# leimao/Voice-Converter-CycleGAN

Measured on NVIDIA H100. Metric: CycleGAN-VC train steps/sec @ batch 256x[24,128] MCEP, higher is better.
Workload: dtype f16f8 (forward / data gradient: fp16 MMA + two e4m3 cross-term MMAs = 2 MMA units per product; weight gradient: fp16 MMA alone, 1 unit; f32 accumulate)

## Files before the change

include/cgvc.h:

```cpp
#ifndef CGVC_H
#define CGVC_H

#include <stddef.h>
#include <stdint.h>

#ifdef __cplusplus
extern "C" {
#endif

#define CGVC_ABI_VERSION 1
#define CGVC_NUM_LOSSES 8

typedef struct cgvc_engine* cgvc_handle;

typedef struct cgvc_config {
  int num_features;
  int max_batch;
  int max_frames;
  int precision;
  int device;
  int train;
} cgvc_config;

enum {
  CGVC_PREC_FP32_SIMT = 0,
  CGVC_PREC_BF16X3 = 1,
  CGVC_PREC_BF16 = 2,
  CGVC_PREC_F16F8 = 3
};

enum cgvc_arena {
  CGVC_ARENA_PARAM = 0,
  CGVC_ARENA_GRAD = 1,
  CGVC_ARENA_ADAM_M = 2,
  CGVC_ARENA_ADAM_V = 3,
  CGVC_ARENA_WORK = 4,
  CGVC_ARENA_COUNT = 5
};

int cgvc_abi_version(void);
int cgvc_create(const cgvc_config* cfg, cgvc_handle* out);
int cgvc_destroy(cgvc_handle h);
const char* cgvc_last_error(cgvc_handle h);

int cgvc_arena_bytes(cgvc_handle h, int arena, size_t* bytes);
int cgvc_bind_arena(cgvc_handle h, int arena, void* dev_ptr, size_t bytes);

int cgvc_param_count(cgvc_handle h, int* n_tensors, size_t* n_elements);
int cgvc_param_info(cgvc_handle h, int index, const char** name, size_t* offset, int* ndim, int shape_out[4]);

int cgvc_params_updated(cgvc_handle h, void* stream);
int cgvc_set_adam_step(cgvc_handle h, long long t);
int cgvc_get_adam_step(cgvc_handle h, long long* t);

typedef struct cgvc_loss_scale_info {
  float scale;
  int good_steps;
  long long skipped;
  int last_skipped;
  unsigned nonfinite;
  unsigned long long sat_grad;
  unsigned long long sat_act;
} cgvc_loss_scale_info;
int cgvc_loss_scale_state(cgvc_handle h, cgvc_loss_scale_info* out_dev, void* stream);
int cgvc_set_loss_scale_state(cgvc_handle h, float scale, int good_steps, long long skipped, void* stream);

int cgvc_train_step(cgvc_handle h, const float* A_dev, const float* B_dev, int batch, int frames,
                    float lambda_cycle, float lambda_identity, float lr_generator, float lr_discriminator,
                    float* gen_A_dev, float* gen_B_dev, float* losses_dev, void* stream);

int cgvc_compute_gradients(cgvc_handle h, const float* A_dev, const float* B_dev, int batch, int frames,
                           float lambda_cycle, float lambda_identity,
                           float* gen_A_dev, float* gen_B_dev, float* losses_dev, void* stream);

int cgvc_adam_step(cgvc_handle h, float lr_generator, float lr_discriminator, float grad_scale, void* stream);

int cgvc_generator_forward(cgvc_handle h, int direction, const float* in_dev, float* out_dev,
                           int batch, int frames, void* stream);
int cgvc_generator_forward_packed(cgvc_handle h, int direction, const float* in_dev, float* out_dev,
                                  const long long* offsets_host, int n, void* stream);
int cgvc_discriminator_forward(cgvc_handle h, int which, const float* in_dev, float* out_dev,
                               int batch, int frames, void* stream);

int cgvc_debug_activation(cgvc_handle h, const char* name, float* out_dev, size_t capacity, size_t* n_out, void* stream);

int cgvc_sample_plan(cgvc_handle h, const long long* offsets_A_dev, int n_A, const long long* offsets_B_dev, int n_B,
                     unsigned long long seed, long long epoch, int crop_frames, int* plan_dev, int* err_dev, void* stream);
int cgvc_gather_minibatch(cgvc_handle h, const float* corpus_A_dev, const long long* offsets_A_dev, const float* corpus_B_dev,
                          const long long* offsets_B_dev, const int* plan_dev, int num_pairs, int first_pair, int batch, int crop_frames,
                          float* A_out_dev, float* B_out_dev, void* stream);

int cgvc_comm_unique_id(cgvc_handle h, void* id128_host);
int cgvc_comm_init(cgvc_handle h, const void* id128_host, int rank, int nranks);
int cgvc_comm_destroy(cgvc_handle h);
int cgvc_allreduce_grads(cgvc_handle h, void* stream);

int cgvc_kernel_launches(unsigned long long* count);
int cgvc_set_option(cgvc_handle h, const char* name, int value);
int cgvc_profile_enable(int on);
int cgvc_profile_collect(double* ms3, double* flops3, long long* launches3);
int cgvc_profile_launches(double* ms, double* flops, long long* meta4, int capacity, int* n_out);

int cgvc_conv_forward(cgvc_handle h, int precision, const float* x, const float* w, const float* bias, float* y,
                      int B, int H, int W, int Cin, int kh, int kw, int Cout, int sh, int sw, void* stream);
int cgvc_conv_backward(cgvc_handle h, int precision, const float* x, const float* w, const float* dy,
                       float* dx, float* dw, float* dbias,
                       int B, int H, int W, int Cin, int kh, int kw, int Cout, int sh, int sw, void* stream);
int cgvc_in_glu_forward(cgvc_handle h, const float* p, const float* beta_a, const float* gamma_a,
                        const float* beta_g, const float* gamma_g, float* y, float* stats,
                        int B, int R, int C, int shuffle, void* stream);
int cgvc_in_glu_backward(cgvc_handle h, const float* dy, const float* p, const float* stats,
                         const float* beta_a, const float* gamma_a, const float* beta_g, const float* gamma_g,
                         float* dp, float* dbeta_a, float* dgamma_a, float* dbeta_g, float* dgamma_g,
                         int B, int R, int C, int shuffle, void* stream);
int cgvc_split_planes(cgvc_handle h, int precision, const float* x, long long rows, int C, void* hi, void* lo,
                      unsigned long long* sat, void* stream);
int cgvc_im2col_planes(cgvc_handle h, int precision, const float* x, long long rows, int T, int C, int kw, int dir, void* hi, void* lo,
                       unsigned long long* sat, void* stream);
int cgvc_in_glu_forward_planes(cgvc_handle h, const float* p, const float* beta_a, const float* gamma_a,
                               const float* beta_g, const float* gamma_g, float* y, float* stats,
                               int B, int R, int C, int shuffle, int precision, int gate, const float* resid,
                               void* hi, void* lo, unsigned long long* sat, void* stream);
int cgvc_in_glu_backward_planes(cgvc_handle h, const float* dy, const float* p, const float* stats,
                                const float* beta_a, const float* gamma_a, const float* beta_g, const float* gamma_g,
                                float* dp, float* dbeta_a, float* dgamma_a, float* dbeta_g, float* dgamma_g,
                                int B, int R, int C, int shuffle, int precision, int gate,
                                void* hi, void* lo, unsigned long long* sat, void* stream);

enum {
  CGVC_OK = 0,
  CGVC_ERR_ARG = -1,
  CGVC_ERR_CUDA = -2,
  CGVC_ERR_UNBOUND = -3,
  CGVC_ERR_DIRECTION = -4,
  CGVC_ERR_UNSUPPORTED = -5,
  CGVC_ERR_NCCL = -6
};

#ifdef __cplusplus
}
#endif
#endif
```

voice-converter-cyclegan_b200/_native.py:

```python
from __future__ import annotations

import ctypes as C
import os

from . import build as _build

_LIB = None

ARENA_PARAM, ARENA_GRAD, ARENA_ADAM_M, ARENA_ADAM_V, ARENA_WORK = range(5)
PREC_FP32_SIMT, PREC_BF16X3, PREC_BF16, PREC_F16F8 = 0, 1, 2, 3
PRECISIONS = {"fp32": PREC_FP32_SIMT, "fp32_simt": PREC_FP32_SIMT, "bf16x3": PREC_BF16X3, "bf16": PREC_BF16, "f16f8": PREC_F16F8}
ERR_DIRECTION = -4
ERR_UNSUPPORTED = -5

LOSS_NAMES = ("cycle_loss", "identity_loss", "generator_loss_A2B", "generator_loss_B2A", "generator_loss",
              "discriminator_loss_A", "discriminator_loss_B", "discriminator_loss")


class Config(C.Structure):
    _fields_ = [("num_features", C.c_int), ("max_batch", C.c_int), ("max_frames", C.c_int),
                ("precision", C.c_int), ("device", C.c_int), ("train", C.c_int)]


LOSS_SCALE_MODES = {"static": 0, "monitor": 1, "dynamic": 2}


class LossScaleInfo(C.Structure):
    _fields_ = [("scale", C.c_float), ("good_steps", C.c_int), ("skipped", C.c_longlong), ("last_skipped", C.c_int),
                ("nonfinite", C.c_uint), ("sat_grad", C.c_ulonglong), ("sat_act", C.c_ulonglong)]


class CgvcError(RuntimeError):
    def __init__(self, code, msg):
        super().__init__("libcgvc error %d: %s" % (code, msg))
        self.code = code


def _declare(lib):
    vp, ci, cf, sz = C.c_void_p, C.c_int, C.c_float, C.c_size_t
    P = C.POINTER
    sig = {
        "cgvc_abi_version": (ci, []),
        "cgvc_create": (ci, [P(Config), P(vp)]),
        "cgvc_destroy": (ci, [vp]),
        "cgvc_last_error": (C.c_char_p, [vp]),
        "cgvc_arena_bytes": (ci, [vp, ci, P(sz)]),
        "cgvc_bind_arena": (ci, [vp, ci, vp, sz]),
        "cgvc_param_count": (ci, [vp, P(ci), P(sz)]),
        "cgvc_param_info": (ci, [vp, ci, P(C.c_char_p), P(sz), P(ci), P(ci * 4)]),
        "cgvc_params_updated": (ci, [vp, vp]),
        "cgvc_set_adam_step": (ci, [vp, C.c_longlong]),
        "cgvc_get_adam_step": (ci, [vp, P(C.c_longlong)]),
        "cgvc_loss_scale_state": (ci, [vp, vp, vp]),
        "cgvc_set_loss_scale_state": (ci, [vp, cf, ci, C.c_longlong, vp]),
        "cgvc_train_step": (ci, [vp, vp, vp, ci, ci, cf, cf, cf, cf, vp, vp, vp, vp]),
        "cgvc_compute_gradients": (ci, [vp, vp, vp, ci, ci, cf, cf, vp, vp, vp, vp]),
        "cgvc_adam_step": (ci, [vp, cf, cf, cf, vp]),
        "cgvc_generator_forward": (ci, [vp, ci, vp, vp, ci, ci, vp]),
        "cgvc_generator_forward_packed": (ci, [vp, ci, vp, vp, P(C.c_longlong), ci, vp]),
        "cgvc_discriminator_forward": (ci, [vp, ci, vp, vp, ci, ci, vp]),
        "cgvc_debug_activation": (ci, [vp, C.c_char_p, vp, sz, P(sz), vp]),
        "cgvc_comm_unique_id": (ci, [vp, vp]),
        "cgvc_comm_init": (ci, [vp, vp, ci, ci]),
        "cgvc_comm_destroy": (ci, [vp]),
        "cgvc_allreduce_grads": (ci, [vp, vp]),
        "cgvc_sample_plan": (ci, [vp, vp, ci, vp, ci, C.c_ulonglong, C.c_longlong, ci, vp, vp, vp]),
        "cgvc_gather_minibatch": (ci, [vp, vp, vp, vp, vp, vp, ci, ci, ci, ci, vp, vp, vp]),
        "cgvc_kernel_launches": (ci, [P(C.c_ulonglong)]),
        "cgvc_set_option": (ci, [vp, C.c_char_p, ci]),
        "cgvc_profile_enable": (ci, [ci]),
        "cgvc_profile_collect": (ci, [P(C.c_double), P(C.c_double), P(C.c_longlong)]),
        "cgvc_profile_launches": (ci, [P(C.c_double), P(C.c_double), P(C.c_longlong), ci, P(ci)]),
        "cgvc_conv_forward": (ci, [vp, ci, vp, vp, vp, vp] + [ci] * 9 + [vp]),
        "cgvc_conv_backward": (ci, [vp, ci, vp, vp, vp, vp, vp, vp] + [ci] * 9 + [vp]),
        "cgvc_in_glu_forward": (ci, [vp] * 8 + [ci] * 4 + [vp]),
        "cgvc_in_glu_backward": (ci, [vp] * 13 + [ci] * 4 + [vp]),
        "cgvc_split_planes": (ci, [vp, ci, vp, C.c_longlong, ci, vp, vp, vp, vp]),
        "cgvc_im2col_planes": (ci, [vp, ci, vp, C.c_longlong, ci, ci, ci, ci, vp, vp, vp, vp]),
        "cgvc_in_glu_forward_planes": (ci, [vp] * 8 + [ci] * 6 + [vp] * 5),
        "cgvc_in_glu_backward_planes": (ci, [vp] * 13 + [ci] * 6 + [vp] * 4),
    }
    for name, (res, args) in sig.items():
        fn = getattr(lib, name)
        fn.restype = res
        fn.argtypes = args
    return sig


EXPORTED_SYMBOLS = None


def lib_path():
    return _build.LIB


def load(build_if_missing=True):
    global _LIB, EXPORTED_SYMBOLS
    if _LIB is not None:
        return _LIB
    path = _build.LIB
    if build_if_missing and _build.is_stale():
        _build.build()
    if not os.path.exists(path):
        raise RuntimeError("libcgvc.so not found at %s (run __graft_entry__.build()); there is no CPU fallback" % path)
    lib = C.CDLL(path, mode=C.RTLD_GLOBAL)
    EXPORTED_SYMBOLS = sorted(_declare(lib).keys())
    if lib.cgvc_abi_version() != 1:
        raise RuntimeError("libcgvc.so ABI version mismatch")
    _LIB = lib
    return lib


def check(handle, code):
    if code != 0:
        msg = _LIB.cgvc_last_error(handle)
        raise CgvcError(code, msg.decode() if msg else "?")
```

voice-converter-cyclegan_b200/csrc/engine.cu:

```cuda
#include "../../include/cgvc.h"
#include "kernels.cuh"
#include "tc_gemm.cuh"
#include "geom.h"

#include <dlfcn.h>
#include <stddef.h>
#include <math.h>
#include <stdarg.h>
#include <stdio.h>
#include <string.h>

#include <map>
#include <string>
#include <utility>
#include <vector>

static thread_local std::string g_create_error;

#define ADAM_B1 0.5f
#define ADAM_B2 0.999f
#define ADAM_EPS 1e-8f

struct TensorInfo { std::string name; size_t off; int ndim; int shape[4]; size_t numel; };
struct ConvW { size_t k, b; int kh, kw, cin, cout; };
// ... 1124 lines not shown
  DeviceGuard dguard; CK(dguard.set(e->cfg.device));
  Bump ws; ws.reset(e->arena[CGVC_ARENA_WORK], e->arena_bytes[CGVC_ARENA_WORK]);
  TrainPlan P; plan_train(e, ws, P, B, T);
  if (ws.overflow) return fail(e, CGVC_ERR_UNBOUND, "WORK arena too small for batch %d x %d frames", B, T);
  const size_t img = (size_t)B * nf * T;
  float* sc = e->d_scalars; float* L = sc + 8;
  (void)lc;
  CK(cudaMemsetAsync(L, 0, 8 * sizeof(float), st));
  if (e->ls_mode) CK(cudaMemsetAsync(&e->ls->nonfinite, 0, (char*)(&e->ls->sat_act + 1) - (char*)&e->ls->nonfinite, st));
  struct Counting { cgvc_engine* e; ~Counting() { e->counting = false; } } counting{e};
  e->counting = true;
  CK(cudaMemsetAsync(e->G(), 0, e->n_params * sizeof(float), st));
  CK(launch_transpose_ft(A_dev, P.lane[0].in, B, nf, T, st));
  CK(launch_transpose_ft(B_dev, P.lane[0].in + img, B, nf, T, st));
  CK(cudaMemcpyAsync(P.lane[1].in, P.lane[0].in + img, img * sizeof(float), cudaMemcpyDeviceToDevice, st));
  CK(cudaMemcpyAsync(P.lane[1].in + img, P.lane[0].in, img * sizeof(float), cudaMemcpyDeviceToDevice, st));
  for (int l = 0; l < 2; ++l) {
    SideQ& q = e->sideq[l];
    q.on = e->side_wgrad && e->two_streams && !e->fuse_bwd && !tc_profile_is_on() && q.side != nullptr;
    q.used[0] = q.used[1] = false; q.cur = 0;
  }
  if (e->two_streams) {
    CK(cudaEventRecord(e->ev_fork, st));
    for (int l = 0; l < 2; ++l) CK(cudaStreamWaitEvent(e->lane_stream[l], e->ev_fork, 0));
    RET(run_lane(e, P.lane[0], 0, B_dev, B, T, li, gen_B_dev, e->lane_stream[0]));
    RET(run_lane(e, P.lane[1], 1, A_dev, B, T, li, gen_A_dev, e->lane_stream[1]));
    for (int l = 0; l < 2; ++l) { CK(cudaEventRecord(e->ev_join[l], e->lane_stream[l])); CK(cudaStreamWaitEvent(st, e->ev_join[l], 0)); }
  } else {
    RET(run_lane(e, P.lane[0], 0, B_dev, B, T, li, gen_B_dev, st));
    RET(run_lane(e, P.lane[1], 1, A_dev, B, T, li, gen_A_dev, st));
  }
  CK(launch_finalize_losses(L, sc, st));
  if (losses_dev) CK(cudaMemcpyAsync(losses_dev, L, 8 * sizeof(float), cudaMemcpyDeviceToDevice, st));
  return 0;
}

}

static int set_lambdas(cgvc_engine* e, float lc, float li, cudaStream_t st) {
  float v[6] = {lc, li, 0, 0, 0, 0};
  CK(launch_set_scalars(e->d_scalars, 0, 2, v, st));
  return 0;
}
static int set_adam_scalars(cgvc_engine* e, float lr_g, float lr_d, float grad_scale, cudaStream_t st, bool deferred = false) {
  e->adam_t += 1;
  if (deferred) {
    float v[6] = {lr_g, grad_scale, lr_d, grad_scale, 0, 0};
    CK(launch_set_scalars(e->d_scalars, 2, 4, v, st));
    return 0;
  }
  double t = (double)e->adam_t;
  double corr = sqrt(1.0 - pow((double)ADAM_B2, t)) / (1.0 - pow((double)ADAM_B1, t));
  float v[6] = {(float)(lr_g * corr), grad_scale, (float)(lr_d * corr), grad_scale, 0, 0};
  CK(launch_set_scalars(e->d_scalars, 2, 4, v, st));
  return 0;
}
static int adam_body(cgvc_engine* e, cudaStream_t st, const int* skip = nullptr) {
  float* p = e->P(); float* g = e->G(); float* m = (float*)e->arena[CGVC_ARENA_ADAM_M]; float* v = (float*)e->arena[CGVC_ARENA_ADAM_V];
  size_t gend = e->gen[1].end;
  CK(launch_adam(p, g, m, v, (long long)gend, e->d_scalars + 2, ADAM_B1, ADAM_B2, ADAM_EPS, st, skip));
  CK(launch_adam(p + gend, g + gend, m + gend, v + gend, (long long)(e->n_params - gend), e->d_scalars + 4, ADAM_B1, ADAM_B2, ADAM_EPS, st, skip));
  return cgvc_params_updated(e, (void*)st);
}

static int ls_check_grads(cgvc_engine* e, cudaStream_t st) {
  CK(launch_check_finite(e->G(), (long long)e->n_params, (long long)e->gen[1].end, &e->ls->nonfinite, st));
  return 0;
}
static int ls_update(cgvc_engine* e, cudaStream_t st) {
  CK(launch_loss_scale_update(e->ls, e->d_scalars + 2, e->cfg.precision == CGVC_PREC_F16F8, e->ls_growth, ADAM_B1, ADAM_B2, st));
  return 0;
}
static const int* ls_skip(const cgvc_engine* e) { return e->ls_mode == 2 ? &e->ls->last_skipped : nullptr; }

static int ls_prepare(cgvc_engine* e, int batch, cudaStream_t st) {
  const bool dyn = e->ls_mode == 2 && !e->ls_ready, mon = e->ls_mode == 1 && e->ls_batch != batch;
  if (!dyn && !mon) return 0;
  const float v[6] = {loss_scale(e, batch), 0, 0, 0, 0, 0};
  CK(launch_set_scalars(&e->ls->scale, 0, 1, v, st));
  e->ls_ready = e->ls_mode == 2; e->ls_batch = e->ls_mode == 1 ? batch : 0;
  return 0;
}

template <class Body>
static int run_captured(cgvc_engine* e, const GraphKey& key, cudaStream_t user, Body body) {
  if (!e->use_graphs || tc_profile_is_on()) return body(user);
  cudaStream_t st = user;
  const bool bridge = (user == nullptr || user == cudaStreamLegacy || user == cudaStreamPerThread);
  if (bridge) { st = e->graph_stream; CK(cudaEventRecord(e->ev_bridge, user)); CK(cudaStreamWaitEvent(st, e->ev_bridge, 0)); }
  auto it = e->graphs.find(key);
  GraphEntry ent{nullptr, 0};
  if (it != e->graphs.end()) ent = it->second;
  else {
    if (e->graphs.size() >= 16) { for (auto& kv : e->graphs) cudaGraphExecDestroy(kv.second.exec); e->graphs.clear(); }
    cudaGraph_t graph = nullptr;
    const unsigned long long before = g_cgvc_launches;
    cudaError_t ce = cudaStreamBeginCapture(st, cudaStreamCaptureModeThreadLocal);
    if (ce != cudaSuccess) { cudaGetLastError(); e->use_graphs = 0; return body(user); }
    int rc = body(st);
    ce = cudaStreamEndCapture(st, &graph);
    ent.launches = g_cgvc_launches - before;
    g_cgvc_launches = before;
    if (rc != 0 || ce != cudaSuccess || !graph) {
      if (graph) cudaGraphDestroy(graph);
      cudaGetLastError();
      if (rc != 0 && ce == cudaSuccess) return rc;
      e->use_graphs = 0;
      return body(user);
    }
    ce = cudaGraphInstantiate(&ent.exec, graph, 0);
    cudaGraphDestroy(graph);
    if (ce != cudaSuccess) { cudaGetLastError(); e->use_graphs = 0; return body(user); }
    e->graphs[key] = ent;
  }
  cudaGraphExec_t exec = ent.exec;
  g_cgvc_launches += ent.launches;
  CK(cudaGraphLaunch(exec, st));
  if (bridge) { CK(cudaEventRecord(e->ev_bridge2, st)); CK(cudaStreamWaitEvent(user, e->ev_bridge2, 0)); }
  return 0;
}

extern "C" {

int cgvc_compute_gradients(cgvc_handle e, const float* A_dev, const float* B_dev, int batch, int frames,
                           float lambda_cycle, float lambda_identity, float* gen_A_dev, float* gen_B_dev, float* losses_dev, void* stream) {
  if (!e || !A_dev || !B_dev) return fail(e, CGVC_ERR_ARG, "null argument");
  DeviceGuard dguard; CK(dguard.set(e->cfg.device));
  RET(set_lambdas(e, lambda_cycle, lambda_identity, (cudaStream_t)stream));
  RET(ls_prepare(e, batch, (cudaStream_t)stream));
  RET(forward_backward(e, A_dev, B_dev, batch, frames, lambda_cycle, lambda_identity, gen_A_dev, gen_B_dev, losses_dev, (cudaStream_t)stream));
  if (e->ls_mode == 2) CK(launch_scale(e->G(), (long long)e->n_params, 1.f, (cudaStream_t)stream, &e->ls->scale));
  else if (loss_scale(e, batch) != 1.f) CK(launch_scale(e->G(), (long long)e->n_params, 1.f / loss_scale(e, batch), (cudaStream_t)stream));
  return 0;
}

int cgvc_adam_step(cgvc_handle e, float lr_g, float lr_d, float grad_scale, void* stream) {
  if (!e) return CGVC_ERR_ARG;
  for (int a = 0; a < 4; ++a) if (!e->arena[a]) return fail(e, CGVC_ERR_UNBOUND, "PARAM/GRAD/ADAM_M/ADAM_V arenas must be bound");
  DeviceGuard dguard; CK(dguard.set(e->cfg.device));
  if (e->ls_mode == 2) { long long t; RET(cgvc_get_adam_step(e, &t)); }
  const long long t_before = e->adam_t;
  RET(set_adam_scalars(e, lr_g, lr_d, grad_scale, (cudaStream_t)stream));
  int r = adam_body(e, (cudaStream_t)stream);
  if (r != 0) { e->adam_t = t_before; return r; }
  if (e->ls_mode == 2) RET(cgvc_set_adam_step(e, e->adam_t));
  return 0;
}

int cgvc_train_step(cgvc_handle e, const float* A_dev, const float* B_dev, int batch, int frames,
                    float lambda_cycle, float lambda_identity, float lr_g, float lr_d,
                    float* gen_A_dev, float* gen_B_dev, float* losses_dev, void* stream) {
  if (!e || !A_dev || !B_dev) return fail(e, CGVC_ERR_ARG, "null argument");
  for (int a = 0; a < 4; ++a) if (!e->arena[a]) return fail(e, CGVC_ERR_UNBOUND, "PARAM/GRAD/ADAM_M/ADAM_V arenas must be bound");
  RET(check_bt(e, batch, frames, 16));
  DeviceGuard dguard; CK(dguard.set(e->cfg.device));
  cudaStream_t st = (cudaStream_t)stream;
  const float gscale = (e->comm ? 1.f / (float)e->nranks : 1.f) / loss_scale(e, batch);
  RET(set_lambdas(e, lambda_cycle, lambda_identity, st));
  const long long adam_t_before = e->adam_t;
  struct Rollback { cgvc_engine* e; long long t; bool armed; ~Rollback() { if (armed) e->adam_t = t; } } rollback{e, adam_t_before, true};
  RET(set_adam_scalars(e, lr_g, lr_d, e->ls_mode == 2 ? (e->comm ? 1.f / (float)e->nranks : 1.f) : gscale, st, e->ls_mode == 2));
  RET(ls_prepare(e, batch, st));
  if (e->use_graphs && !tc_profile_is_on()) {
    const size_t img = (size_t)batch * e->cfg.num_features * frames;
    const size_t cap = (size_t)e->cfg.max_batch * e->cfg.num_features * e->cfg.max_frames;
    if (!e->stage) CK(cudaMalloc(&e->stage, 2 * cap * sizeof(float)));
    float* sA = e->stage; float* sB = e->stage + cap;
    CK(cudaMemcpyAsync(sA, A_dev, img * sizeof(float), cudaMemcpyDeviceToDevice, st));
    CK(cudaMemcpyAsync(sB, B_dev, img * sizeof(float), cudaMemcpyDeviceToDevice, st));
    GraphKey key; memset(&key, 0, sizeof key);
    key.batch = batch; key.frames = frames; key.id_off = lambda_identity == 0.f; key.lanes = e->two_streams; key.fuse = e->fuse_in | (e->fuse_bwd << 1) | (e->side_wgrad << 2) | (e->fuse_c1 << 3) | (e->edge_lower << 4); key.kind = 0;
    RET(run_captured(e, key, st, [&](cudaStream_t s) {
      return forward_backward(e, sA, sB, batch, frames, lambda_cycle, lambda_identity, nullptr, nullptr, nullptr, s);
    }));
    if (gen_A_dev || gen_B_dev) {
      Bump ws; ws.reset(e->arena[CGVC_ARENA_WORK], e->arena_bytes[CGVC_ARENA_WORK]);
      TrainPlan P; plan_train(e, ws, P, batch, frames);
      if (gen_B_dev) CK(cudaMemcpyAsync(gen_B_dev, P.lane[0].din + img, img * sizeof(float), cudaMemcpyDeviceToDevice, st));
      if (gen_A_dev) CK(cudaMemcpyAsync(gen_A_dev, P.lane[1].din + img, img * sizeof(float), cudaMemcpyDeviceToDevice, st));
    }
    if (losses_dev) CK(cudaMemcpyAsync(losses_dev, e->d_scalars + 8, 8 * sizeof(float), cudaMemcpyDeviceToDevice, st));
  } else {
    RET(forward_backward(e, A_dev, B_dev, batch, frames, lambda_cycle, lambda_identity, gen_A_dev, gen_B_dev, losses_dev, st));
  }
  if (e->comm && e->pipelined_comm && e->comm_stream) {
    auto al4 = [](size_t v) { return (v + 3) & ~(size_t)3; };
    const size_t cut[5] = {0, al4(e->gen[1].begin), al4(e->disc[0].begin), al4(e->disc[1].begin), e->n_params};
    struct Range { size_t b, n; const float* hyper; } rg[4];
    for (int k = 0; k < 4; ++k) { rg[k].b = cut[k]; rg[k].n = cut[k + 1] - cut[k]; rg[k].hyper = e->d_scalars + (k < 2 ? 2 : 4); }
    CK(cudaEventRecord(e->ev_grads, st));
    CK(cudaStreamWaitEvent(e->comm_stream, e->ev_grads, 0));
    for (int k = 0; k < 4; ++k) {
      int r = e->nccl.AllReduce(e->G() + rg[k].b, e->G() + rg[k].b, rg[k].n, 7, 0, e->comm, e->comm_stream);
      if (r != 0) return fail(e, CGVC_ERR_NCCL, "ncclAllReduce: %s", e->nccl.GetErrorString ? e->nccl.GetErrorString(r) : "?");
      CK(cudaEventRecord(e->ev_ar[k], e->comm_stream));
    }
    if (e->ls_mode) {
      if (e->ls_mode == 2) {
        int r = e->nccl.AllReduce(&e->ls->sat_grad, &e->ls->sat_grad, 1, 5, 0, e->comm, e->comm_stream);
        if (r != 0) return fail(e, CGVC_ERR_NCCL, "ncclAllReduce: %s", e->nccl.GetErrorString ? e->nccl.GetErrorString(r) : "?");
      }
      RET(ls_check_grads(e, e->comm_stream));
      CK(cudaEventRecord(e->ev_ls, e->comm_stream));
      if (e->ls_mode == 2) { CK(cudaStreamWaitEvent(st, e->ev_ls, 0)); RET(ls_update(e, st)); }
    }
    float* pp = e->P(); float* gg = e->G(); float* mm = (float*)e->arena[CGVC_ARENA_ADAM_M]; float* vv = (float*)e->arena[CGVC_ARENA_ADAM_V];
    for (int k = 0; k < 4; ++k) {
      CK(cudaStreamWaitEvent(st, e->ev_ar[k], 0));
      GraphKey kk; memset(&kk, 0, sizeof kk); kk.kind = 2 + k;
      const Range R = rg[k];
      RET(run_captured(e, kk, st, [&](cudaStream_t s) {
        CK(launch_adam(pp + R.b, gg + R.b, mm + R.b, vv + R.b, (long long)R.n, R.hyper, ADAM_B1, ADAM_B2, ADAM_EPS, s, ls_skip(e)));
        if (e->cfg.precision != CGVC_PREC_FP32_SIMT) {
          int r = tc_refresh_weights_range(e->tcw, pp, R.b, R.b + R.n, s);
          if (r != 0) return fail(e, CGVC_ERR_CUDA, "tc_refresh_weights: %s", cudaGetErrorString((cudaError_t)r));
        }
        return 0;
      }));
    }
    if (e->ls_mode == 1) CK(cudaStreamWaitEvent(st, e->ev_ls, 0));
    rollback.armed = false;
    return 0;
  }
  if (e->comm) {
    RET(cgvc_allreduce_grads(e, stream));
    if (e->ls_mode == 2) {
      int r = e->nccl.AllReduce(&e->ls->sat_grad, &e->ls->sat_grad, 1, 5, 0, e->comm, st);
      if (r != 0) return fail(e, CGVC_ERR_NCCL, "ncclAllReduce: %s", e->nccl.GetErrorString ? e->nccl.GetErrorString(r) : "?");
    }
  }
  GraphKey k2; memset(&k2, 0, sizeof k2); k2.kind = 1;
  RET(run_captured(e, k2, st, [&](cudaStream_t s) {
    if (e->ls_mode) RET(ls_check_grads(e, s));
    if (e->ls_mode == 2) RET(ls_update(e, s));
    return adam_body(e, s, ls_skip(e));
  }));
  rollback.armed = false;
  return 0;
}

static int load_nccl(cgvc_engine* e) {
  if (e->nccl.lib) return 0;
  const char* names[] = {"libnccl.so.2", "libnccl.so"};
  void* lib = nullptr;
  for (const char* n : names) { lib = dlopen(n, RTLD_NOW | RTLD_GLOBAL); if (lib) break; }
  if (!lib) return fail(e, CGVC_ERR_NCCL, "cannot dlopen libnccl.so.2: %s", dlerror());
  e->nccl.lib = lib;
  *(void**)&e->nccl.GetUniqueId = dlsym(lib, "ncclGetUniqueId");
  *(void**)&e->nccl.CommInitRank = dlsym(lib, "ncclCommInitRank");
  *(void**)&e->nccl.CommDestroy = dlsym(lib, "ncclCommDestroy");
  *(void**)&e->nccl.AllReduce = dlsym(lib, "ncclAllReduce");
  *(void**)&e->nccl.GetErrorString = dlsym(lib, "ncclGetErrorString");
  if (!e->nccl.GetUniqueId || !e->nccl.CommInitRank || !e->nccl.AllReduce || !e->nccl.CommDestroy)
    return fail(e, CGVC_ERR_NCCL, "libnccl is missing required symbols");
  return 0;
}

int cgvc_comm_unique_id(cgvc_handle e, void* id128_host) {
  if (!e || !id128_host) return CGVC_ERR_ARG;
  RET(load_nccl(e));
  int r = e->nccl.GetUniqueId(id128_host);
  if (r != 0) return fail(e, CGVC_ERR_NCCL, "ncclGetUniqueId: %s", e->nccl.GetErrorString ? e->nccl.GetErrorString(r) : "?");
  return 0;
}

int cgvc_comm_init(cgvc_handle e, const void* id128_host, int rank, int nranks) {
  if (!e || !id128_host || nranks < 1 || rank < 0 || rank >= nranks) return fail(e, CGVC_ERR_ARG, "cgvc_comm_init: bad argument");
  RET(load_nccl(e));
  DeviceGuard dguard; CK(dguard.set(e->cfg.device));
  Id128 id; memcpy(id.b, id128_host, 128);
  int r = e->nccl.CommInitRank(&e->comm, nranks, id, rank);
  if (r != 0) { e->comm = nullptr; return fail(e, CGVC_ERR_NCCL, "ncclCommInitRank: %s", e->nccl.GetErrorString ? e->nccl.GetErrorString(r) : "?"); }
  e->rank = rank; e->nranks = nranks;
  return 0;
}

int cgvc_comm_destroy(cgvc_handle e) {
  if (!e) return CGVC_ERR_ARG;
  if (e->comm) { e->nccl.CommDestroy(e->comm); e->comm = nullptr; e->nranks = 1; e->rank = 0; }
  return 0;
}

int cgvc_allreduce_grads(cgvc_handle e, void* stream) {
  if (!e) return CGVC_ERR_ARG;
  if (!e->comm) return fail(e, CGVC_ERR_NCCL, "no communicator attached");
  if (!e->arena[CGVC_ARENA_GRAD]) return fail(e, CGVC_ERR_UNBOUND, "GRAD arena must be bound");
  int r = e->nccl.AllReduce(e->G(), e->G(), e->n_params, 7, 0, e->comm, (cudaStream_t)stream);
  if (r != 0) return fail(e, CGVC_ERR_NCCL, "ncclAllReduce: %s", e->nccl.GetErrorString ? e->nccl.GetErrorString(r) : "?");
  return 0;
}

int cgvc_set_option(cgvc_handle e, const char* name, int value) {
  if (!e || !name) return CGVC_ERR_ARG;
  if (!strcmp(name, "two_streams")) { e->two_streams = value != 0; return 0; }
  if (!strcmp(name, "fuse_in")) { e->fuse_in = value != 0; return 0; }
  if (!strcmp(name, "fuse_bwd")) { e->fuse_bwd = value != 0; return 0; }
  if (!strcmp(name, "edge_lower")) { e->edge_lower = value != 0; return 0; }
  if (!strcmp(name, "side_wgrad")) { e->side_wgrad = value != 0; return 0; }
  if (!strcmp(name, "pipelined_comm")) { e->pipelined_comm = value != 0; return 0; }
  if (!strcmp(name, "fuse_c1")) { e->fuse_c1 = value != 0; return 0; }
  if (!strcmp(name, "debug_taps")) { e->debug_taps = value != 0; return 0; }
  if (!strcmp(name, "cuda_graph")) { e->use_graphs = value != 0; return 0; }
  if (!strcmp(name, "tc_debug")) { tc_set_debug(value); return 0; }
  if (!strcmp(name, "post_onepass")) {
    post_set_onepass(value);
    for (auto& kv : e->graphs) cudaGraphExecDestroy(kv.second.exec);
    e->graphs.clear();
    return 0;
  }
  if (!strcmp(name, "wgrad_f16")) {
    e->tcw.wgrad16 = value != 0;
    for (auto& kv : e->graphs) cudaGraphExecDestroy(kv.second.exec);
    e->graphs.clear();
    return 0;
  }
  if (!strcmp(name, "loss_scale") || !strcmp(name, "loss_scale_growth_interval")) {
    const bool mode = !strcmp(name, "loss_scale");
    if (mode ? (value < 0 || value > 2) : value < 1) return fail(e, CGVC_ERR_ARG, "option %s: bad value %d", name, value);
    if (mode && value != e->ls_mode) {
      DeviceGuard dguard; CK(dguard.set(e->cfg.device));
      long long t = 0;
      RET(cgvc_get_adam_step(e, &t));
      e->ls_mode = value;
      RET(cgvc_set_adam_step(e, t));
      e->ls_ready = false; e->ls_batch = 0;
    }
    if (!mode) e->ls_growth = value;
    for (auto& kv : e->graphs) cudaGraphExecDestroy(kv.second.exec);
    e->graphs.clear();
    return 0;
  }
  if (!strcmp(name, "post_stream")) {
    post_set_stream(value);
    for (auto& kv : e->graphs) cudaGraphExecDestroy(kv.second.exec);
    e->graphs.clear();
    return 0;
  }
  if (!strcmp(name, "prep_batched")) {
    tc_set_prep_batched(value);
    for (auto& kv : e->graphs) cudaGraphExecDestroy(kv.second.exec);
    e->graphs.clear();
    return 0;
  }
  return fail(e, CGVC_ERR_ARG, "unknown option '%s'", name);
}
int cgvc_kernel_launches(unsigned long long* count) { if (!count) return CGVC_ERR_ARG; *count = g_cgvc_launches; return 0; }
int cgvc_profile_enable(int on) { tc_profile_enable(on); return 0; }
int cgvc_profile_launches(double* ms, double* flops, long long* meta4, int capacity, int* n_out) {
  if (!ms || !flops || !meta4 || capacity < 0) return CGVC_ERR_ARG;
  return tc_profile_launches(ms, flops, meta4, capacity, n_out) == 0 ? 0 : CGVC_ERR_CUDA;
}
int cgvc_profile_collect(double* ms3, double* flops3, long long* launches3) {
  if (!ms3 || !flops3 || !launches3) return CGVC_ERR_ARG;
  return tc_profile_collect(ms3, flops3, launches3) == 0 ? 0 : CGVC_ERR_CUDA;
}

int cgvc_sample_plan(cgvc_handle e, const long long* offsets_A_dev, int n_A, const long long* offsets_B_dev, int n_B,
                     unsigned long long seed, long long epoch, int crop_frames, int* plan_dev, int* err_dev, void* stream) {
  if (!e || !offsets_A_dev || !offsets_B_dev || !plan_dev || !err_dev) return fail(e, CGVC_ERR_ARG, "null argument");
  if (n_A < 1 || n_B < 1 || crop_frames < 1 || epoch < 0) return fail(e, CGVC_ERR_ARG, "cgvc_sample_plan: empty corpus or bad crop / epoch");
  DeviceGuard dguard; CK(dguard.set(e->cfg.device));
  CK(cudaMemsetAsync(err_dev, 0, sizeof(int), (cudaStream_t)stream));
  CK(launch_sample_plan(offsets_A_dev, n_A, offsets_B_dev, n_B, seed, epoch, crop_frames, plan_dev, err_dev, (cudaStream_t)stream));
  return 0;
}

int cgvc_gather_minibatch(cgvc_handle e, const float* corpus_A_dev, const long long* offsets_A_dev, const float* corpus_B_dev,
                          const long long* offsets_B_dev, const int* plan_dev, int num_pairs, int first_pair, int batch, int crop_frames,
                          float* A_out_dev, float* B_out_dev, void* stream) {
  if (!e || !corpus_A_dev || !corpus_B_dev || !offsets_A_dev || !offsets_B_dev || !plan_dev || !A_out_dev || !B_out_dev)
    return fail(e, CGVC_ERR_ARG, "null argument");
  if (batch < 1 || first_pair < 0 || first_pair + batch > num_pairs || crop_frames < 1)
    return fail(e, CGVC_ERR_ARG, "cgvc_gather_minibatch: pairs [%d, %d) outside the epoch's %d", first_pair, first_pair + batch, num_pairs);
  DeviceGuard dguard; CK(dguard.set(e->cfg.device));
  CK(launch_gather_minibatch(corpus_A_dev, offsets_A_dev, corpus_B_dev, offsets_B_dev, plan_dev, num_pairs, first_pair, batch,
                             e->cfg.num_features, crop_frames, A_out_dev, B_out_dev, (cudaStream_t)stream));
  return 0;
}

int cgvc_conv_forward(cgvc_handle e, int precision, const float* x, const float* w, const float* bias, float* y,
                      int B, int H, int W, int Cin, int kh, int kw, int Cout, int sh, int sw, void* stream) {
  if (!e || !x || !w || !y) return fail(e, CGVC_ERR_ARG, "null argument");
  if (kh * kw > CGVC_MAX_TAPS) return fail(e, CGVC_ERR_UNSUPPORTED, "at most %d filter taps", CGVC_MAX_TAPS);
  DeviceGuard dguard; CK(dguard.set(e->cfg.device));
  cudaStream_t st = (cudaStream_t)stream;
  if (precision != CGVC_PREC_FP32_SIMT)
    return tc_result(e, tc_conv_fwd_adhoc(precision, x, w, bias, y, B, H, W, Cin, kh, kw, Cout, sh, sw, st), nullptr, "conv forward");
  GatherGeom g = fwd_geom(B, H, W, kh, kw, sh, sw);
  GemmOperands op; memset(&op, 0, sizeof op);
  op.src = x; op.s_ld = Cin; op.C = Cin; op.w = w; op.w_ts = (long long)Cin * Cout; op.w_cs = Cout; op.w_ns = 1; op.N = Cout;
  op.dst = y; op.d_ld = Cout; op.bias = bias;
  CK(launch_gg_simt(g, op, st));
  return 0;
}

int cgvc_conv_backward(cgvc_handle e, int precision, const float* x, const float* w, const float* dy,
                       float* dx, float* dw, float* dbias, int B, int H, int W, int Cin, int kh, int kw, int Cout, int sh, int sw, void* stream) {
  if (!e || !x || !w || !dy) return fail(e, CGVC_ERR_ARG, "null argument");
  if (kh * kw > CGVC_MAX_TAPS) return fail(e, CGVC_ERR_UNSUPPORTED, "at most %d filter taps", CGVC_MAX_TAPS);
  DeviceGuard dguard; CK(dguard.set(e->cfg.device));
  cudaStream_t st = (cudaStream_t)stream;
  if (precision != CGVC_PREC_FP32_SIMT)
    return tc_result(e, tc_conv_bwd_adhoc(precision, x, w, dy, dx, dw, dbias, B, H, W, Cin, kh, kw, Cout, sh, sw, st, e->tcw.wgrad16 ? 1 : 0),
                     nullptr, "conv backward");
  ConvW c; c.k = 0; c.b = 0; c.kh = kh; c.kw = kw; c.cin = Cin; c.cout = Cout;
  if (dx) RET(conv_dgrad_simt(e, w, c, sh, sw, B, H, W, dy, Cout, 0, dx, 0, st));
  if (dw) {
    GatherGeom g = fwd_geom(B, H, W, kh, kw, sh, sw);
    CK(launch_wgrad_simt(g, x, Cin, 0, Cin, dy, Cout, 0, Cout, dw, (long long)Cin * Cout, Cout, 1, st));
    if (dbias) CK(launch_colsum(dy, (long long)g.B * g.Hy * g.Wx, Cout, 0, Cout, dbias, st));
  }
  return 0;
}

static int plane_precision(cgvc_engine* e, int precision, const void* hi, const void* lo) {
  if (precision != CGVC_PREC_BF16X3 && precision != CGVC_PREC_BF16 && precision != CGVC_PREC_F16F8)
    return fail(e, CGVC_ERR_ARG, "operand planes: precision %d has none", precision);
  if (!hi || !lo) return fail(e, CGVC_ERR_ARG, "null argument");
  return 0;
}

int cgvc_split_planes(cgvc_handle e, int precision, const float* x, long long rows, int C, void* hi, void* lo,
                      unsigned long long* sat, void* stream) {
  if (!e || !x) return fail(e, CGVC_ERR_ARG, "null argument");
  RET(plane_precision(e, precision, hi, lo));
  if (rows < 0 || C < 1) return fail(e, CGVC_ERR_ARG, "cgvc_split_planes: bad shape [%lld, %d]", rows, C);
  DeviceGuard dguard; CK(dguard.set(e->cfg.device));
  CK(tc_split_planes(precision, x, rows, C, (__nv_bfloat16*)hi, (__nv_bfloat16*)lo, (cudaStream_t)stream, sat));
  return 0;
}

int cgvc_im2col_planes(cgvc_handle e, int precision, const float* x, long long rows, int T, int C, int kw, int dir, void* hi, void* lo,
                       unsigned long long* sat, void* stream) {
  if (!e || !x) return fail(e, CGVC_ERR_ARG, "null argument");
  RET(plane_precision(e, precision, hi, lo));
  if (T < 1 || rows < 0 || rows % T || C < 4 || C % 4 || kw < 1 || kw > CGVC_MAX_TAPS || (dir != 1 && dir != -1))
    return fail(e, CGVC_ERR_ARG, "cgvc_im2col_planes: bad shape (rows %lld, T %d, C %d, kw %d, dir %d)", rows, T, C, kw, dir);
  DeviceGuard dguard; CK(dguard.set(e->cfg.device));
  CK(launch_im2col_taps(x, rows, T, C, kw, dir, edge_cpad(kw * C), precision == CGVC_PREC_F16F8, hi, lo, (cudaStream_t)stream,
                        nullptr, 0, sat));
  return 0;
}

int cgvc_in_glu_forward_planes(cgvc_handle e, const float* p, const float* beta_a, const float* gamma_a, const float* beta_g,
                               const float* gamma_g, float* y, float* stats, int B, int R, int C, int shuffle, int precision, int gate,
                               const float* resid, void* hi, void* lo, unsigned long long* sat, void* stream) {
  if (!e || !p || !y || !stats) return fail(e, CGVC_ERR_ARG, "null argument");
  if (C % 32 != 0 || shuffle < 1 || R % shuffle != 0) return fail(e, CGVC_ERR_UNSUPPORTED, "C must be a multiple of 32 and R of shuffle");
  if (precision != CGVC_PREC_FP32_SIMT) RET(plane_precision(e, precision, hi, lo));
  DeviceGuard dguard; CK(dguard.set(e->cfg.device));
  PostParams q; memset(&q, 0, sizeof q);
  q.p = p; q.ldp = (gate ? 2 : 1) * C * shuffle; q.Cc = C * shuffle; q.B = B; q.R = R; q.C = C; q.sh = shuffle;
  q.beta_a = beta_a; q.gamma_a = gamma_a; q.beta_g = beta_g; q.gamma_g = gamma_g; q.has_in = 1; q.has_gate = gate != 0; q.resid = resid;
  q.y = y; q.stats = stats;
  if (precision != CGVC_PREC_FP32_SIMT) {
    q.y_hi = (__nv_bfloat16*)hi; q.y_lo = (__nv_bfloat16*)lo; q.qmode = precision == CGVC_PREC_F16F8; q.sat = q.qmode ? sat : nullptr;
  }
  CK(launch_post_fwd(q, (cudaStream_t)stream));
  return 0;
}

int cgvc_in_glu_backward_planes(cgvc_handle e, const float* dy, const float* p, const float* stats,
                                const float* beta_a, const float* gamma_a, const float* beta_g, const float* gamma_g,
                                float* dp, float* dbeta_a, float* dgamma_a, float* dbeta_g, float* dgamma_g,
                                int B, int R, int C, int shuffle, int precision, int gate, void* hi, void* lo, unsigned long long* sat,
                                void* stream) {
  if (!e || !dy || !p || !stats || !dp) return fail(e, CGVC_ERR_ARG, "null argument");
  if (C % 32 != 0 || shuffle < 1 || R % shuffle != 0) return fail(e, CGVC_ERR_UNSUPPORTED, "C must be a multiple of 32 and R of shuffle");
  if (precision != CGVC_PREC_FP32_SIMT) RET(plane_precision(e, precision, hi, lo));
  DeviceGuard dguard; CK(dguard.set(e->cfg.device));
  PostBwdParams q; memset(&q, 0, sizeof q);
  q.dy1 = dy; q.p = p; q.ldp = (gate ? 2 : 1) * C * shuffle; q.Cc = C * shuffle; q.B = B; q.R = R; q.C = C; q.sh = shuffle;
  q.beta_a = beta_a; q.gamma_a = gamma_a; q.beta_g = beta_g; q.gamma_g = gamma_g; q.has_in = 1; q.has_gate = gate != 0; q.stats = stats;
  q.dp = dp; q.dbeta_a = dbeta_a; q.dgamma_a = dgamma_a; q.dbeta_g = dbeta_g; q.dgamma_g = dgamma_g;
  if (precision != CGVC_PREC_FP32_SIMT) {
    q.dp_hi = (__nv_bfloat16*)hi; q.dp_lo = (__nv_bfloat16*)lo; q.qmode = precision == CGVC_PREC_F16F8; q.sat = q.qmode ? sat : nullptr;
  }
  CK(launch_post_bwd(q, (cudaStream_t)stream));
  return 0;
}

int cgvc_in_glu_forward(cgvc_handle e, const float* p, const float* beta_a, const float* gamma_a, const float* beta_g, const float* gamma_g,
                        float* y, float* stats, int B, int R, int C, int shuffle, void* stream) {
  return cgvc_in_glu_forward_planes(e, p, beta_a, gamma_a, beta_g, gamma_g, y, stats, B, R, C, shuffle, CGVC_PREC_FP32_SIMT, 1, nullptr,
                                    nullptr, nullptr, nullptr, stream);
}

int cgvc_in_glu_backward(cgvc_handle e, const float* dy, const float* p, const float* stats,
                         const float* beta_a, const float* gamma_a, const float* beta_g, const float* gamma_g,
                         float* dp, float* dbeta_a, float* dgamma_a, float* dbeta_g, float* dgamma_g,
                         int B, int R, int C, int shuffle, void* stream) {
  return cgvc_in_glu_backward_planes(e, dy, p, stats, beta_a, gamma_a, beta_g, gamma_g, dp, dbeta_a, dgamma_a, dbeta_g, dgamma_g,
                                     B, R, C, shuffle, CGVC_PREC_FP32_SIMT, 1, nullptr, nullptr, nullptr, stream);
}

}
```

voice-converter-cyclegan_b200/csrc/geom.h:

```cpp
#pragma once
#include "kernels.cuh"
#include <string.h>
#include <vector>

static inline void same_pad(int n, int k, int s, int& before, int& out) {
  out = (n + s - 1) / s;
  int total = (out - 1) * s + k - n; if (total < 0) total = 0;
  before = total / 2;
}

static inline GatherGeom fwd_geom(int B, int H, int W, int kh, int kw, int sh, int sw) {
  GatherGeom g; memset(&g, 0, sizeof g);
  int ph, pw, Ho, Wo; same_pad(H, kh, sh, ph, Ho); same_pad(W, kw, sw, pw, Wo);
  g.B = B; g.Hy = Ho; g.Wx = Wo; g.Hs = H; g.Ws = W; g.sy = sh; g.sx = sw;
  g.Hd = Ho; g.Wd = Wo; g.dsy = 1; g.dsx = 1; g.doy = 0; g.dox = 0;
  g.ntaps = 0;
  for (int i = 0; i < kh; ++i) for (int j = 0; j < kw; ++j) {
    g.oy[g.ntaps] = (short)(i - ph); g.ox[g.ntaps] = (short)(j - pw); g.widx[g.ntaps] = (short)(i * kw + j); g.ntaps++;
  }
  return g;
}

static inline bool divisible(int v, int s) { return ((v % s) + s) % s == 0; }

static inline std::vector<GatherGeom> dgrad_geoms(int B, int H, int W, int kh, int kw, int sh, int sw) {
  std::vector<GatherGeom> out;
  int ph, pw, Ho, Wo; same_pad(H, kh, sh, ph, Ho); same_pad(W, kw, sw, pw, Wo);
  for (int py = 0; py < sh; ++py) for (int px = 0; px < sw; ++px) {
    GatherGeom g; memset(&g, 0, sizeof g);
    g.B = B; g.Hy = (H - py + sh - 1) / sh; g.Wx = (W - px + sw - 1) / sw;
    if (g.Hy <= 0 || g.Wx <= 0) continue;
    g.Hs = Ho; g.Ws = Wo; g.sy = 1; g.sx = 1;
    g.Hd = H; g.Wd = W; g.dsy = sh; g.dsx = sw; g.doy = py; g.dox = px;
    g.ntaps = 0;
    for (int i = 0; i < kh; ++i) for (int j = 0; j < kw; ++j) {
      if (!divisible(py + ph - i, sh) || !divisible(px + pw - j, sw)) continue;
      g.oy[g.ntaps] = (short)((py + ph - i) / sh); g.ox[g.ntaps] = (short)((px + pw - j) / sw);
      g.widx[g.ntaps] = (short)(i * kw + j); g.ntaps++;
    }
    out.push_back(g);
  }
  return out;
}
```

voice-converter-cyclegan_b200/csrc/tc_gemm.cu:

```cuda
#include "tc_gemm.cuh"
#include "geom.h"
#include "kernels.cuh"
#include "wgmma.cuh"

#include <cuda.h>
#include <stdint.h>
#include <stdio.h>

namespace {

typedef CUresult (*EncodeTiledFn)(CUtensorMap*, CUtensorMapDataType, cuuint32_t, void*, const cuuint64_t*, const cuuint64_t*,
                                  const cuuint32_t*, const cuuint32_t*, CUtensorMapInterleave, CUtensorMapSwizzle,
                                  CUtensorMapL2promotion, CUtensorMapFloatOOBfill);
EncodeTiledFn get_encoder() {
  static EncodeTiledFn fn = nullptr;
  if (!fn) {
    void* p = nullptr; cudaDriverEntryPointQueryResult q;
    if (cudaGetDriverEntryPoint("cuTensorMapEncodeTiled", &p, cudaEnableDefault, &q) == cudaSuccess && q == cudaDriverEntryPointSuccess)
      fn = (EncodeTiledFn)p;
  }
  return fn;
}
bool make_tmap3(CUtensorMap* m, const void* base, uint64_t d0, uint64_t d1, uint64_t d2, uint32_t b1) {
  EncodeTiledFn enc = get_encoder();
  if (!enc) return false;
  cuuint64_t dims[3] = {d0, d1, d2};
  cuuint64_t strides[2] = {d0 * 2, d0 * d1 * 2};
  cuuint32_t box[3] = {64, b1, 1};
  cuuint32_t es[3] = {1, 1, 1};
  return enc(m, CU_TENSOR_MAP_DATA_TYPE_BFLOAT16, 3, const_cast<void*>(base), dims, strides, box, es, CU_TENSOR_MAP_INTERLEAVE_NONE,
             CU_TENSOR_MAP_SWIZZLE_128B, CU_TENSOR_MAP_L2_PROMOTION_L2_256B, CU_TENSOR_MAP_FLOAT_OOB_FILL_NONE) == CUDA_SUCCESS;
}

bool make_tmap3_t(CUtensorMap* m, const void* base, CUtensorMapDataType dt, int esize, uint64_t d0, uint64_t d1, uint64_t d2, uint32_t b0, uint32_t b1) {
  EncodeTiledFn enc = get_encoder();
  if (!enc) return false;
  cuuint64_t dims[3] = {d0, d1, d2};
  cuuint64_t strides[2] = {d0 * (uint64_t)esize, d0 * d1 * (uint64_t)esize};
  cuuint32_t box[3] = {b0, b1, 1};
  cuuint32_t es[3] = {1, 1, 1};
  return enc(m, dt, 3, const_cast<void*>(base), dims, strides, box, es, CU_TENSOR_MAP_INTERLEAVE_NONE,
             b0 * esize == 64 ? CU_TENSOR_MAP_SWIZZLE_64B : CU_TENSOR_MAP_SWIZZLE_128B, CU_TENSOR_MAP_L2_PROMOTION_L2_256B,
             CU_TENSOR_MAP_FLOAT_OOB_FILL_NONE) == CUDA_SUCCESS;
}

__device__ __forceinline__ uint32_t smem_u32(const void* p) { return (uint32_t)__cvta_generic_to_shared(p); }

__device__ __forceinline__ void mbar_init(uint64_t* bar, uint32_t count) {
  asm volatile("mbarrier.init.shared::cta.b64 [%0], %1;" ::"r"(smem_u32(bar)), "r"(count));
}
__device__ __forceinline__ void fence_barrier_init() { asm volatile("fence.mbarrier_init.release.cluster;" ::: "memory"); }
__device__ __forceinline__ void mbar_wait(uint64_t* bar, uint32_t parity) {
  asm volatile(
      "{\n\t"
      ".reg .pred p;\n\t"
      "WAIT_LOOP:\n\t"
      "mbarrier.try_wait.parity.shared::cta.b64 p, [%0], %1;\n\t"
      "@p bra.uni WAIT_DONE;\n\t"
      "bra.uni WAIT_LOOP;\n\t"
      "WAIT_DONE:\n\t"
      "}" ::"r"(smem_u32(bar)), "r"(parity) : "memory");
}
__device__ __forceinline__ void cp_async16(uint32_t dst_smem, const void* src, uint32_t src_bytes) {
  asm volatile("cp.async.cg.shared.global [%0], [%1], 16, %2;" ::"r"(dst_smem), "l"(src), "r"(src_bytes) : "memory");
}
__device__ __forceinline__ void cp_async_arrive_noinc(uint64_t* bar) {
  asm volatile("cp.async.mbarrier.arrive.noinc.shared::cta.b64 [%0];" ::"r"(smem_u32(bar)) : "memory");
}
__device__ __forceinline__ void mbar_expect_tx(uint64_t* bar, uint32_t bytes) {
  asm volatile("mbarrier.arrive.expect_tx.shared::cta.b64 _, [%0], %1;" ::"r"(smem_u32(bar)), "r"(bytes) : "memory");
}
__device__ __forceinline__ void tma_load3(uint32_t dst_smem, const CUtensorMap* map, int c0, int c1, int c2, uint64_t* bar) {
  asm volatile("cp.async.bulk.tensor.3d.shared::cluster.global.tile.mbarrier::complete_tx::bytes [%0], [%1, {%2, %3, %4}], [%5];"
               ::"r"(dst_smem), "l"(map), "r"(c0), "r"(c1), "r"(c2), "r"(smem_u32(bar)) : "memory");
}
__device__ __forceinline__ void tma_prefetch_desc(const CUtensorMap* map) {
  asm volatile("prefetch.tensormap [%0];" ::"l"(map) : "memory");
}
__device__ __forceinline__ void fence_proxy_async() { asm volatile("fence.proxy.async.shared::cta;" ::: "memory"); }
__device__ __forceinline__ uint64_t make_desc(uint32_t smem_addr, uint32_t lbo_bytes, uint32_t sbo_bytes, uint64_t layout = 1) {
  return (uint64_t)((smem_addr >> 4) & 0x3FFF) | ((uint64_t)((lbo_bytes >> 4) & 0x3FFF) << 16) |
         ((uint64_t)((sbo_bytes >> 4) & 0x3FFF) << 32) | (layout << 62);
}
__device__ __forceinline__ uint64_t make_desc64(uint32_t smem_addr) { return make_desc(smem_addr, 16, 512, 2); }
template <int N>
__device__ __forceinline__ void fence_acc(float (&d)[N]) {
#pragma unroll
  for (int i = 0; i < N; ++i) asm volatile("" : "+f"(d[i])::"memory");
}
__device__ __forceinline__ void mbar_arrive(uint64_t* bar) {
  asm volatile("mbarrier.arrive.shared::cta.b64 _, [%0];" ::"r"(smem_u32(bar)) : "memory");
}
__device__ __forceinline__ void consumer_bar() { asm volatile("bar.sync 3, 256;" ::: "memory"); }
__device__ __forceinline__ void st_shared16(uint32_t addr, uint4 v) {
  asm volatile("st.shared.v4.b32 [%0], {%1, %2, %3, %4};" ::"r"(addr), "r"(v.x), "r"(v.y), "r"(v.z), "r"(v.w) : "memory");
}
__device__ __forceinline__ uint4 e4m3x8_to_f16x8(uint2 v) {
  uint32_t w[4];
#pragma unroll
  for (int i = 0; i < 4; ++i) {
    const uint32_t src = (i < 2 ? v.x : v.y) >> (16 * (i & 1));
    const __half2_raw h = __nv_cvt_fp8x2_to_halfraw2((__nv_fp8x2_storage_t)(src & 0xFFFFu), __NV_E4M3);
    w[i] = (uint32_t)h.x | ((uint32_t)h.y << 16);
  }
  return make_uint4(w[0], w[1], w[2], w[3]);
}

struct FastDiv { uint32_t mul, shr, d; };
__host__ inline FastDiv make_fastdiv(uint32_t d) {
  FastDiv f; f.d = d;
  uint32_t l = 0; while ((1ull << l) < d) ++l;
  f.mul = (uint32_t)(((1ull << 32) * ((1ull << l) - d)) / d + 1);
  f.shr = l;
  return f;
}
__device__ __forceinline__ uint32_t fdiv(uint32_t n, const FastDiv& f) { return (uint32_t)(((uint64_t)__umulhi(n, f.mul) + n) >> f.shr); }

__device__ __forceinline__ uint32_t sw128(int r, int c) { return (uint32_t)((r >> 3) * 1024 + (r & 7) * 128 + ((c ^ (r & 7)) << 4)); }

struct TcNTParams {
  GatherGeom g;
  const __nv_bfloat16 *a_hi, *a_lo; int a_ld; int C;
  const __nv_bfloat16 *b_hi, *b_lo; int Nw;
  int N;
  int n_tiles;
  int debug;
  float* dst; int d_ld; const float* bias; int accumulate;
  int perm; int Cc;
  int R;
  const float *gamma_a, *beta_a, *gamma_g, *beta_g;
  float* stats;
  const float* resid;
  float* y; __nv_bfloat16 *y_hi, *y_lo;
  int C_out;
  const float* bp; int bp_ld;
  __nv_bfloat16 *dp_hi, *dp_lo; int dp_ld;
  float *dbeta_a, *dgamma_a, *dbeta_g, *dgamma_g;
  CUtensorMap tm_b_hi, tm_b_lo;
  const uint8_t *a8_hi, *a8_lo;
  CUtensorMap tm_b8_hi, tm_b8_lo;
  uint8_t* y8;
  PackGeom pk;
};

struct TcTNParams {
  GatherGeom g;
  const __nv_bfloat16 *x_hi, *x_lo; int x_ld; int C;
  const __nv_bfloat16 *g_hi, *g_lo; int g_ld; int N;
  float* dw_a; float* dw_g; int n_split;
  int ksplit;
  FastDiv div_hw, div_w;
  CUtensorMap tm_g_hi, tm_g_lo;
  const uint8_t *x8_hi, *x8_lo;
  const uint8_t *g8_hi, *g8_lo;
  int w16;
  int fold_n;
};

__device__ __forceinline__ float* tn_dst(float* base, int slab, int C, int c, int ncols, int col, int fold_n) {
  if (fold_n) { const int t = col / fold_n; return base + ((long long)t * C + c) * fold_n + (col - t * fold_n); }
  return base + ((long long)slab * C + c) * ncols + col;
}

constexpr int kProducerThreads = 128;


template <int BN, int NPL>
struct NTCfg {
  static constexpr int A_PLANE = 128 * 128;
  static constexpr int B_PLANE = BN * 128;
  static constexpr int PLANES = NPL == 2 ? 2 : 1;
  static constexpr int STAGE = PLANES * (A_PLANE + B_PLANE);
  static constexpr int STAGES = (192 * 1024) / STAGE;
  static constexpr int SMEM = STAGES * STAGE + 1024;
  static_assert(STAGES * STAGE >= 128 * BN * 4, "the finished fp32 tile is staged over the pipeline stages");
};

template <int BN>
__device__ __forceinline__ int acc_off(int r, int n) { return r * BN + (n & ~31) + ((((n >> 2) & 7) ^ (r & 7)) << 2) + (n & 3); }
template <int BN>
__device__ __forceinline__ void acc_ld32(const float* acc, int r, int col, uint32_t (&v)[32]) {
#pragma unroll
  for (int c = 0; c < 8; ++c) {
    const float4 x = *reinterpret_cast<const float4*>(acc + r * BN + col + ((c ^ (r & 7)) << 2));
    v[4 * c] = __float_as_uint(x.x); v[4 * c + 1] = __float_as_uint(x.y); v[4 * c + 2] = __float_as_uint(x.z); v[4 * c + 3] = __float_as_uint(x.w);
  }
}

__device__ __forceinline__ float warp_colsum32(float (&t)[32], int lane) {
#pragma unroll
  for (int o = 16, n = 32; o >= 1; o >>= 1, n >>= 1) {
    const bool up = (lane & o) != 0;
#pragma unroll
    for (int i = 0; i < n / 2; ++i) {
      float send = up ? t[i] : t[i + n / 2];
      float keep = up ? t[i + n / 2] : t[i];
      t[i] = keep + __shfl_xor_sync(0xffffffffu, send, o);
    }
  }
  return t[0];
}
__device__ __forceinline__ void epi_bar(int id) { asm volatile("bar.sync %0, 128;" ::"r"(id) : "memory"); }

__device__ __forceinline__ float sample_sum(float v, float (*xch)[32], int q, int lane, int spw, int barid) {
  if (spw == 1) return v;
  epi_bar(barid);
  xch[q][lane] = v;
  epi_bar(barid);
  const int q0 = (q / spw) * spw;
  float r = 0.f;
  for (int w = 0; w < spw; ++w) r += xch[q0 + w][lane];
  return r;
}
__device__ __forceinline__ void bc4(const float* p, float (&v)[4]) { const float4 x = *reinterpret_cast<const float4*>(p); v[0] = x.x; v[1] = x.y; v[2] = x.z; v[3] = x.w; }
__device__ __forceinline__ float fast_sigmoid(float x) { return __fdividef(1.f, 1.f + __expf(-x)); }
__device__ __forceinline__ void chunk_norm_coeffs(const float (&v)[32], const float* __restrict__ gamma, const float* __restrict__ beta,
                                                  int ch, int R, float (*xch)[32], float* bc, int q, int lane, int spw, int barid, float& mean, float& rstd) {
  float t[32];
#pragma unroll
  for (int k = 0; k < 32; ++k) t[k] = v[k];
  float s = warp_colsum32(t, lane);
  s = sample_sum(s, xch, q, lane, spw, barid);
  mean = s / (float)R;
  __syncwarp();
  bc[lane] = mean;
  __syncwarp();
#pragma unroll
  for (int k = 0; k < 32; k += 4) {
    float4 m4 = *reinterpret_cast<const float4*>(bc + k);
    float d0 = v[k] - m4.x, d1 = v[k + 1] - m4.y, d2 = v[k + 2] - m4.z, d3 = v[k + 3] - m4.w;
    t[k] = d0 * d0; t[k + 1] = d1 * d1; t[k + 2] = d2 * d2; t[k + 3] = d3 * d3;
  }
  float ss = warp_colsum32(t, lane);
  ss = sample_sum(ss, xch, q, lane, spw, barid);
  rstd = 1.f / sqrtf(ss / (float)R + 1e-6f);
  const float sc = rstd * gamma[ch + lane];
  const float of = beta[ch + lane] - mean * sc;
  __syncwarp();
  bc[lane] = sc; bc[32 + lane] = of;
  __syncwarp();
}

__device__ __forceinline__ void pair_norm_coeffs(const float (&v0)[32], const float (&v1)[32], const float* __restrict__ gamma, const float* __restrict__ beta,
                                                 int ch, int R, float (*xch)[32], float* bc, int q, int lane, int spw, int barid, float& mean, float& rstd) {
  float t[32];
#pragma unroll
  for (int k = 0; k < 32; ++k) t[k] = v0[k] + v1[k];
  float s = warp_colsum32(t, lane);
  s = sample_sum(s, xch, q, lane, spw, barid);
  const float inv = 1.f / (float)(2 * R);
  mean = s * inv;
  __syncwarp();
  bc[lane] = mean;
  __syncwarp();
#pragma unroll
  for (int k = 0; k < 32; k += 4) {
    float4 m4 = *reinterpret_cast<const float4*>(bc + k);
    const float m[4] = {m4.x, m4.y, m4.z, m4.w};
#pragma unroll
    for (int j = 0; j < 4; ++j) { const float d0 = v0[k + j] - m[j], d1 = v1[k + j] - m[j]; t[k + j] = fmaf(d0, d0, d1 * d1); }
  }
  float ss = warp_colsum32(t, lane);
  ss = sample_sum(ss, xch, q, lane, spw, barid);
  rstd = 1.f / sqrtf(ss * inv + 1e-6f);
  const float sc = rstd * gamma[ch + lane];
  const float of = beta[ch + lane] - mean * sc;
  __syncwarp();
  bc[lane] = sc; bc[32 + lane] = of;
  __syncwarp();
}

__device__ __forceinline__ uint32_t hp_off(int r, int c) { return (uint32_t)(r * 16 + ((c ^ ((r >> 1) & 3)) << 2)); }
template <class F>
__device__ __forceinline__ void rows_out(float* stg, const float (&o)[32], int lane, F f) {
  const int hc = lane & 3, hr = lane >> 2;
#pragma unroll
  for (int h = 0; h < 2; ++h) {
    __syncwarp();
#pragma unroll
    for (int c = 0; c < 4; ++c)
      *reinterpret_cast<float4*>(stg + hp_off(lane, c)) = make_float4(o[16 * h + 4 * c], o[16 * h + 4 * c + 1], o[16 * h + 4 * c + 2], o[16 * h + 4 * c + 3]);
    __syncwarp();
#pragma unroll
    for (int i = 0; i < 4; ++i) {
      const int rr = hr + 8 * i;
      f(rr, 16 * h + 4 * hc, *reinterpret_cast<const float4*>(stg + hp_off(rr, hc)));
    }
  }
}
__device__ __forceinline__ void rows_in(float* stg, float (&v)[32], int lane, const float4 (&pre)[8]) {
  const int hc = lane & 3, hr = lane >> 2;
#pragma unroll
  for (int h = 0; h < 2; ++h) {
    __syncwarp();
#pragma unroll
    for (int i = 0; i < 4; ++i) *reinterpret_cast<float4*>(stg + hp_off(hr + 8 * i, hc)) = pre[4 * h + i];
    __syncwarp();
#pragma unroll
    for (int c = 0; c < 4; ++c) {
      const float4 x = *reinterpret_cast<const float4*>(stg + hp_off(lane, c));
      v[16 * h + 4 * c] = x.x; v[16 * h + 4 * c + 1] = x.y; v[16 * h + 4 * c + 2] = x.z; v[16 * h + 4 * c + 3] = x.w;
    }
  }
}
__device__ __forceinline__ void rows_fetch(float4 (&pre)[8], const float* base, long long ld, long long mq, long long M, int col, int lane) {
  const int hc = lane & 3, hr = lane >> 2;
#pragma unroll
  for (int h = 0; h < 2; ++h)
#pragma unroll
    for (int i = 0; i < 4; ++i) {
      const int rr = hr + 8 * i;
      pre[4 * h + i] = make_float4(0.f, 0.f, 0.f, 0.f);
      if (mq + rr < M) pre[4 * h + i] = *reinterpret_cast<const float4*>(base + (mq + rr) * ld + col + 16 * h + 4 * hc);
    }
}
__device__ __forceinline__ void hload_rows(float* stg, float (&v)[32], const float* base, long long ld, long long mq, long long M, int col, int lane) {
  float4 pre[8];
  rows_fetch(pre, base, ld, mq, M, col, lane);
  rows_in(stg, v, lane, pre);
}
__device__ __forceinline__ void hwrite_rows_f32(float* stg, const float (&o)[32], float* const* rowp, int col0, int lane) {
  rows_out(stg, o, lane, [&](int rr, int w0, float4 val) {
    float* rp = rowp[rr];
    if (rp != nullptr) *reinterpret_cast<float4*>(rp + col0 + w0) = val;
  });
}
__device__ __forceinline__ void hwrite_y(float* stg, const float (&y)[32], float* yf, __nv_bfloat16* yhi, __nv_bfloat16* ylo,
                                         long long mq, long long M, int C, int ch, int lane, int rs = 1, int ro = 0) {
  if (yf)
    rows_out(stg, y, lane, [&](int rr, int w0, float4 val) {
      if (mq + rr < M) *reinterpret_cast<float4*>(yf + ((mq + rr) * rs + ro) * C + ch + w0) = val;
    });
  float hl[32];
#pragma unroll
  for (int k = 0; k < 16; ++k) {
    __nv_bfloat162 hh = __floats2bfloat162_rn(y[2 * k], y[2 * k + 1]);
    float2 f = __bfloat1622float2(hh);
    __nv_bfloat162 ll = __floats2bfloat162_rn(y[2 * k] - f.x, y[2 * k + 1] - f.y);
    hl[k] = __uint_as_float(*reinterpret_cast<uint32_t*>(&hh)); hl[16 + k] = __uint_as_float(*reinterpret_cast<uint32_t*>(&ll));
  }
  rows_out(stg, hl, lane, [&](int rr, int w0, float4 val) {
    __nv_bfloat16* plane = (w0 < 16) ? yhi : ylo;
    if (mq + rr < M) *reinterpret_cast<float4*>(plane + ((mq + rr) * rs + ro) * C + ch + 2 * (w0 & 15)) = val;
  });
}
__device__ __forceinline__ void hwrite_yq(float* stg, const float (&y)[32], float* yf, __nv_bfloat16* q16, uint8_t* q8,
                                          long long mq, long long M, int C, int ch, int lane, int rs = 1, int ro = 0) {
  if (yf)
    rows_out(stg, y, lane, [&](int rr, int w0, float4 val) {
      if (mq + rr < M) *reinterpret_cast<float4*>(yf + ((mq + rr) * rs + ro) * C + ch + w0) = val;
    });
  float w[32];
#pragma unroll
  for (int k = 0; k < 8; ++k) {
    const float v[4] = {y[4 * k], y[4 * k + 1], y[4 * k + 2], y[4 * k + 3]};
    uint2 h; uint32_t b_hi, b_lo;
    cgvc_quant4(v, CGVC_Q_ACT_SHI, CGVC_Q_ACT_SLO, h, b_hi, b_lo);
    w[2 * k] = __uint_as_float(h.x); w[2 * k + 1] = __uint_as_float(h.y);
    w[16 + k] = __uint_as_float(b_hi); w[24 + k] = __uint_as_float(b_lo);
  }
  rows_out(stg, w, lane, [&](int rr, int w0, float4 val) {
    if (mq + rr >= M) return;
    const long long r = (mq + rr) * rs + ro;
    uint8_t* dst;
    if (w0 < 16) dst = reinterpret_cast<uint8_t*>(q16) + (r * C + ch + 2 * w0) * 2;
    else if (w0 < 24) dst = q8 + r * C + ch + 4 * (w0 - 16);
    else dst = q8 + M * rs * C + r * C + ch + 4 * (w0 - 24);
    *reinterpret_cast<float4*>(dst) = val;
  });
}

template <int BN, int NPL, int EPI>
__device__ __forceinline__ void nt_tile_epilogue(const TcNTParams& p, const long long M, const int HW, const long long m0, const int n0,
                                                 const int q, const int lane, float* stg, float** rowp, float* bc, float (*epi_xch)[32],
                                                 const float* acc, const int grp = 0, const int ngrp = 1) {
  const GatherGeom& g = p.g;
  const int barid = 1 + grp;
  const int arow = q * 32 + lane;
  const long long mq = m0 + q * 32;
  const long long m = mq + lane;
  float* drow = nullptr;
  if (m < M && p.dst) {
    int b = (int)(m / HW); int rem = (int)(m - (long long)b * HW);
    int y = rem / g.Wx; int x = rem - y * g.Wx;
    long long dr = ((long long)(b * g.Hd + y * g.dsy + g.doy) * g.Wd + x * g.dsx + g.dox);
    drow = p.dst + dr * p.d_ld;
  }
  __syncwarp();
  rowp[lane] = drow;
  __syncwarp();
  {
    const int spw = p.R >> 5;
    const long long sample = mq / p.R;
    const bool stat_writer = (q % spw) == 0 && mq < M && p.stats != nullptr;
    if (EPI == 1) {
      const int ch0 = n0 >> 1;
#pragma unroll 1
      for (int cb = grp; cb < 4; cb += ngrp) {
        const int ch = ch0 + cb * 32;
        float va[32], vg[32];
        { uint32_t u[32]; acc_ld32<BN>(acc, arow, (cb * 32), u);
#pragma unroll
          for (int k = 0; k < 32; k += 4) { float4 bb = *reinterpret_cast<const float4*>(p.bias + n0 + cb * 32 + k);
            va[k] = __uint_as_float(u[k]) + bb.x; va[k + 1] = __uint_as_float(u[k + 1]) + bb.y; va[k + 2] = __uint_as_float(u[k + 2]) + bb.z; va[k + 3] = __uint_as_float(u[k + 3]) + bb.w; } }
        { uint32_t u[32]; acc_ld32<BN>(acc, arow, (128 + cb * 32), u);
#pragma unroll
          for (int k = 0; k < 32; k += 4) { float4 bb = *reinterpret_cast<const float4*>(p.bias + n0 + 128 + cb * 32 + k);
            vg[k] = __uint_as_float(u[k]) + bb.x; vg[k + 1] = __uint_as_float(u[k + 1]) + bb.y; vg[k + 2] = __uint_as_float(u[k + 2]) + bb.z; vg[k + 3] = __uint_as_float(u[k + 3]) + bb.w; } }
        if (p.dst) {
          hwrite_rows_f32(stg, va, rowp, ch, lane);
          hwrite_rows_f32(stg, vg, rowp, p.Cc + ch, lane);
        }
        float mean_a, rstd_a, mean_g, rstd_g;
        chunk_norm_coeffs(va, p.gamma_a, p.beta_a, ch, p.R, epi_xch, bc, q, lane, spw, barid, mean_a, rstd_a);
        chunk_norm_coeffs(vg, p.gamma_g, p.beta_g, ch, p.R, epi_xch, bc + 64, q, lane, spw, barid, mean_g, rstd_g);
        if (stat_writer) {
          float* st = p.stats + sample * 4 * p.C_out + ch + lane;
          st[0] = mean_a; st[p.C_out] = rstd_a; st[2 * p.C_out] = mean_g; st[3 * p.C_out] = rstd_g;
        }
#pragma unroll
        for (int k = 0; k < 32; k += 4) {
          float4 sa = *reinterpret_cast<const float4*>(bc + k), oa = *reinterpret_cast<const float4*>(bc + 32 + k);
          float4 sg = *reinterpret_cast<const float4*>(bc + 64 + k), og = *reinterpret_cast<const float4*>(bc + 96 + k);
          va[k]     = fmaf(va[k],     sa.x, oa.x) * fast_sigmoid(fmaf(vg[k],     sg.x, og.x));
          va[k + 1] = fmaf(va[k + 1], sa.y, oa.y) * fast_sigmoid(fmaf(vg[k + 1], sg.y, og.y));
          va[k + 2] = fmaf(va[k + 2], sa.z, oa.z) * fast_sigmoid(fmaf(vg[k + 2], sg.z, og.z));
          va[k + 3] = fmaf(va[k + 3], sa.w, oa.w) * fast_sigmoid(fmaf(vg[k + 3], sg.w, og.w));
        }
        if (NPL == 3) hwrite_yq(stg, va, p.y, p.y_hi, p.y8, mq, M, p.C_out, ch, lane);
        else hwrite_y(stg, va, p.y, p.y_hi, p.y_lo, mq, M, p.C_out, ch, lane);
      }
    } else if (EPI == 5) {
      const int Ch = p.C_out;
      const int ch0 = n0 >> 2;
#pragma unroll 1
      for (int cb = grp; cb < 2; cb += ngrp) {
        const int ch = ch0 + cb * 32;
        auto load = [&](float (&v)[32], int tcol) {
          uint32_t u[32]; acc_ld32<BN>(acc, arow, tcol, u);
#pragma unroll
          for (int k = 0; k < 32; k += 4) { float4 bb = *reinterpret_cast<const float4*>(p.bias + n0 + tcol + k);
            v[k] = __uint_as_float(u[k]) + bb.x; v[k + 1] = __uint_as_float(u[k + 1]) + bb.y; v[k + 2] = __uint_as_float(u[k + 2]) + bb.z; v[k + 3] = __uint_as_float(u[k + 3]) + bb.w; }
        };
        float mean_a, rstd_a, mean_g, rstd_g;
        {
          float g0[32], g1[32];
          load(g0, 128 + cb * 32); load(g1, 192 + cb * 32);
          if (p.dst) { hwrite_rows_f32(stg, g0, rowp, p.Cc + ch, lane); hwrite_rows_f32(stg, g1, rowp, p.Cc + Ch + ch, lane); }
          pair_norm_coeffs(g0, g1, p.gamma_g, p.beta_g, ch, p.R, epi_xch, bc + 64, q, lane, spw, barid, mean_g, rstd_g);
        }
        float a0[32], a1[32];
        load(a0, cb * 32); load(a1, 64 + cb * 32);
        if (p.dst) { hwrite_rows_f32(stg, a0, rowp, ch, lane); hwrite_rows_f32(stg, a1, rowp, Ch + ch, lane); }
        pair_norm_coeffs(a0, a1, p.gamma_a, p.beta_a, ch, p.R, epi_xch, bc, q, lane, spw, barid, mean_a, rstd_a);
        if (stat_writer) {
          float* st = p.stats + sample * 4 * Ch + ch + lane;
          st[0] = mean_a; st[Ch] = rstd_a; st[2 * Ch] = mean_g; st[3 * Ch] = rstd_g;
        }
        auto emit = [&](const float (&a)[32], const int s) {
          float gg[32];
          load(gg, 128 + s * 64 + cb * 32);
#pragma unroll
          for (int k = 0; k < 32; k += 4) {
            float4 sa = *reinterpret_cast<const float4*>(bc + k), oa = *reinterpret_cast<const float4*>(bc + 32 + k);
            float4 sg = *reinterpret_cast<const float4*>(bc + 64 + k), og = *reinterpret_cast<const float4*>(bc + 96 + k);
            gg[k]     = fmaf(a[k],     sa.x, oa.x) * fast_sigmoid(fmaf(gg[k],     sg.x, og.x));
            gg[k + 1] = fmaf(a[k + 1], sa.y, oa.y) * fast_sigmoid(fmaf(gg[k + 1], sg.y, og.y));
            gg[k + 2] = fmaf(a[k + 2], sa.z, oa.z) * fast_sigmoid(fmaf(gg[k + 2], sg.z, og.z));
            gg[k + 3] = fmaf(a[k + 3], sa.w, oa.w) * fast_sigmoid(fmaf(gg[k + 3], sg.w, og.w));
          }
          if (NPL == 3) hwrite_yq(stg, gg, p.y, p.y_hi, p.y8, mq, M, Ch, ch, lane, 2, s);
          else hwrite_y(stg, gg, p.y, p.y_hi, p.y_lo, mq, M, Ch, ch, lane, 2, s);
        };
        emit(a1, 1);
        emit(a0, 0);
      }
    } else if (EPI == 2) {
#pragma unroll 1
      for (int cb = grp; cb < BN / 32; cb += ngrp) {
        const int ch = n0 + cb * 32;
        if (ch >= p.N) break;
        float4 rpre[8];
        rows_fetch(rpre, p.resid, p.C_out, mq, M, ch, lane);
        float va[32];
        { uint32_t u[32]; acc_ld32<BN>(acc, arow, (cb * 32), u);
#pragma unroll
          for (int k = 0; k < 32; k += 4) { float4 bb = *reinterpret_cast<const float4*>(p.bias + ch + k);
            va[k] = __uint_as_float(u[k]) + bb.x; va[k + 1] = __uint_as_float(u[k + 1]) + bb.y; va[k + 2] = __uint_as_float(u[k + 2]) + bb.z; va[k + 3] = __uint_as_float(u[k + 3]) + bb.w; } }
        if (p.dst) hwrite_rows_f32(stg, va, rowp, ch, lane);
        float mean_a, rstd_a;
        chunk_norm_coeffs(va, p.gamma_a, p.beta_a, ch, p.R, epi_xch, bc, q, lane, spw, barid, mean_a, rstd_a);
        if (stat_writer) {
          float* st = p.stats + sample * 4 * p.C_out + ch + lane;
          st[0] = mean_a; st[p.C_out] = rstd_a; st[2 * p.C_out] = 0.f; st[3 * p.C_out] = 1.f;
        }
        float res[32];
        rows_in(stg, res, lane, rpre);
#pragma unroll
        for (int k = 0; k < 32; k += 4) {
          float4 scl = *reinterpret_cast<const float4*>(bc + k), of = *reinterpret_cast<const float4*>(bc + 32 + k);
          va[k] = fmaf(va[k], scl.x, of.x) + res[k]; va[k + 1] = fmaf(va[k + 1], scl.y, of.y) + res[k + 1];
          va[k + 2] = fmaf(va[k + 2], scl.z, of.z) + res[k + 2]; va[k + 3] = fmaf(va[k + 3], scl.w, of.w) + res[k + 3];
        }
        if (NPL == 3) hwrite_yq(stg, va, p.y, p.y_hi, p.y8, mq, M, p.C_out, ch, lane);
        else hwrite_y(stg, va, p.y, p.y_hi, p.y_lo, mq, M, p.C_out, ch, lane);
      }
    } else {
      const int C = p.C_out;
      const float invR = 1.f / (float)p.R;
      const bool live = mq < M;
#pragma unroll 1
      for (int cb = grp; cb < BN / 32; cb += ngrp) {
        const int ch = n0 + cb * 32;
        if (ch >= p.N) break;
        float dy[32], xa[32];
        { uint32_t u[32]; acc_ld32<BN>(acc, arow, (cb * 32), u);
#pragma unroll
          for (int k = 0; k < 32; ++k) dy[k] = __uint_as_float(u[k]); }
        if (p.accumulate) {
          hload_rows(stg, xa, p.dst, p.d_ld, mq, M, ch, lane);
#pragma unroll
          for (int k = 0; k < 32; ++k) dy[k] += xa[k];
        }
        if (EPI == 4) {
          rows_out(stg, dy, lane, [&](int rr, int w0, float4 val) {
            if (mq + rr < M) *reinterpret_cast<float4*>(p.dst + (mq + rr) * p.d_ld + ch + w0) = val;
          });
        }
        {
          const float* st = p.stats + sample * 4 * C + ch + lane;
          const float mean = live ? st[0] : 0.f, rstd = live ? st[C] : 1.f;
          const float scl = rstd * p.gamma_a[ch + lane];
          __syncwarp();
          bc[lane] = rstd; bc[32 + lane] = -mean * rstd; bc[64 + lane] = scl;
          if (EPI == 3) {
            bc[96 + lane] = p.beta_a[ch + lane] - mean * scl;
            const float mg = live ? st[2 * C] : 0.f, rg = live ? st[3 * C] : 1.f;
            const float sg = rg * p.gamma_g[ch + lane];
            bc[128 + lane] = rg; bc[160 + lane] = -mg * rg; bc[192 + lane] = sg; bc[224 + lane] = p.beta_g[ch + lane] - mg * sg;
          }
          __syncwarp();
        }
        hload_rows(stg, xa, p.bp, p.bp_ld, mq, M, ch, lane);
        float dg[32], xg[32];
        if (EPI == 3) {
          hload_rows(stg, xg, p.bp, p.bp_ld, mq, M, C + ch, lane);
#pragma unroll
          for (int k = 0; k < 32; k += 4) {
            float ra[4], ha[4], sa[4], oa[4], rg[4], hg[4], sg[4], og[4];
            bc4(bc + k, ra); bc4(bc + 32 + k, ha); bc4(bc + 64 + k, sa); bc4(bc + 96 + k, oa);
            bc4(bc + 128 + k, rg); bc4(bc + 160 + k, hg); bc4(bc + 192 + k, sg); bc4(bc + 224 + k, og);
#pragma unroll
            for (int j = 0; j < 4; ++j) {
              const float na = fmaf(xa[k + j], sa[j], oa[j]), ng = fmaf(xg[k + j], sg[j], og[j]);
              const float sgm = fast_sigmoid(ng);
              const float dna = dy[k + j] * sgm;
              dy[k + j] = dna; dg[k + j] = dna * na * (1.f - sgm);
              xa[k + j] = fmaf(xa[k + j], ra[j], ha[j]);
              xg[k + j] = fmaf(xg[k + j], rg[j], hg[j]);
            }
          }
        } else {
#pragma unroll
          for (int k = 0; k < 32; k += 4) {
            float ra[4], ha[4];
            bc4(bc + k, ra); bc4(bc + 32 + k, ha);
#pragma unroll
            for (int j = 0; j < 4; ++j) xa[k + j] = fmaf(xa[k + j], ra[j], ha[j]);
          }
        }
        float t[32];
#pragma unroll
        for (int k = 0; k < 32; ++k) t[k] = dy[k];
        float s1a = warp_colsum32(t, lane);
#pragma unroll
        for (int k = 0; k < 32; ++k) t[k] = dy[k] * xa[k];
        float s2a = warp_colsum32(t, lane);
        float s1g = 0.f, s2g = 0.f;
        if (EPI == 3) {
#pragma unroll
          for (int k = 0; k < 32; ++k) t[k] = dg[k];
          s1g = warp_colsum32(t, lane);
#pragma unroll
          for (int k = 0; k < 32; ++k) t[k] = dg[k] * xg[k];
          s2g = warp_colsum32(t, lane);
        }
        if (p.dbeta_a && live) {
          atomicAdd(p.dbeta_a + ch + lane, s1a); atomicAdd(p.dgamma_a + ch + lane, s2a);
          if (EPI == 3) { atomicAdd(p.dbeta_g + ch + lane, s1g); atomicAdd(p.dgamma_g + ch + lane, s2g); }
        }
        s1a = sample_sum(s1a, epi_xch, q, lane, spw, barid); s2a = sample_sum(s2a, epi_xch, q, lane, spw, barid);
        if (EPI == 3) { s1g = sample_sum(s1g, epi_xch, q, lane, spw, barid); s2g = sample_sum(s2g, epi_xch, q, lane, spw, barid); }
        {
          const float sca = bc[64 + lane], scg = EPI == 3 ? bc[192 + lane] : 0.f;
          __syncwarp();
          bc[256 + lane] = sca * s1a * invR; bc[288 + lane] = sca * s2a * invR;
          if (EPI == 3) { bc[320 + lane] = scg * s1g * invR; bc[352 + lane] = scg * s2g * invR; }
          __syncwarp();
        }
#pragma unroll
        for (int k = 0; k < 32; k += 4) {
          float c1[4], c2[4], c3[4];
          bc4(bc + 64 + k, c1); bc4(bc + 256 + k, c2); bc4(bc + 288 + k, c3);
#pragma unroll
          for (int j = 0; j < 4; ++j) dy[k + j] = fmaf(c1[j], dy[k + j], -fmaf(xa[k + j], c3[j], c2[j]));
        }
        hwrite_y(stg, dy, nullptr, p.dp_hi, p.dp_lo, mq, M, p.dp_ld, ch, lane);
        if (EPI == 3) {
#pragma unroll
          for (int k = 0; k < 32; k += 4) {
            float c1[4], c2[4], c3[4];
            bc4(bc + 192 + k, c1); bc4(bc + 320 + k, c2); bc4(bc + 352 + k, c3);
#pragma unroll
            for (int j = 0; j < 4; ++j) dg[k + j] = fmaf(c1[j], dg[k + j], -fmaf(xg[k + j], c3[j], c2[j]));
          }
          hwrite_y(stg, dg, nullptr, p.dp_hi, p.dp_lo, mq, M, p.dp_ld, C + ch, lane);
        }
      }
    }
  }
}

enum { MMA_BF16 = 0, MMA_BF16X3 = 1, MMA_E4M3_CROSS = 2, MMA_F16 = 3, MMA_F16_CROSS = 4 };

template <int BN, int KIND, int TN, class Cfg>
__device__ __forceinline__ void consume_stages(float (&d)[BN / 2], int nkb, int& stage, uint32_t& phase, int& prev,
                                               uint64_t* full_bar, uint64_t* empty_bar, uint32_t smem_base, int wg, int lane) {
  for (int kb = 0; kb < nkb; ++kb) {
    mbar_wait(&full_bar[stage], phase);
    fence_proxy_async();
    const uint32_t sA = smem_base + stage * Cfg::STAGE + wg * 8192;
    const uint32_t sB = smem_base + stage * Cfg::STAGE + Cfg::PLANES * Cfg::A_PLANE;
    fence_acc(d);
    wgmma_fence();
    if constexpr (TN == 0) {
      if constexpr (KIND == MMA_E4M3_CROSS) {
#pragma unroll
        for (int k = 0; k < 2; ++k) {
          wgmma_e4m3<BN>(d, make_desc(sA + k * 32, 16, 1024), make_desc64(sB + Cfg::B_PLANE / 2 + k * 32), 1);
          wgmma_e4m3<BN>(d, make_desc(sA + 64 + k * 32, 16, 1024), make_desc64(sB + k * 32), 1);
        }
      } else if constexpr (KIND == MMA_F16) {
#pragma unroll
        for (int k = 0; k < 4; ++k)
          wgmma_f16<BN, 0, 0>(d, make_desc(sA + k * 32, 16, 1024), make_desc(sB + k * 32, 16, 1024), 1);
      } else {
#pragma unroll
        for (int k = 0; k < 4; ++k) {
          const uint64_t a_hi = make_desc(sA + k * 32, 16, 1024), b_hi = make_desc(sB + k * 32, 16, 1024);
          wgmma_bf16<BN, 0, 0>(d, a_hi, b_hi, 1);
          if constexpr (KIND == MMA_BF16X3) {
            const uint64_t a_lo = make_desc(sA + Cfg::A_PLANE + k * 32, 16, 1024), b_lo = make_desc(sB + Cfg::B_PLANE + k * 32, 16, 1024);
            wgmma_bf16<BN, 0, 0>(d, a_hi, b_lo, 1);
            wgmma_bf16<BN, 0, 0>(d, a_lo, b_hi, 1);
          }
        }
      }
    } else {
#pragma unroll
      for (int k = 0; k < 4; ++k) {
        const uint64_t a0 = make_desc(sA + k * 2048, 8192, 1024), b0 = make_desc(sB + k * 2048, 8192, 1024);
        const uint64_t a1 = make_desc(sA + Cfg::A_PLANE + k * 2048, 8192, 1024), b1 = make_desc(sB + Cfg::B_PLANE + k * 2048, 8192, 1024);
        if constexpr (KIND == MMA_F16_CROSS) {
          wgmma_f16<BN, 1, 1>(d, a0, b1, 1);
          wgmma_f16<BN, 1, 1>(d, a1, b0, 1);
        } else if constexpr (KIND == MMA_F16) {
          wgmma_f16<BN, 1, 1>(d, a0, b0, 1);
        } else {
          wgmma_bf16<BN, 1, 1>(d, a0, b0, 1);
          if constexpr (KIND == MMA_BF16X3) {
            wgmma_bf16<BN, 1, 1>(d, a0, b1, 1);
            wgmma_bf16<BN, 1, 1>(d, a1, b0, 1);
          }
        }
      }
    }
    wgmma_commit();
    wgmma_wait<1>();
    fence_acc(d);
    if (prev >= 0 && lane == 0) mbar_arrive(&empty_bar[prev]);
    prev = stage;
    if (++stage == Cfg::STAGES) { stage = 0; phase ^= 1; }
  }
}
template <int N>
__device__ __forceinline__ void rescale_acc(float (&d)[N], float scale) {
  wgmma_wait<0>();
  fence_acc(d);
#pragma unroll
  for (int i = 0; i < N; ++i) d[i] *= scale;
}

template <int BN>
__device__ __forceinline__ void nt_store_fragments(const TcNTParams& p, const float (&d)[BN / 2], const long long M, const int HW,
                                                   const long long m0, const int n0, const int r, const int c) {
  const GatherGeom& g = p.g;
  float* rowp[2];
#pragma unroll
  for (int h = 0; h < 2; ++h) {
    const long long m = m0 + r + 8 * h;
    rowp[h] = nullptr;
    if (m < M && p.dst) {
      int b = (int)(m / HW); int rem = (int)(m - (long long)b * HW);
      int y = rem / g.Wx; int x = rem - y * g.Wx;
      rowp[h] = p.dst + ((long long)(b * g.Hd + y * g.dsy + g.doy) * g.Wd + x * g.dsx + g.dox) * p.d_ld;
    }
  }
  const bool vec = (p.d_ld & 1) == 0;
#pragma unroll
  for (int j = 0; j < BN / 8; ++j) {
    const int cb = j >> 2;
    const int n = (p.perm == 2 ? (cb >> 2) * p.Cc + ((cb >> 1) & 1) * (p.Cc >> 1) + (n0 >> 2) + (cb & 1) * 32
                   : p.perm    ? ((cb < 4) ? (n0 >> 1) + cb * 32 : p.Cc + (n0 >> 1) + (cb - 4) * 32) : n0 + cb * 32) + ((8 * j) & 31) + c;
    if (n >= p.N) continue;
    float2 bb = make_float2(0.f, 0.f);
    if (p.bias) bb = *reinterpret_cast<const float2*>(p.bias + n0 + 8 * j + c);
#pragma unroll
    for (int h = 0; h < 2; ++h) {
      float* rp = rowp[h];
      if (rp == nullptr) continue;
      float v0 = d[4 * j + 2 * h], v1 = d[4 * j + 2 * h + 1];
      if (p.bias) { v0 += bb.x; v1 += bb.y; }
      if (vec && n + 2 <= p.N) {
        if (p.accumulate)
          asm volatile("red.global.add.v2.f32 [%0], {%1, %2};" ::"l"(rp + n), "f"(v0), "f"(v1) : "memory");
        else
          *reinterpret_cast<float2*>(rp + n) = make_float2(v0, v1);
      } else {
        if (p.accumulate) atomicAdd(rp + n, v0); else rp[n] = v0;
        if (n + 1 < p.N) { if (p.accumulate) atomicAdd(rp + n + 1, v1); else rp[n + 1] = v1; }
      }
    }
  }
}

constexpr int kNTThreads = 384;

template <int BN, int NPL, int EPI, bool PK = false>
__global__ void __launch_bounds__(kNTThreads, 1)
tc_gg_nt_kernel(const __grid_constant__ TcNTParams p) {
  static_assert(!PK || EPI == 0, "packed rows never take the fused epilogues (they need whole equal-length samples per tile)");
  using Cfg = NTCfg<BN, NPL>;
  __shared__ float epi_xch[2][4][32];
  __shared__ __align__(16) float epi_bc[8][(EPI == 3 || EPI == 4) ? 384 : 128];
  __shared__ __align__(16) float epi_stage[8][32 * 16];
  __shared__ float* epi_rowp[8][32];
  constexpr int S = Cfg::STAGES;
  extern __shared__ uint8_t smem_raw[];
  __shared__ __align__(8) uint64_t full_bar[S], empty_bar[S], acc_free_bar;

  const uint32_t smem_base = (smem_u32(smem_raw) + 1023u) & ~1023u;
  const int warp = threadIdx.x >> 5, lane = threadIdx.x & 31;
  const GatherGeom& g = p.g;
  const long long M = (long long)g.B * g.Hy * g.Wx;
  const int HW = g.Hy * g.Wx;
  const int cchunks = p.C >> 6;
  const int kb_pass = g.ntaps * cchunks;
  const int num_kb = NPL == 3 ? 2 * kb_pass : kb_pass;
  const int m_tiles = (int)((M + 127) / 128);
  const int n_tiles = p.n_tiles;
  const int num_tiles = m_tiles * n_tiles;

  if (threadIdx.x == 0) {
    for (int s = 0; s < S; ++s) { mbar_init(&full_bar[s], kProducerThreads + 1); mbar_init(&empty_bar[s], 8); }
    mbar_init(&acc_free_bar, 8);
    fence_barrier_init();
    tma_prefetch_desc(&p.tm_b_hi);
    if (NPL == 2) tma_prefetch_desc(&p.tm_b_lo);
    if (NPL == 3) { tma_prefetch_desc(&p.tm_b8_hi); tma_prefetch_desc(&p.tm_b8_lo); }
  }
  __syncthreads();

  if (warp < 4) {
    const int t = threadIdx.x;
    const int chunk = t & 7, rsub = t >> 3;
    int stage = 0; uint32_t phase = 0;
    int it = 0;
    for (int tile = blockIdx.x; tile < num_tiles; tile += gridDim.x, ++it) {
      const long long m0 = (long long)(tile % m_tiles) * 128;
      const int n0 = (tile / m_tiles) * BN;
      if (EPI != 0 && it > 0) mbar_wait(&acc_free_bar, (uint32_t)(it - 1) & 1u);
      int rb[8], ry[8], rx[8];
#pragma unroll
      for (int i = 0; i < 8; ++i) {
        long long m = m0 + rsub + 16 * i;
        if (m < M) {
          if constexpr (PK) {
            const int dout = p.pk.div * g.sx;
            const int u = pack_find(p.pk.off, p.pk.n, m * dout);
            const long long o0 = __ldg(p.pk.off + u), o1 = __ldg(p.pk.off + u + 1);
            rb[i] = (int)(o0 / p.pk.div); ry[i] = (int)((o1 - o0) / p.pk.div); rx[i] = (int)(m - o0 / dout) * g.sx;
          } else {
            int b = (int)(m / HW); int rem = (int)(m - (long long)b * HW);
            int y = rem / g.Wx; int x = rem - y * g.Wx;
            rb[i] = b; ry[i] = y * g.sy; rx[i] = x * g.sx;
          }
        } else { rb[i] = -1; ry[i] = 0; rx[i] = 0; }
      }
      for (int pass = 0; pass < (NPL == 3 ? 2 : 1); ++pass)
      for (int tap = 0; tap < g.ntaps; ++tap) {
        long long aoff[8];
#pragma unroll
        for (int i = 0; i < 8; ++i) {
          const int cofs = NPL == 3 && pass == 0 ? (chunk & 3) * 16 : chunk * 8;
          if constexpr (PK) {
            const int xx = rx[i] + g.ox[tap];
            aoff[i] = rb[i] >= 0 && xx >= 0 && xx < ry[i] ? (long long)(rb[i] + xx) * p.a_ld + cofs : -1;
          } else {
            int yy = ry[i] + g.oy[tap], xx = rx[i] + g.ox[tap];
            bool ok = rb[i] >= 0 && yy >= 0 && yy < g.Hs && xx >= 0 && xx < g.Ws;
            aoff[i] = ok ? ((long long)(rb[i] * g.Hs + yy) * g.Ws + xx) * p.a_ld + cofs : -1;
          }
        }
        for (int cc = 0; cc < cchunks; ++cc) {
          const int c0 = cc << 6;
          mbar_wait(&empty_bar[stage], phase ^ 1);
          const uint32_t sA = smem_base + stage * Cfg::STAGE;
          const uint32_t sB = sA + Cfg::PLANES * Cfg::A_PLANE;
          if (t == 0) {
            mbar_expect_tx(&full_bar[stage], Cfg::PLANES * Cfg::B_PLANE);
            if (NPL == 3) {
              if (pass == 0) {
                tma_load3(sB, &p.tm_b8_hi, c0, n0, g.widx[tap], &full_bar[stage]);
                tma_load3(sB + Cfg::B_PLANE / 2, &p.tm_b8_lo, c0, n0, g.widx[tap], &full_bar[stage]);
              } else {
                tma_load3(sB, &p.tm_b_hi, c0, n0, g.widx[tap], &full_bar[stage]);
              }
            } else {
              tma_load3(sB, &p.tm_b_hi, c0, n0, g.widx[tap], &full_bar[stage]);
              if (NPL == 2) tma_load3(sB + Cfg::B_PLANE, &p.tm_b_lo, c0, n0, g.widx[tap], &full_bar[stage]);
            }
          }
          if (!(p.debug & 4)) {
#pragma unroll
            for (int i = 0; i < 8; ++i) {
              const int r = rsub + 16 * i;
              const uint32_t so = sw128(r, chunk);
              const bool ok = aoff[i] >= 0;
              const long long off = ok ? aoff[i] + c0 : 0;
              if (NPL == 3) {
                if (pass == 0)
                  cp_async16(sA + so, (chunk < 4 ? p.a8_hi : p.a8_lo) + off, ok ? 16u : 0u);
                else
                  cp_async16(sA + so, p.a_hi + off, ok ? 16u : 0u);
              } else {
                cp_async16(sA + so, p.a_hi + off, ok ? 16u : 0u);
                if (NPL == 2) cp_async16(sA + Cfg::A_PLANE + so, p.a_lo + off, ok ? 16u : 0u);
              }
            }
          }
          cp_async_arrive_noinc(&full_bar[stage]);
          if (++stage == S) { stage = 0; phase ^= 1; }
        }
      }
    }
  } else {
    const int cw = warp - 4;
    const int wg = cw >> 2;
    const int tw = threadIdx.x - 128 * (wg + 1);
    float* acc_s = reinterpret_cast<float*>(smem_raw + (smem_base - smem_u32(smem_raw)));
    int stage = 0; uint32_t phase = 0;
    for (int tile = blockIdx.x; tile < num_tiles; tile += gridDim.x) {
      const long long m0 = (long long)(tile % m_tiles) * 128;
      const int n0 = (tile / m_tiles) * BN;
      float d[BN / 2];
#pragma unroll
      for (int i = 0; i < BN / 2; ++i) d[i] = 0.f;
      int prev = -1;
      if constexpr (NPL == 3) {
        consume_stages<BN, MMA_E4M3_CROSS, 0, Cfg>(d, kb_pass, stage, phase, prev, full_bar, empty_bar, smem_base, wg, lane);
        rescale_acc(d, 1.f / (float)(1 << CGVC_Q_ACC_SHIFT));
        consume_stages<BN, MMA_F16, 0, Cfg>(d, kb_pass, stage, phase, prev, full_bar, empty_bar, smem_base, wg, lane);
      } else {
        consume_stages<BN, NPL == 2 ? MMA_BF16X3 : MMA_BF16, 0, Cfg>(d, num_kb, stage, phase, prev, full_bar, empty_bar, smem_base, wg, lane);
      }
      wgmma_wait<0>();
      fence_acc(d);
      if (lane == 0) mbar_arrive(&empty_bar[prev]);
      const int r0 = wg * 64 + (tw >> 5) * 16 + ((tw & 31) >> 2), c0 = 2 * (tw & 3);
      if constexpr (EPI == 0) {
        if (!(p.debug & 3)) nt_store_fragments<BN>(p, d, M, HW, m0, n0, r0, c0);
      } else {
        consumer_bar();
        if (!(p.debug & 2)) {
#pragma unroll
          for (int j = 0; j < BN / 8; ++j) {
            *reinterpret_cast<float2*>(acc_s + acc_off<BN>(r0, 8 * j + c0)) = make_float2(d[4 * j], d[4 * j + 1]);
            *reinterpret_cast<float2*>(acc_s + acc_off<BN>(r0 + 8, 8 * j + c0)) = make_float2(d[4 * j + 2], d[4 * j + 3]);
          }
        }
        consumer_bar();
        nt_tile_epilogue<BN, NPL, EPI>(p, M, HW, m0, n0, cw & 3, lane, epi_stage[cw], epi_rowp[cw], epi_bc[cw], epi_xch[wg], acc_s, wg, 2);
        fence_proxy_async();
        __syncwarp();
        if (lane == 0) mbar_arrive(&acc_free_bar);
      }
    }
  }
}

#define CGVC_Q_WGRAD_SHIFT 12
template <int NPL, int W16>
struct TNCfg {
  static constexpr int A_PLANE = 64 * 256;
  static constexpr int B_PLANE = 64 * 512;
  static constexpr int PLANES = (NPL == 1 || W16) ? 1 : 2;
  static constexpr int STAGE = PLANES * (A_PLANE + B_PLANE);
  static constexpr int STAGES = (192 * 1024) / STAGE;
  static constexpr int SMEM = STAGES * STAGE + 1024;
};

template <int NPL, int W16>
__global__ void __launch_bounds__(kNTThreads, 1)
tc_gg_tn_kernel(const __grid_constant__ TcTNParams p) {
  static_assert(W16 == 0 || NPL == 3, "the fp16-only weight gradient is a form of CGVC_PREC_F16F8");
  using Cfg = TNCfg<NPL, W16>;
  constexpr int S = Cfg::STAGES;
  constexpr int BN = 256;
  extern __shared__ uint8_t smem_raw[];
  __shared__ __align__(8) uint64_t full_bar[S], empty_bar[S];

  const uint32_t smem_base = (smem_u32(smem_raw) + 1023u) & ~1023u;
  const int warp = threadIdx.x >> 5, lane = threadIdx.x & 31;
  const GatherGeom& g = p.g;
  const long long M = (long long)g.B * g.Hy * g.Wx;
  const int HW = g.Hy * g.Wx;
  const int n_tiles = (p.g_ld + BN - 1) / BN, c_tiles = (p.x_ld + 127) / 128;
  const int num_items = n_tiles * c_tiles * g.ntaps * p.ksplit;
  constexpr int pass0 = (NPL == 3 && !W16) ? 0 : 1;
  long long chunk_rows = (M + p.ksplit - 1) / p.ksplit;
  chunk_rows = (chunk_rows + 63) / 64 * 64;

  struct Item { int n0, c0, tap; long long mbeg, mend; int num_kb; };
  auto decode = [&](int item) -> Item {
    Item w;
    int n_t = item % n_tiles; int t1 = item / n_tiles;
    int c_t = t1 % c_tiles; int t2 = t1 / c_tiles;
    w.tap = t2 % g.ntaps; int ks = t2 / g.ntaps;
    w.n0 = n_t * BN; w.c0 = c_t * 128;
    w.mbeg = (long long)ks * chunk_rows;
    w.mend = (w.mbeg + chunk_rows < M) ? w.mbeg + chunk_rows : M;
    w.num_kb = w.mend > w.mbeg ? (int)((w.mend - w.mbeg + 63) / 64) : 0;
    return w;
  };

  if (threadIdx.x == 0) {
    for (int s = 0; s < S; ++s) { mbar_init(&full_bar[s], kProducerThreads + 1); mbar_init(&empty_bar[s], 8); }
    fence_barrier_init();
    tma_prefetch_desc(&p.tm_g_hi);
    if (NPL == 2) tma_prefetch_desc(&p.tm_g_lo);
  }
  __syncthreads();

  if (warp < 4) {
    const int t = threadIdx.x;
    const int chunk = t & 7, rsub = t >> 3;
    int stage = 0; uint32_t phase = 0;
    for (int item = blockIdx.x; item < num_items; item += gridDim.x) {
      const Item w = decode(item);
      for (int pass = pass0; pass < 2; ++pass)
      for (int kb = 0; kb < w.num_kb; ++kb) {
        mbar_wait(&empty_bar[stage], phase ^ 1);
        const uint32_t sA = smem_base + stage * Cfg::STAGE;
        const uint32_t sB = sA + Cfg::PLANES * Cfg::A_PLANE;
        long long xoff[4];
#pragma unroll
        for (int i = 0; i < 4; ++i) {
          const long long m = w.mbeg + (long long)kb * 64 + rsub + 16 * i;
          xoff[i] = -1;
          if (m < w.mend) {
            const uint32_t mu = (uint32_t)m;
            int b = (int)fdiv(mu, p.div_hw); int rem = (int)(mu - (uint32_t)b * (uint32_t)HW);
            int y = (int)fdiv((uint32_t)rem, p.div_w); int x = rem - y * g.Wx;
            int yy = y * g.sy + g.oy[w.tap], xx = x * g.sx + g.ox[w.tap];
            if (yy >= 0 && yy < g.Hs && xx >= 0 && xx < g.Ws)
              xoff[i] = ((long long)(b * g.Hs + yy) * g.Ws + xx) * p.x_ld + w.c0 + chunk * 8;
          }
        }
        if (NPL == 3 && pass == 0) {
#pragma unroll
          for (int i = 0; i < 4; ++i) {
            const int kr = rsub + 16 * i;
            const uint32_t so = sw128(kr, chunk);
#pragma unroll
            for (int a = 0; a < 2; ++a) {
              const bool ok = xoff[i] >= 0 && (w.c0 + a * 64) < p.x_ld;
              uint2 vh = make_uint2(0u, 0u), vl = make_uint2(0u, 0u);
              if (ok) { vh = __ldg(reinterpret_cast<const uint2*>(p.x8_hi + xoff[i] + a * 64)); vl = __ldg(reinterpret_cast<const uint2*>(p.x8_lo + xoff[i] + a * 64)); }
              st_shared16(sA + a * 8192 + so, e4m3x8_to_f16x8(vh));
              st_shared16(sA + Cfg::A_PLANE + a * 8192 + so, e4m3x8_to_f16x8(vl));
            }
            const long long m = w.mbeg + (long long)kb * 64 + kr;
#pragma unroll
            for (int a = 0; a < 4; ++a) {
              const int col = w.n0 + a * 64 + chunk * 8;
              const bool ok = m < w.mend && col < p.g_ld;
              uint2 vh = make_uint2(0u, 0u), vl = make_uint2(0u, 0u);
              if (ok) { vh = __ldg(reinterpret_cast<const uint2*>(p.g8_hi + m * p.g_ld + col)); vl = __ldg(reinterpret_cast<const uint2*>(p.g8_lo + m * p.g_ld + col)); }
              st_shared16(sB + a * 8192 + so, e4m3x8_to_f16x8(vh));
              st_shared16(sB + Cfg::B_PLANE + a * 8192 + so, e4m3x8_to_f16x8(vl));
            }
          }
          fence_proxy_async();
          if (t == 0) mbar_expect_tx(&full_bar[stage], 0);
          mbar_arrive(&full_bar[stage]);
        } else {
          if (t == 0) {
            const int row0 = (int)(w.mbeg + (long long)kb * 64);
            int natoms = 0;
#pragma unroll
            for (int a = 0; a < 4; ++a) natoms += (w.n0 + a * 64) < p.g_ld ? 1 : 0;
            mbar_expect_tx(&full_bar[stage], (NPL == 2 ? 2 : 1) * natoms * 8192);
#pragma unroll
            for (int a = 0; a < 4; ++a) {
              if ((w.n0 + a * 64) < p.g_ld) {
                tma_load3(sB + a * 8192, &p.tm_g_hi, w.n0 + a * 64, row0, 0, &full_bar[stage]);
                if (NPL == 2) tma_load3(sB + Cfg::B_PLANE + a * 8192, &p.tm_g_lo, w.n0 + a * 64, row0, 0, &full_bar[stage]);
              }
            }
          }
#pragma unroll
          for (int i = 0; i < 4; ++i) {
            const uint32_t so = sw128(rsub + 16 * i, chunk);
#pragma unroll
            for (int a = 0; a < 2; ++a) {
              const bool ok = xoff[i] >= 0 && (w.c0 + a * 64) < p.x_ld;
              const long long off = ok ? xoff[i] + a * 64 : 0;
              cp_async16(sA + a * 8192 + so, p.x_hi + off, ok ? 16u : 0u);
              if (NPL == 2) cp_async16(sA + Cfg::A_PLANE + a * 8192 + so, p.x_lo + off, ok ? 16u : 0u);
            }
          }
          cp_async_arrive_noinc(&full_bar[stage]);
        }
        if (++stage == S) { stage = 0; phase ^= 1; }
      }
    }
  } else {
    const int cw = warp - 4;
    const int wg = cw >> 2;
    const int tw = threadIdx.x - 128 * (wg + 1);
    int stage = 0; uint32_t phase = 0;
    for (int item = blockIdx.x; item < num_items; item += gridDim.x) {
      const Item w = decode(item);
      if (w.num_kb == 0) continue;
      float d[BN / 2];
#pragma unroll
      for (int i = 0; i < BN / 2; ++i) d[i] = 0.f;
      int prev = -1;
      if constexpr (NPL == 3 && !W16) {
        consume_stages<BN, MMA_F16_CROSS, 1, Cfg>(d, w.num_kb, stage, phase, prev, full_bar, empty_bar, smem_base, wg, lane);
        rescale_acc(d, 1.f / (float)(1 << CGVC_Q_WGRAD_SHIFT));
        consume_stages<BN, MMA_F16, 1, Cfg>(d, w.num_kb, stage, phase, prev, full_bar, empty_bar, smem_base, wg, lane);
      } else if constexpr (NPL == 3) {
        consume_stages<BN, MMA_F16, 1, Cfg>(d, w.num_kb, stage, phase, prev, full_bar, empty_bar, smem_base, wg, lane);
      } else {
        consume_stages<BN, NPL == 2 ? MMA_BF16X3 : MMA_BF16, 1, Cfg>(d, w.num_kb, stage, phase, prev, full_bar, empty_bar, smem_base, wg, lane);
      }
      wgmma_wait<0>();
      fence_acc(d);
      if (lane == 0) mbar_arrive(&empty_bar[prev]);
      const int c = w.c0 + wg * 64 + (tw >> 5) * 16 + ((tw & 31) >> 2);
#pragma unroll
      for (int j = 0; j < BN / 8; ++j) {
        const int n = w.n0 + 8 * j + 2 * (tw & 3);
        if (n >= p.N) continue;
        float* base; int nn; int ncols;
        if (n < p.n_split) { base = p.dw_a; nn = n; ncols = p.n_split; } else { base = p.dw_g; nn = n - p.n_split; ncols = p.N - p.n_split; }
#pragma unroll
        for (int h = 0; h < 2; ++h) {
          if (c + 8 * h >= p.C) continue;
          float* dst = tn_dst(base, g.widx[w.tap], p.C, c + 8 * h, ncols, nn, p.fold_n);
          asm volatile("red.global.add.v2.f32 [%0], {%1, %2};" ::"l"(dst), "f"(d[4 * j + 2 * h]), "f"(d[4 * j + 2 * h + 1]) : "memory");
        }
      }
    }
  }
}

__host__ __device__ __forceinline__ int perm_row(int perm, int co, int cout, int noff) {
  if (perm == 1) return (co >> 7) * 256 + (noff ? 128 : 0) + (co & 127);
  if (perm == 2) { const int Ch = cout >> 1; const int s = co >= Ch ? 1 : 0; const int c = co - s * Ch; return (c >> 6) * 256 + (noff ? 128 : 0) + s * 64 + (c & 63); }
  return noff + co;
}
__host__ __device__ __forceinline__ long long w_src(int tap, int ci, int co, int cin, int cout, int fold_n) {
  if (fold_n) { const int t = co / fold_n; return ((long long)t * cin + ci) * fold_n + (co - t * fold_n); }
  return ((long long)tap * cin + ci) * cout + co;
}
__global__ void __launch_bounds__(256)
prep_weights_kernel(const float* __restrict__ w, int taps, int cin, int cout, int nt_n, int cin_k, int cin_n, int nt_k, int noff, int perm, int fold_n,
                    __nv_bfloat16* __restrict__ wf_hi, __nv_bfloat16* __restrict__ wf_lo,
                    __nv_bfloat16* __restrict__ wd_hi, __nv_bfloat16* __restrict__ wd_lo) {
  __shared__ float tile[32][33];
  const int tap = blockIdx.z;
  const int ci0 = blockIdx.y * 32, co0 = blockIdx.x * 32;
  const int tx = threadIdx.x & 31, ty = threadIdx.x >> 5;
  for (int r = ty; r < 32; r += 8) {
    int ci = ci0 + r, co = co0 + tx;
    float v = 0.f;
    if (ci < cin && co < cout) {
      v = w[w_src(tap, ci, co, cin, cout, fold_n)];
      __nv_bfloat16 h = __float2bfloat16_rn(v);
      __nv_bfloat16 l = __float2bfloat16_rn(v - __bfloat162float(h));
      long long o = ((long long)tap * cin_n + ci) * nt_k + noff + co;
      wd_hi[o] = h; wd_lo[o] = l;
    }
    tile[r][tx] = v;
  }
  __syncthreads();
  for (int r = ty; r < 32; r += 8) {
    int co = co0 + r, ci = ci0 + tx;
    if (ci < cin && co < cout) {
      float v = tile[tx][r];
      __nv_bfloat16 h = __float2bfloat16_rn(v);
      __nv_bfloat16 l = __float2bfloat16_rn(v - __bfloat162float(h));
      const int nrow = perm_row(perm, co, cout, noff);
      long long o = ((long long)tap * nt_n + nrow) * cin_k + ci;
      wf_hi[o] = h; wf_lo[o] = l;
    }
  }
}

__global__ void copy_bias_kernel(const float* __restrict__ b, float* __restrict__ dst, int n, int noff, int perm) {
  int i = blockIdx.x * 256 + threadIdx.x;
  if (i < n) dst[perm_row(perm, i, n, noff)] = b[i];
}

__global__ void __launch_bounds__(256)
prep_weights_q_kernel(const float* __restrict__ w, int taps, int cin, int cout, int nt_n, int cin_q, int noff, int perm, int fold_n,
                      __half* __restrict__ q16, uint8_t* __restrict__ q8hi, uint8_t* __restrict__ q8lo) {
  const int cq = cin / 4;
  const long long total = (long long)taps * cout * cq;
  for (long long i = (long long)blockIdx.x * 256 + threadIdx.x; i < total; i += (long long)gridDim.x * 256) {
    const int c4 = (int)(i % cq); long long r = i / cq;
    const int co = (int)(r % cout); const int tap = (int)(r / cout);
    const int ci = c4 * 4;
    float v[4];
#pragma unroll
    for (int k = 0; k < 4; ++k) v[k] = w[w_src(tap, ci + k, co, cin, cout, fold_n)];
    const int nrow = perm_row(perm, co, cout, noff);
    const long long o = ((long long)tap * nt_n + nrow) * cin_q + ci;
    uint2 hh; uint32_t b_hi, b_lo;
    cgvc_quant4(v, CGVC_Q_W_SHI, CGVC_Q_W_SLO, hh, b_hi, b_lo);
    *reinterpret_cast<uint2*>(q16 + o) = hh;
    *reinterpret_cast<uint32_t*>(q8hi + o) = b_hi;
    *reinterpret_cast<uint32_t*>(q8lo + o) = b_lo;
  }
}

__global__ void __launch_bounds__(256)
prep_weights_qd_kernel(const float* __restrict__ w, int taps, int cin, int cout, int cin_n, int nt_q, int noff, int fold_n,
                       __half* __restrict__ q16, uint8_t* __restrict__ q8hi, uint8_t* __restrict__ q8lo) {
  const int cq = cout / 4;
  const long long total = (long long)taps * cin * cq;
  for (long long i = (long long)blockIdx.x * 256 + threadIdx.x; i < total; i += (long long)gridDim.x * 256) {
    const int c4 = (int)(i % cq); long long r = i / cq;
    const int ci = (int)(r % cin); const int tap = (int)(r / cin);
    const float4 v4 = *reinterpret_cast<const float4*>(w + w_src(tap, ci, c4 * 4, cin, cout, fold_n));
    const float v[4] = {v4.x, v4.y, v4.z, v4.w};
    const long long o = ((long long)tap * cin_n + ci) * nt_q + noff + c4 * 4;
    uint2 hh; uint32_t b_hi, b_lo;
    cgvc_quant4(v, CGVC_Q_W_SHI, CGVC_Q_W_SLO, hh, b_hi, b_lo);
    *reinterpret_cast<uint2*>(q16 + o) = hh;
    *reinterpret_cast<uint32_t*>(q8hi + o) = b_hi;
    *reinterpret_cast<uint32_t*>(q8lo + o) = b_lo;
  }
}

struct PrepJob {
  long long w_off, b_off;
  int taps, cin, cout, nt_n, cin_q, cin_n, nt_q, noff, perm, fold_n;
  __half* q16; uint8_t *q8hi, *q8lo;
  __half* dq16; uint8_t *dq8hi, *dq8lo;
  float* bias;
  int tiles_ci, tiles_co;
  int first_block;
};

__global__ void __launch_bounds__(256)
prep_weights_q_all_kernel(const float* __restrict__ params, const PrepJob* __restrict__ jobs, int j0, int j1, int block0) {
  __shared__ float tile[32][65];
  const int blk = (int)blockIdx.x + block0;
  int lo = j0, hi = j1 - 1;
  while (lo < hi) { const int mid = (lo + hi + 1) >> 1; if (jobs[mid].first_block <= blk) lo = mid; else hi = mid - 1; }
  const PrepJob& J = jobs[lo];
  int r = blk - J.first_block;
  const int tco = r % J.tiles_co; r /= J.tiles_co;
  const int tci = r % J.tiles_ci; const int tap = r / J.tiles_ci;
  const int ci0 = tci * 32, co0 = tco * 64;
  const float* __restrict__ w = params + J.w_off;
  const int t = threadIdx.x;
  {
    const int c4 = (t & 15) * 4;
    for (int rr = t >> 4; rr < 32; rr += 16) {
      const int ci = ci0 + rr, co = co0 + c4;
      float v[4] = {0.f, 0.f, 0.f, 0.f};
      if (ci < J.cin && co < J.cout) {
        const float4 q = *reinterpret_cast<const float4*>(w + w_src(tap, ci, co, J.cin, J.cout, J.fold_n));
        v[0] = q.x; v[1] = q.y; v[2] = q.z; v[3] = q.w;
        if (J.dq16) {
          const long long o = ((long long)tap * J.cin_n + ci) * J.nt_q + J.noff + co;
          uint2 hh; uint32_t b_hi, b_lo;
          cgvc_quant4(v, CGVC_Q_W_SHI, CGVC_Q_W_SLO, hh, b_hi, b_lo);
          *reinterpret_cast<uint2*>(J.dq16 + o) = hh;
          *reinterpret_cast<uint32_t*>(J.dq8hi + o) = b_hi;
          *reinterpret_cast<uint32_t*>(J.dq8lo + o) = b_lo;
        }
      }
      tile[rr][c4] = v[0]; tile[rr][c4 + 1] = v[1]; tile[rr][c4 + 2] = v[2]; tile[rr][c4 + 3] = v[3];
    }
  }
  __syncthreads();
  {
    const int lane = t & 31, warp = t >> 5;
    const int cig = (lane & 3) * 8;
    const int col = warp * 8 + (lane >> 2);
    const int co = co0 + col;
    if (co < J.cout && ci0 + cig < J.cin_q) {
      float va[4], vb[4];
#pragma unroll
      for (int k = 0; k < 4; ++k) { va[k] = tile[cig + k][col]; vb[k] = tile[cig + 4 + k][col]; }
      const int nrow = perm_row(J.perm, co, J.cout, J.noff);
      const long long o = ((long long)tap * J.nt_n + nrow) * J.cin_q + ci0 + cig;
      uint2 ha, hb; uint32_t a_hi, a_lo, b_hi, b_lo;
      cgvc_quant4(va, CGVC_Q_W_SHI, CGVC_Q_W_SLO, ha, a_hi, a_lo);
      cgvc_quant4(vb, CGVC_Q_W_SHI, CGVC_Q_W_SLO, hb, b_hi, b_lo);
      *reinterpret_cast<uint4*>(J.q16 + o) = make_uint4(ha.x, ha.y, hb.x, hb.y);
      *reinterpret_cast<uint2*>(J.q8hi + o) = make_uint2(a_hi, b_hi);
      *reinterpret_cast<uint2*>(J.q8lo + o) = make_uint2(a_lo, b_lo);
    }
  }
  if (tap == 0 && tci == 0 && tco == 0 && J.b_off >= 0)
    for (int i = t; i < J.cout; i += 256) J.bias[perm_row(J.perm, i, J.cout, J.noff)] = params[J.b_off + i];
}

template <class K>
cudaError_t set_smem(K kernel, int bytes) {
  static std::vector<const void*> done;
  const void* key = (const void*)kernel;
  for (const void* d : done) if (d == key) return cudaSuccess;
  cudaError_t e = cudaFuncSetAttribute(kernel, cudaFuncAttributeMaxDynamicSharedMemorySize, bytes);
  if (e == cudaSuccess) done.push_back(key);
  return e;
}

struct ProfRec { cudaEvent_t a, b; double flops; int cls; long long M; int N, K; };
int g_tc_debug = 0;
int g_tc_prep_batched = 1;
bool g_prof_on = false;
std::vector<ProfRec> g_prof;
void prof_begin(cudaStream_t st, double flops, int cls, long long M = 0, int N = 0, int K = 0) {
  if (!g_prof_on) return;
  ProfRec r; r.flops = flops; r.cls = cls; r.M = M; r.N = N; r.K = K;
  cudaEventCreate(&r.a); cudaEventCreate(&r.b);
  cudaEventRecord(r.a, st);
  g_prof.push_back(r);
}
void prof_end(cudaStream_t st) { if (g_prof_on && !g_prof.empty()) cudaEventRecord(g_prof.back().b, st); }

inline int tile_rows(int n_real, int n_padded) { return (n_padded % 256 == 0) ? 256 : (n_real <= 32 ? 32 : 128); }

int num_sms() {
  static int n = 0;
  if (!n) { int dev = 0; cudaGetDevice(&dev); cudaDeviceGetAttribute(&n, cudaDevAttrMultiProcessorCount, dev); }
  return n;
}

cudaError_t launch_nt(TcNTParams p, int precision, cudaStream_t st, int epi) {
  const long long M = (long long)p.g.B * p.g.Hy * p.g.Wx;
  if (M == 0) return cudaSuccess;
  const bool x3 = precision == 1;
  if (p.g.ntaps == 0) return cudaErrorInvalidValue;
  const int bn = tile_rows(p.N, p.Nw);
  p.n_tiles = bn == 32 ? 1 : p.Nw / bn;
  const long long tiles = ((M + 127) / 128) * p.n_tiles;
  dim3 grid((unsigned)(tiles < num_sms() ? tiles : num_sms()));
  cudaError_t e;
  ++g_cgvc_launches;
  p.debug = g_tc_debug;
  prof_begin(st, 2.0 * (double)M * p.N * p.g.ntaps * p.C, (epi == 1 || epi == 2 || epi == 5) ? 2 : 0, M, p.N, p.g.ntaps * p.C);
#define LAUNCH_NT(BN_, NPL_, EPI_, ...)                                                                        \
  do {                                                                                                         \
    e = set_smem(tc_gg_nt_kernel<BN_, NPL_, EPI_, ##__VA_ARGS__>, NTCfg<BN_, NPL_>::SMEM);                     \
    if (e != cudaSuccess) return e;                                                                            \
    tc_gg_nt_kernel<BN_, NPL_, EPI_, ##__VA_ARGS__><<<grid, kNTThreads, NTCfg<BN_, NPL_>::SMEM, st>>>(p);      \
  } while (0)
  if (epi != 0 && bn != 256) return cudaErrorInvalidValue;
  if (p.pk.off) {
    if (epi != 0 || p.g.B != 1 || p.g.Hy != 1) return cudaErrorInvalidValue;
    const int npl = precision == 3 ? 3 : x3 ? 2 : 1;
    if (bn == 256)      { if (npl == 3) LAUNCH_NT(256, 3, 0, true); else if (npl == 2) LAUNCH_NT(256, 2, 0, true); else LAUNCH_NT(256, 1, 0, true); }
    else if (bn == 128) { if (npl == 3) LAUNCH_NT(128, 3, 0, true); else if (npl == 2) LAUNCH_NT(128, 2, 0, true); else LAUNCH_NT(128, 1, 0, true); }
    else                { if (npl == 3) LAUNCH_NT(32, 3, 0, true);  else if (npl == 2) LAUNCH_NT(32, 2, 0, true);  else LAUNCH_NT(32, 1, 0, true); }
  }
  else if (precision == 3) {
    if (epi == 1)       LAUNCH_NT(256, 3, 1);
    else if (epi == 2)  LAUNCH_NT(256, 3, 2);
    else if (epi == 5)  LAUNCH_NT(256, 3, 5);
    else if (epi != 0)  return cudaErrorInvalidValue;
    else if (bn == 256) LAUNCH_NT(256, 3, 0);
    else if (bn == 128) LAUNCH_NT(128, 3, 0);
    else                LAUNCH_NT(32, 3, 0);
  }
  else if (epi == 1)  { if (x3) LAUNCH_NT(256, 2, 1); else LAUNCH_NT(256, 1, 1); }
  else if (epi == 2)  { if (x3) LAUNCH_NT(256, 2, 2); else LAUNCH_NT(256, 1, 2); }
  else if (epi == 3)  { if (x3) LAUNCH_NT(256, 2, 3); else LAUNCH_NT(256, 1, 3); }
  else if (epi == 4)  { if (x3) LAUNCH_NT(256, 2, 4); else LAUNCH_NT(256, 1, 4); }
  else if (epi == 5)  { if (x3) LAUNCH_NT(256, 2, 5); else LAUNCH_NT(256, 1, 5); }
  else if (bn == 256) { if (x3) LAUNCH_NT(256, 2, 0); else LAUNCH_NT(256, 1, 0); }
  else if (bn == 128) { if (x3) LAUNCH_NT(128, 2, 0); else LAUNCH_NT(128, 1, 0); }
  else                { if (x3) LAUNCH_NT(32, 2, 0);  else LAUNCH_NT(32, 1, 0); }
#undef LAUNCH_NT
  prof_end(st);
  return cudaGetLastError();
}

cudaError_t launch_tn(TcTNParams p, int precision, cudaStream_t st) {
  const long long M = (long long)p.g.B * p.g.Hy * p.g.Wx;
  if (M == 0) return cudaSuccess;
  if (M >= (1ll << 31)) return cudaErrorInvalidValue;
  const int tiles = ((p.g_ld + 255) / 256) * ((p.x_ld + 127) / 128) * p.g.ntaps;
  const int nsm = num_sms();
  long long maxsplit = M / 1024; if (maxsplit < 1) maxsplit = 1; if (maxsplit > 32) maxsplit = 32;
  int ksplit = 1; double best = 0.0;
  for (int ks = 1; ks <= (int)maxsplit; ++ks) {
    long long items = (long long)tiles * ks;
    double eff = (double)items / (double)(((items + nsm - 1) / nsm) * nsm);
    if (items < nsm) eff *= 0.5;
    if (eff > best + 0.02) { best = eff; ksplit = ks; }
  }
  p.ksplit = ksplit;
  p.div_hw = make_fastdiv((uint32_t)(p.g.Hy * p.g.Wx)); p.div_w = make_fastdiv((uint32_t)p.g.Wx);
  const long long items = (long long)tiles * ksplit;
  dim3 grid((unsigned)(items < nsm ? items : nsm));
  cudaError_t e;
  ++g_cgvc_launches;
  prof_begin(st, 2.0 * (double)M * p.N * p.g.ntaps * p.C, 1, M, p.N, p.g.ntaps * p.C);
#define LAUNCH_TN(NPL_, W16_)                                                                     \
  do {                                                                                            \
    e = set_smem(tc_gg_tn_kernel<NPL_, W16_>, TNCfg<NPL_, W16_>::SMEM);                           \
    if (e != cudaSuccess) return e;                                                               \
    tc_gg_tn_kernel<NPL_, W16_><<<grid, kNTThreads, TNCfg<NPL_, W16_>::SMEM, st>>>(p);            \
  } while (0)
  if (precision == 3) { if (p.w16) LAUNCH_TN(3, 1); else LAUNCH_TN(3, 0); }
  else if (precision == 1) LAUNCH_TN(2, 0);
  else                     LAUNCH_TN(1, 0);
#undef LAUNCH_TN
  prof_end(st);
  return cudaGetLastError();
}

inline int ru(int v, int m) { return (v + m - 1) / m * m; }
inline int Ntot(const TcLayer& L) { return L.cout * (L.gated ? 2 : 1); }
inline int cin_k(const TcLayer& L) { return ru(L.cin, 64); }
inline int cin_n(const TcLayer& L) { return ru(L.cin, 128); }
inline int nt_k(const TcLayer& L) { return ru(Ntot(L), 64); }
inline int nt_n(const TcLayer& L) { return ru(Ntot(L), 128); }
inline int cin_q(const TcLayer& L) { return ru(L.cin, 128); }
inline int nt_q(const TcLayer& L) { return ru(Ntot(L), 128); }
inline size_t wq_elems(const TcLayer& L) { return (size_t)L.kh * L.kw * nt_n(L) * cin_q(L); }
inline size_t wdq_elems(const TcLayer& L) { return (size_t)L.kh * L.kw * cin_n(L) * nt_q(L); }
inline size_t wf_elems(const TcLayer& L) { return (size_t)L.kh * L.kw * nt_n(L) * cin_k(L); }
inline size_t wd_elems(const TcLayer& L) { return (size_t)L.kh * L.kw * cin_n(L) * nt_k(L); }
inline int layer_perm(const TcLayer& L) {
  if (L.gated && L.shuffle == 2 && L.cout % 128 == 0) return 2;
  return (L.gated && L.cout % 128 == 0) ? 1 : 0;
}
inline bool layer_ok(const TcLayer& L) {
  if (L.fold && (L.gated || L.kh * L.kw != 1 || L.cout % L.fold || (L.cout / L.fold) % 4)) return false;
  return L.kh * L.kw <= CGVC_MAX_TAPS && Ntot(L) % 4 == 0;
}
inline bool layer_ok_q(const TcLayer& L) { return layer_ok(L) && L.cin % 4 == 0; }


bool make_layer_maps(TcLayer& L) {
  const int taps = L.kh * L.kw;
  const int bf = tile_rows(Ntot(L), nt_n(L)), bd = tile_rows(L.cin, cin_n(L));
  return make_tmap3(&L.tm_f_hi, L.wf_hi, cin_k(L), nt_n(L), taps, bf) &&
         make_tmap3(&L.tm_f_lo, L.wf_lo, cin_k(L), nt_n(L), taps, bf) &&
         make_tmap3(&L.tm_d_hi, L.wd_hi, nt_k(L), cin_n(L), taps, bd) &&
         make_tmap3(&L.tm_d_lo, L.wd_lo, nt_k(L), cin_n(L), taps, bd);
}

bool make_layer_maps_q(TcLayer& L) {
  const int taps = L.kh * L.kw;
  const int bf = tile_rows(Ntot(L), nt_n(L)), bd = tile_rows(L.cin, cin_n(L));
  const CUtensorMapDataType F16 = CU_TENSOR_MAP_DATA_TYPE_FLOAT16, U8 = CU_TENSOR_MAP_DATA_TYPE_UINT8;
  bool ok = make_tmap3_t(&L.tm_q16, L.wq16, F16, 2, cin_q(L), nt_n(L), taps, 64, bf) &&
            make_tmap3_t(&L.tm_q8hi, L.wq8hi, U8, 1, cin_q(L), nt_n(L), taps, 64, bf) &&
            make_tmap3_t(&L.tm_q8lo, L.wq8lo, U8, 1, cin_q(L), nt_n(L), taps, 64, bf);
  if (ok && L.wdq16)
    ok = make_tmap3_t(&L.tm_dq16, L.wdq16, F16, 2, nt_q(L), cin_n(L), taps, 64, bd) &&
         make_tmap3_t(&L.tm_dq8hi, L.wdq8hi, U8, 1, nt_q(L), cin_n(L), taps, 64, bd) &&
         make_tmap3_t(&L.tm_dq8lo, L.wdq8lo, U8, 1, nt_q(L), cin_n(L), taps, 64, bd);
  return ok;
}


int refresh_layer(TcLayer& L, const float* ka, const float* kg, const float* ba, const float* bg, cudaStream_t st) {
  const int taps = L.kh * L.kw;
  dim3 grid((L.cout + 31) / 32, (L.cin + 31) / 32, taps);
  g_cgvc_launches += L.gated ? 4 : 2;
  const int perm = layer_perm(L);
  const int fn = L.fold ? L.cout / L.fold : 0;
  if (!L.wq16) prep_weights_kernel<<<grid, 256, 0, st>>>(ka, taps, L.cin, L.cout, nt_n(L), cin_k(L), cin_n(L), nt_k(L), 0, perm, fn, L.wf_hi, L.wf_lo, L.wd_hi, L.wd_lo);
  if (!L.fold) copy_bias_kernel<<<(L.cout + 255) / 256, 256, 0, st>>>(ba, L.bias, L.cout, 0, perm);
  if (L.gated) {
    if (!L.wq16) prep_weights_kernel<<<grid, 256, 0, st>>>(kg, taps, L.cin, L.cout, nt_n(L), cin_k(L), cin_n(L), nt_k(L), L.cout, perm, fn, L.wf_hi, L.wf_lo, L.wd_hi, L.wd_lo);
    copy_bias_kernel<<<(L.cout + 255) / 256, 256, 0, st>>>(bg, L.bias, L.cout, L.cout, perm);
  }
  if (L.wq16) {
    long long tot = (long long)taps * L.cout * (L.cin / 4); long long nb = (tot + 255) / 256; if (nb > num_sms() * 32) nb = num_sms() * 32;
    g_cgvc_launches += L.gated ? 2 : 1;
    prep_weights_q_kernel<<<(unsigned)nb, 256, 0, st>>>(ka, taps, L.cin, L.cout, nt_n(L), cin_q(L), 0, perm, fn, (__half*)L.wq16, L.wq8hi, L.wq8lo);
    if (L.gated) prep_weights_q_kernel<<<(unsigned)nb, 256, 0, st>>>(kg, taps, L.cin, L.cout, nt_n(L), cin_q(L), L.cout, perm, fn, (__half*)L.wq16, L.wq8hi, L.wq8lo);
    if (L.wdq16) {
      g_cgvc_launches += L.gated ? 2 : 1;
      prep_weights_qd_kernel<<<(unsigned)nb, 256, 0, st>>>(ka, taps, L.cin, L.cout, cin_n(L), nt_q(L), 0, fn, (__half*)L.wdq16, L.wdq8hi, L.wdq8lo);
      if (L.gated) prep_weights_qd_kernel<<<(unsigned)nb, 256, 0, st>>>(kg, taps, L.cin, L.cout, cin_n(L), nt_q(L), L.cout, fn, (__half*)L.wdq16, L.wdq8hi, L.wdq8lo);
    }
  }
  return (int)cudaGetLastError();
}

int layer_fwd(const TcLayer& L, int precision, const __nv_bfloat16* xhi, const __nv_bfloat16* xlo, int n, int H, int W, int sh, int sw,
              float* P, cudaStream_t st, const TcFuse* fuse = nullptr, bool* fused_out = nullptr, const PackGeom* pk = nullptr) {
  if (!layer_ok(L) || (precision == 3 && !layer_ok_q(L))) return TC_UNSUPPORTED;
  if (pk && (n != 1 || H != 1 || L.kh != 1 || fuse)) return (int)cudaErrorInvalidValue;
  TcNTParams p; memset(&p, 0, sizeof p);
  p.g = fwd_geom(n, H, W, L.kh, L.kw, sh, sw);
  if (pk) p.pk = *pk;
  p.a_hi = xhi; p.a_lo = xlo; p.a_ld = cin_k(L); p.C = cin_k(L);
  p.b_hi = L.wf_hi; p.b_lo = L.wf_lo; p.Nw = nt_n(L); p.N = Ntot(L);
  p.dst = P; p.d_ld = Ntot(L); p.bias = L.bias; p.accumulate = 0;
  p.perm = layer_perm(L); p.Cc = L.cout;
  p.tm_b_hi = L.tm_f_hi; p.tm_b_lo = L.tm_f_lo;
  if (precision == 3) {
    if (!L.wq16) return TC_UNSUPPORTED;
    p.a_ld = cin_q(L); p.C = cin_q(L); p.a_lo = nullptr;
    p.a8_hi = reinterpret_cast<const uint8_t*>(xlo); p.a8_lo = p.a8_hi + (size_t)n * H * W * cin_q(L);
    p.tm_b_hi = L.tm_q16; p.tm_b8_hi = L.tm_q8hi; p.tm_b8_lo = L.tm_q8lo;
  }
  int epi = 0;
  if (fuse && fuse->R > 0) {
    const bool shape_ok = H == 1 && (fuse->R == 32 || fuse->R == 64 || fuse->R == 128) && p.g.Wx == fuse->R && nt_n(L) % 256 == 0 && Ntot(L) == nt_n(L);
    if (shape_ok && L.gated && p.perm == 1) epi = 1; else if (shape_ok && L.gated && p.perm == 2) epi = 5; else if (shape_ok && !L.gated) epi = 2;
    if (epi) {
      p.R = fuse->R; p.gamma_a = fuse->gamma_a; p.beta_a = fuse->beta_a; p.gamma_g = fuse->gamma_g; p.beta_g = fuse->beta_g;
      p.stats = fuse->stats; p.resid = fuse->resid; p.y = fuse->y; p.y_hi = fuse->y_hi; p.y_lo = fuse->y_lo;
      p.y8 = reinterpret_cast<uint8_t*>(fuse->y_lo);
      p.C_out = epi == 5 ? L.cout / 2 : (L.gated ? L.cout : Ntot(L));
      if (!p.y_hi || (epi == 2 && !p.resid)) epi = 0;
    }
  }
  if (fused_out) *fused_out = epi != 0;
  if (!epi && !P) return (int)cudaErrorInvalidValue;
  return (int)launch_nt(p, precision, st, epi);
}

int layer_dgrad(const TcLayer& L, int precision, const __nv_bfloat16* dPhi, const __nv_bfloat16* dPlo, int n, int H, int W, int sh, int sw,
                float* dx, int accumulate, cudaStream_t st, const TcBwdFuse* fuse = nullptr, bool* fused_out = nullptr) {
  if (fused_out) *fused_out = false;
  if (!layer_ok(L) || (precision == 3 && (!layer_ok_q(L) || !L.wdq16))) return TC_UNSUPPORTED;
  std::vector<GatherGeom> gs = dgrad_geoms(n, H, W, L.kh, L.kw, sh, sw);
  for (const GatherGeom& g : gs) if (g.ntaps == 0) return TC_UNSUPPORTED;
  int epi = 0;
  if (fuse && fuse->R > 0 && gs.size() == 1 && H == 1 && sh == 1 && sw == 1 && (fuse->R == 32 || fuse->R == 64 || fuse->R == 128) &&
      gs[0].Wx == fuse->R && cin_n(L) % 256 == 0 && L.cin == cin_n(L) && fuse->bp && fuse->stats && fuse->dp_hi && fuse->dp_lo && fuse->gamma_a &&
      (fuse->gated ? (fuse->gamma_g && fuse->beta_a && fuse->beta_g) : (dx != nullptr)) && precision != 3)
    epi = fuse->gated ? 3 : 4;
  for (const GatherGeom& g : gs) {
    TcNTParams p; memset(&p, 0, sizeof p);
    p.g = g;
    p.a_hi = dPhi; p.a_lo = dPlo; p.a_ld = nt_k(L); p.C = nt_k(L);
    p.b_hi = L.wd_hi; p.b_lo = L.wd_lo; p.Nw = cin_n(L); p.N = L.cin;
    p.dst = dx; p.d_ld = L.cin; p.bias = nullptr; p.accumulate = accumulate;
    p.tm_b_hi = L.tm_d_hi; p.tm_b_lo = L.tm_d_lo;
    if (precision == 3) {
      p.a_ld = nt_q(L); p.C = nt_q(L); p.a_lo = nullptr;
      p.a8_hi = reinterpret_cast<const uint8_t*>(dPlo); p.a8_lo = p.a8_hi + (size_t)g.B * g.Hs * g.Ws * nt_q(L);
      p.tm_b_hi = L.tm_dq16; p.tm_b8_hi = L.tm_dq8hi; p.tm_b8_lo = L.tm_dq8lo;
    }
    if (epi) {
      p.R = fuse->R; p.C_out = L.cin; p.stats = const_cast<float*>(fuse->stats);
      p.gamma_a = fuse->gamma_a; p.beta_a = fuse->beta_a; p.gamma_g = fuse->gamma_g; p.beta_g = fuse->beta_g;
      p.bp = fuse->bp; p.bp_ld = fuse->bp_ld; p.dp_hi = fuse->dp_hi; p.dp_lo = fuse->dp_lo; p.dp_ld = fuse->dp_ld;
      p.dbeta_a = fuse->dbeta_a; p.dgamma_a = fuse->dgamma_a; p.dbeta_g = fuse->dbeta_g; p.dgamma_g = fuse->dgamma_g;
    }
    cudaError_t e = launch_nt(p, precision, st, epi);
    if (e != cudaSuccess) return (int)e;
  }
  if (fused_out) *fused_out = epi != 0;
  return 0;
}

int layer_wgrad(const TcLayer& L, int precision, const __nv_bfloat16* xhi, const __nv_bfloat16* xlo,
                const __nv_bfloat16* dPhi, const __nv_bfloat16* dPlo, int n, int H, int W, int sh, int sw,
                float* dwa, float* dwg, cudaStream_t st, int w16 = 0) {
  if (!layer_ok(L) || (precision == 3 && !layer_ok_q(L))) return TC_UNSUPPORTED;
  TcTNParams p; memset(&p, 0, sizeof p);
  p.w16 = (precision == 3 && w16) ? 1 : 0;
  p.fold_n = L.fold ? L.cout / L.fold : 0;
  p.g = fwd_geom(n, H, W, L.kh, L.kw, sh, sw);
  p.x_hi = xhi; p.x_lo = xlo; p.x_ld = cin_k(L); p.C = L.cin;
  p.g_hi = dPhi; p.g_lo = dPlo; p.g_ld = nt_k(L); p.N = Ntot(L);
  p.dw_a = dwa; p.dw_g = dwg; p.n_split = L.cout;
  const long long M = (long long)p.g.B * p.g.Hy * p.g.Wx;
  if (precision == 3) {
    const long long rows_in = (long long)n * H * W;
    p.x_ld = cin_q(L); p.g_ld = nt_q(L); p.x_lo = p.g_lo = nullptr;
    p.x8_hi = reinterpret_cast<const uint8_t*>(xlo); p.x8_lo = p.x8_hi + rows_in * p.x_ld;
    p.g8_hi = reinterpret_cast<const uint8_t*>(dPlo); p.g8_lo = p.g8_hi + M * p.g_ld;
    if (!make_tmap3_t(&p.tm_g_hi, dPhi, CU_TENSOR_MAP_DATA_TYPE_FLOAT16, 2, (uint64_t)p.g_ld, (uint64_t)M, 1, 64, 64))
      return (int)cudaErrorInvalidValue;
  } else if (!make_tmap3(&p.tm_g_hi, dPhi, (uint64_t)nt_k(L), (uint64_t)M, 1, 64) || !make_tmap3(&p.tm_g_lo, dPlo, (uint64_t)nt_k(L), (uint64_t)M, 1, 64)) {
    return (int)cudaErrorInvalidValue;
  }
  return (int)launch_tn(p, precision, st);
}

}

int tc_register(TcWeights& w, size_t ka, size_t kg, size_t ba, size_t bg, int kh, int kw, int cin, int cout, int gated, int shuffle, int fold) {
  TcLayer L{}; L.ka = ka; L.kg = kg; L.ba = ba; L.bg = bg; L.kh = kh; L.kw = kw; L.cin = cin; L.cout = cout; L.gated = gated; L.shuffle = shuffle; L.fold = fold;
  w.layers.push_back(L);
  return (int)w.layers.size() - 1;
}

static cudaError_t tc_init_kernels();

int tc_alloc(TcWeights& w, int precision, bool train) {
  { cudaError_t ie = tc_init_kernels(); if (ie != cudaSuccess) return (int)ie; }
  w.precision = precision;
  w.quant = precision == 3;
  w.quant_bwd = w.quant && train;
  w.wgrad16 = w.quant;
  size_t total = 0;
  auto rnd = [](size_t b) { return (b + 255) & ~(size_t)255; };
  for (TcLayer& L : w.layers) {
    total += 2 * rnd(wf_elems(L) * sizeof(__nv_bfloat16)) + 2 * rnd(wd_elems(L) * sizeof(__nv_bfloat16)) + rnd((size_t)nt_n(L) * sizeof(float));
    if (w.quant && layer_ok_q(L)) total += rnd(wq_elems(L) * 2) + 2 * rnd(wq_elems(L));
    if (w.quant && w.quant_bwd && layer_ok_q(L)) total += rnd(wdq_elems(L) * 2) + 2 * rnd(wdq_elems(L));
  }
  cudaError_t err = cudaMalloc(&w.pool, total);
  if (err != cudaSuccess) return (int)err;
  err = cudaMemset(w.pool, 0, total);
  if (err != cudaSuccess) return (int)err;
  w.pool_bytes = total;
  char* p = (char*)w.pool;
  for (TcLayer& L : w.layers) {
    size_t ef = rnd(wf_elems(L) * sizeof(__nv_bfloat16)), ed = rnd(wd_elems(L) * sizeof(__nv_bfloat16));
    L.wf_hi = (__nv_bfloat16*)p; p += ef; L.wf_lo = (__nv_bfloat16*)p; p += ef;
    L.wd_hi = (__nv_bfloat16*)p; p += ed; L.wd_lo = (__nv_bfloat16*)p; p += ed;
    L.bias = (float*)p; p += rnd((size_t)nt_n(L) * sizeof(float));
    if (!make_layer_maps(L)) return (int)cudaErrorInvalidValue;
    L.wq16 = nullptr; L.wq8hi = L.wq8lo = nullptr; L.wdq16 = nullptr; L.wdq8hi = L.wdq8lo = nullptr;
    if (w.quant && layer_ok_q(L)) {
      L.wq16 = p; p += rnd(wq_elems(L) * 2);
      L.wq8hi = (uint8_t*)p; p += rnd(wq_elems(L)); L.wq8lo = (uint8_t*)p; p += rnd(wq_elems(L));
      if (w.quant_bwd) {
        L.wdq16 = p; p += rnd(wdq_elems(L) * 2);
        L.wdq8hi = (uint8_t*)p; p += rnd(wdq_elems(L)); L.wdq8lo = (uint8_t*)p; p += rnd(wdq_elems(L));
      }
      if (!make_layer_maps_q(L)) return (int)cudaErrorInvalidValue;
    }
  }
  w.job_first.clear(); w.job_ka.clear();
  if (w.quant) {
    std::vector<PrepJob> jobs;
    int blocks = 0;
    for (TcLayer& L : w.layers) {
      if (!L.wq16) continue;
      for (int br = 0; br < (L.gated ? 2 : 1); ++br) {
        PrepJob J; memset(&J, 0, sizeof J);
        J.w_off = (long long)(br ? L.kg : L.ka); J.b_off = L.fold ? -1 : (long long)(br ? L.bg : L.ba);
        J.taps = L.kh * L.kw; J.cin = L.cin; J.cout = L.cout; J.nt_n = nt_n(L); J.cin_q = cin_q(L); J.cin_n = cin_n(L); J.nt_q = nt_q(L);
        J.noff = br ? L.cout : 0; J.perm = layer_perm(L); J.fold_n = L.fold ? L.cout / L.fold : 0;
        J.q16 = (__half*)L.wq16; J.q8hi = L.wq8hi; J.q8lo = L.wq8lo;
        J.dq16 = (__half*)L.wdq16; J.dq8hi = L.wdq8hi; J.dq8lo = L.wdq8lo;
        J.bias = L.bias;
        J.tiles_ci = (L.cin + 31) / 32; J.tiles_co = (L.cout + 63) / 64;
        J.first_block = blocks;
        blocks += J.taps * J.tiles_ci * J.tiles_co;
        jobs.push_back(J); w.job_first.push_back(J.first_block); w.job_ka.push_back(L.ka);
      }
    }
    w.job_first.push_back(blocks);
    if (!jobs.empty()) {
      err = cudaMalloc(&w.prep_jobs, jobs.size() * sizeof(PrepJob));
      if (err != cudaSuccess) return (int)err;
      err = cudaMemcpy(w.prep_jobs, jobs.data(), jobs.size() * sizeof(PrepJob), cudaMemcpyHostToDevice);
      if (err != cudaSuccess) return (int)err;
    }
  }
  w.ready = false;
  return 0;
}

static cudaError_t tc_init_kernels() {
  cudaError_t e;
#define INIT_NT(BN_, NPL_, EPI_) if ((e = set_smem(tc_gg_nt_kernel<BN_, NPL_, EPI_>, NTCfg<BN_, NPL_>::SMEM)) != cudaSuccess) return e;
  INIT_NT(256, 2, 0) INIT_NT(256, 1, 0) INIT_NT(128, 2, 0) INIT_NT(128, 1, 0) INIT_NT(32, 2, 0) INIT_NT(32, 1, 0)
  INIT_NT(256, 2, 1) INIT_NT(256, 1, 1) INIT_NT(256, 2, 2) INIT_NT(256, 1, 2)
  INIT_NT(256, 2, 3) INIT_NT(256, 1, 3) INIT_NT(256, 2, 4) INIT_NT(256, 1, 4) INIT_NT(256, 2, 5) INIT_NT(256, 1, 5)
  INIT_NT(256, 3, 0) INIT_NT(128, 3, 0) INIT_NT(32, 3, 0) INIT_NT(256, 3, 1) INIT_NT(256, 3, 2) INIT_NT(256, 3, 5)
#undef INIT_NT
#define INIT_NT_PK(BN_, NPL_) if ((e = set_smem(tc_gg_nt_kernel<BN_, NPL_, 0, true>, NTCfg<BN_, NPL_>::SMEM)) != cudaSuccess) return e;
  INIT_NT_PK(256, 1) INIT_NT_PK(256, 2) INIT_NT_PK(256, 3) INIT_NT_PK(128, 1) INIT_NT_PK(128, 2) INIT_NT_PK(128, 3)
  INIT_NT_PK(32, 1) INIT_NT_PK(32, 2) INIT_NT_PK(32, 3)
#undef INIT_NT_PK
#define INIT_TN(NPL_, W16_) if ((e = set_smem(tc_gg_tn_kernel<NPL_, W16_>, TNCfg<NPL_, W16_>::SMEM)) != cudaSuccess) return e;
  INIT_TN(3, 1) INIT_TN(3, 0) INIT_TN(2, 0) INIT_TN(1, 0)
#undef INIT_TN
  return cudaSuccess;
}

void tc_free(TcWeights& w) {
  if (w.pool) cudaFree(w.pool);
  if (w.prep_jobs) cudaFree(w.prep_jobs);
  w.pool = nullptr; w.prep_jobs = nullptr; w.ready = false;
}

static int refresh_jobs(TcWeights& w, const float* params, int j0, int j1, cudaStream_t st) {
  if (j1 <= j0) return 0;
  const int b0 = w.job_first[j0], nb = w.job_first[j1] - b0;
  ++g_cgvc_launches;
  prep_weights_q_all_kernel<<<(unsigned)nb, 256, 0, st>>>(params, (const PrepJob*)w.prep_jobs, j0, j1, b0);
  return (int)cudaGetLastError();
}

int tc_refresh_weights(TcWeights& w, const float* params, cudaStream_t st) {
  if (!w.pool) return 0;
  const bool batched = g_tc_prep_batched && w.prep_jobs;
  for (TcLayer& L : w.layers) {
    if (batched && L.wq16) continue;
    int r = refresh_layer(L, params + L.ka, params + L.kg, params + L.ba, params + L.bg, st);
    if (r != 0) return r;
  }
  if (batched) { int r = refresh_jobs(w, params, 0, (int)w.job_ka.size(), st); if (r != 0) return r; }
  w.ready = true;
  return 0;
}

int tc_refresh_weights_range(TcWeights& w, const float* params, size_t begin, size_t end, cudaStream_t st) {
  if (!w.pool) return 0;
  const bool batched = g_tc_prep_batched && w.prep_jobs;
  for (TcLayer& L : w.layers) {
    if (L.ka < begin || L.ka >= end) continue;
    if (batched && L.wq16) continue;
    int r = refresh_layer(L, params + L.ka, params + L.kg, params + L.ba, params + L.bg, st);
    if (r != 0) return r;
  }
  if (batched) {
    const int nj = (int)w.job_ka.size();
    int j = 0;
    while (j < nj) {
      if (w.job_ka[j] < begin || w.job_ka[j] >= end) { ++j; continue; }
      int k = j; while (k < nj && w.job_ka[k] >= begin && w.job_ka[k] < end) ++k;
      int r = refresh_jobs(w, params, j, k, st); if (r != 0) return r;
      j = k;
    }
  }
  return 0;
}

void tc_set_prep_batched(int v) { g_tc_prep_batched = v != 0; }

cudaError_t tc_split_planes(int precision, const float* x, long long rows, int C, __nv_bfloat16* hi, __nv_bfloat16* lo, cudaStream_t st,
                            unsigned long long* sat) {
  return precision == 3 ? launch_pad_split_q(x, rows, C, C, ru(C, 128), hi, lo, st, sat) : launch_pad_split(x, rows, C, C, ru(C, 64), hi, lo, st);
}

int tc_conv_fwd(TcWeights& w, int slot, const __nv_bfloat16* xhi, const __nv_bfloat16* xlo, int n, int H, int W, int sh, int sw,
                float* P, cudaStream_t st, const TcFuse* fuse, bool* fused, const PackGeom* pk) {
  return layer_fwd(w.layers[slot], w.precision, xhi, xlo, n, H, W, sh, sw, P, st, fuse, fused, pk);
}

int tc_conv_dgrad(TcWeights& w, int slot, const __nv_bfloat16* dPhi, const __nv_bfloat16* dPlo, int n, int H, int W, int sh, int sw,
                  float* dx, int accumulate, cudaStream_t st, const TcBwdFuse* fuse, bool* fused) {
  return layer_dgrad(w.layers[slot], w.precision, dPhi, dPlo, n, H, W, sh, sw, dx, accumulate, st, fuse, fused);
}

int tc_conv_wgrad(TcWeights& w, int slot, const __nv_bfloat16* xhi, const __nv_bfloat16* xlo,
                  const __nv_bfloat16* dPhi, const __nv_bfloat16* dPlo, int n, int H, int W, int sh, int sw,
                  float* dwa, float* dwg, cudaStream_t st) {
  return layer_wgrad(w.layers[slot], w.precision, xhi, xlo, dPhi, dPlo, n, H, W, sh, sw, dwa, dwg, st, w.wgrad16 ? 1 : 0);
}

bool tc_profile_is_on() { return g_prof_on; }

void tc_profile_enable(int on) {
  for (ProfRec& r : g_prof) { cudaEventDestroy(r.a); cudaEventDestroy(r.b); }
  g_prof.clear();
  g_prof_on = on != 0;
}

int tc_profile_collect(double ms[3], double flops[3], long long launches[3]) {
  cudaError_t e = cudaDeviceSynchronize();
  if (e != cudaSuccess) return (int)e;
  for (int c = 0; c < 3; ++c) { ms[c] = 0; flops[c] = 0; launches[c] = 0; }
  for (ProfRec& r : g_prof) {
    float t = 0.f;
    if (cudaEventElapsedTime(&t, r.a, r.b) != cudaSuccess) continue;
    ms[r.cls] += t; flops[r.cls] += r.flops; launches[r.cls] += 1;
  }
  return 0;
}

int tc_profile_launches(double* ms, double* flops, long long* meta4, int capacity, int* n_out) {
  cudaError_t e = cudaDeviceSynchronize();
  if (e != cudaSuccess) return (int)e;
  int n = 0;
  for (ProfRec& r : g_prof) {
    float t = 0.f;
    if (cudaEventElapsedTime(&t, r.a, r.b) != cudaSuccess) continue;
    if (n < capacity) { ms[n] = t; flops[n] = r.flops; meta4[4 * n] = r.cls; meta4[4 * n + 1] = r.M; meta4[4 * n + 2] = r.N; meta4[4 * n + 3] = r.K; }
    ++n;
  }
  if (n_out) *n_out = n;
  return 0;
}
void tc_set_debug(int v) { g_tc_debug = v; }

namespace {
struct Temp {
  std::vector<void*> ptrs;
  ~Temp() { for (void* p : ptrs) cudaFree(p); }
  template <class T> T* get(size_t n) { void* p = nullptr; if (cudaMalloc(&p, n * sizeof(T) + 256) != cudaSuccess) return nullptr; ptrs.push_back(p); return (T*)p; }
};
}

static int adhoc_layer_q(Temp& T, TcLayer& L, cudaStream_t st) {
  L.wq16 = T.get<uint16_t>(wq_elems(L)); L.wq8hi = T.get<uint8_t>(wq_elems(L)); L.wq8lo = T.get<uint8_t>(wq_elems(L));
  if (!L.wq16 || !L.wq8hi || !L.wq8lo) return (int)cudaErrorMemoryAllocation;
  cudaMemsetAsync(L.wq16, 0, wq_elems(L) * 2, st); cudaMemsetAsync(L.wq8hi, 0, wq_elems(L), st); cudaMemsetAsync(L.wq8lo, 0, wq_elems(L), st);
  L.wdq16 = T.get<uint16_t>(wdq_elems(L)); L.wdq8hi = T.get<uint8_t>(wdq_elems(L)); L.wdq8lo = T.get<uint8_t>(wdq_elems(L));
  if (!L.wdq16 || !L.wdq8hi || !L.wdq8lo) return (int)cudaErrorMemoryAllocation;
  cudaMemsetAsync(L.wdq16, 0, wdq_elems(L) * 2, st); cudaMemsetAsync(L.wdq8hi, 0, wdq_elems(L), st); cudaMemsetAsync(L.wdq8lo, 0, wdq_elems(L), st);
  return make_layer_maps_q(L) ? 0 : (int)cudaErrorInvalidValue;
}

static int adhoc_layer(Temp& T, TcLayer& L, cudaStream_t st) {
  L.wf_hi = T.get<__nv_bfloat16>(wf_elems(L)); L.wf_lo = T.get<__nv_bfloat16>(wf_elems(L));
  L.wd_hi = T.get<__nv_bfloat16>(wd_elems(L)); L.wd_lo = T.get<__nv_bfloat16>(wd_elems(L));
  L.bias = T.get<float>(nt_n(L));
  if (!L.wf_hi || !L.wf_lo || !L.wd_hi || !L.wd_lo || !L.bias) return (int)cudaErrorMemoryAllocation;
  cudaMemsetAsync(L.wf_hi, 0, wf_elems(L) * 2, st); cudaMemsetAsync(L.wf_lo, 0, wf_elems(L) * 2, st);
  cudaMemsetAsync(L.wd_hi, 0, wd_elems(L) * 2, st); cudaMemsetAsync(L.wd_lo, 0, wd_elems(L) * 2, st);
  cudaMemsetAsync(L.bias, 0, nt_n(L) * sizeof(float), st);
  if (!make_layer_maps(L)) return (int)cudaErrorInvalidValue;
  return 0;
}

int tc_conv_fwd_adhoc(int precision, const float* x, const float* w, const float* bias, float* y,
                      int B, int H, int W, int Cin, int kh, int kw, int Cout, int sh, int sw, cudaStream_t st) {
  TcLayer L{}; L.kh = kh; L.kw = kw; L.cin = Cin; L.cout = Cout; L.gated = 0;
  if (!layer_ok(L) || (precision == 3 && !layer_ok_q(L))) return TC_UNSUPPORTED;
  Temp T;
  int r = adhoc_layer(T, L, st); if (r) return r;
  size_t rows = (size_t)B * H * W;
  const int cpad = precision == 3 ? cin_q(L) : cin_k(L);
  if (precision == 3) { r = adhoc_layer_q(T, L, st); if (r) return r; }
  __nv_bfloat16* xhi = T.get<__nv_bfloat16>(rows * cpad); __nv_bfloat16* xlo = T.get<__nv_bfloat16>(rows * cpad);
  float* zero = T.get<float>(Cout);
  if (!xhi || !xlo || !zero) return (int)cudaErrorMemoryAllocation;
  cudaMemsetAsync(zero, 0, Cout * sizeof(float), st);
  r = refresh_layer(L, w, nullptr, bias ? bias : zero, nullptr, st); if (r) return r;
  cudaError_t e = tc_split_planes(precision, x, (long long)rows, Cin, xhi, xlo, st);
  if (e != cudaSuccess) return (int)e;
  r = layer_fwd(L, precision, xhi, xlo, B, H, W, sh, sw, y, st); if (r) return r;
  return (int)cudaStreamSynchronize(st);
}

int tc_conv_bwd_adhoc(int precision, const float* x, const float* w, const float* dy, float* dx, float* dw, float* dbias,
                      int B, int H, int W, int Cin, int kh, int kw, int Cout, int sh, int sw, cudaStream_t st, int w16) {
  TcLayer L{}; L.kh = kh; L.kw = kw; L.cin = Cin; L.cout = Cout; L.gated = 0;
  if (!layer_ok(L) || (precision == 3 && !layer_ok_q(L))) return TC_UNSUPPORTED;
  Temp T;
  int r = adhoc_layer(T, L, st); if (r) return r;
  if (precision == 3) { r = adhoc_layer_q(T, L, st); if (r) return r; }
  GatherGeom g = fwd_geom(B, H, W, kh, kw, sh, sw);
  size_t rows = (size_t)B * H * W, orows = (size_t)g.B * g.Hy * g.Wx;
  const int xpad = precision == 3 ? cin_q(L) : cin_k(L), gpad = precision == 3 ? nt_q(L) : nt_k(L);
  __nv_bfloat16* xhi = T.get<__nv_bfloat16>(rows * xpad); __nv_bfloat16* xlo = T.get<__nv_bfloat16>(rows * xpad);
  __nv_bfloat16* ghi = T.get<__nv_bfloat16>(orows * gpad); __nv_bfloat16* glo = T.get<__nv_bfloat16>(orows * gpad);
  float* zero = T.get<float>(Cout);
  if (!xhi || !xlo || !ghi || !glo || !zero) return (int)cudaErrorMemoryAllocation;
  cudaMemsetAsync(zero, 0, Cout * sizeof(float), st);
  r = refresh_layer(L, w, nullptr, zero, nullptr, st); if (r) return r;
  cudaError_t e = tc_split_planes(precision, x, (long long)rows, Cin, xhi, xlo, st);
  if (e != cudaSuccess) return (int)e;
  e = tc_split_planes(precision, dy, (long long)orows, Cout, ghi, glo, st);
  if (e != cudaSuccess) return (int)e;
  if (dx) { r = layer_dgrad(L, precision, ghi, glo, B, H, W, sh, sw, dx, 0, st); if (r) return r; }
  if (dw) {
    r = layer_wgrad(L, precision, xhi, xlo, ghi, glo, B, H, W, sh, sw, dw, nullptr, st, w16); if (r) return r;
    if (dbias) { e = launch_colsum(dy, (long long)orows, Cout, 0, Cout, dbias, st); if (e != cudaSuccess) return (int)e; }
  }
  return (int)cudaStreamSynchronize(st);
}
```

voice-converter-cyclegan_b200/csrc/tc_gemm.cuh:

```cuda
#pragma once
#include <cuda.h>
#include <cuda_runtime.h>
#include <cuda_bf16.h>
#include <stddef.h>
#include <vector>
#include "kernels.cuh"

#define TC_UNSUPPORTED (-12345)

struct TcLayer {
  size_t ka, kg, ba, bg;
  int kh, kw, cin, cout, gated;
  int shuffle;
  int fold;
  __nv_bfloat16 *wf_hi, *wf_lo;
  __nv_bfloat16 *wd_hi, *wd_lo;
  float* bias;
  CUtensorMap tm_f_hi, tm_f_lo;
  CUtensorMap tm_d_hi, tm_d_lo;
  void* wq16; uint8_t *wq8hi, *wq8lo;
  CUtensorMap tm_q16, tm_q8hi, tm_q8lo;
  void* wdq16; uint8_t *wdq8hi, *wdq8lo;
  CUtensorMap tm_dq16, tm_dq8hi, tm_dq8lo;
};

struct TcWeights {
  std::vector<TcLayer> layers;
  void* pool = nullptr;
  size_t pool_bytes = 0;
  bool ready = false;
  int precision = 0;
  bool quant = false;
  bool wgrad16 = false;
  bool quant_bwd = false;
  void* prep_jobs = nullptr;
  std::vector<int> job_first;
  std::vector<size_t> job_ka;
};

struct TcFuse {
  int R;
  const float *gamma_a, *beta_a, *gamma_g, *beta_g;
  float* stats;
  const float* resid;
  float* y; __nv_bfloat16 *y_hi, *y_lo;
};

struct TcBwdFuse {
  int R;
  int gated;
  const float* bp; int bp_ld;
  const float* stats;
  const float *gamma_a, *beta_a, *gamma_g, *beta_g;
  __nv_bfloat16 *dp_hi, *dp_lo; int dp_ld;
  float *dbeta_a, *dgamma_a, *dbeta_g, *dgamma_g;
};

int tc_register(TcWeights& w, size_t ka, size_t kg, size_t ba, size_t bg, int kh, int kw, int cin, int cout, int gated, int shuffle = 1, int fold = 0);
int tc_alloc(TcWeights& w, int precision, bool train);
void tc_free(TcWeights& w);
int tc_refresh_weights(TcWeights& w, const float* params, cudaStream_t st);
int tc_refresh_weights_range(TcWeights& w, const float* params, size_t begin, size_t end, cudaStream_t st);

cudaError_t tc_split_planes(int precision, const float* x, long long rows, int C, __nv_bfloat16* hi, __nv_bfloat16* lo, cudaStream_t st,
                            unsigned long long* sat = nullptr);

int tc_conv_fwd(TcWeights& w, int slot, const __nv_bfloat16* xhi, const __nv_bfloat16* xlo, int n, int H, int W, int sh, int sw,
                float* P, cudaStream_t st, const TcFuse* fuse = nullptr, bool* fused = nullptr, const PackGeom* pk = nullptr);
int tc_conv_dgrad(TcWeights& w, int slot, const __nv_bfloat16* dPhi, const __nv_bfloat16* dPlo, int n, int H, int W, int sh, int sw,
                  float* dx, int accumulate, cudaStream_t st, const TcBwdFuse* fuse = nullptr, bool* fused = nullptr);
int tc_conv_wgrad(TcWeights& w, int slot, const __nv_bfloat16* xhi, const __nv_bfloat16* xlo,
                  const __nv_bfloat16* dPhi, const __nv_bfloat16* dPlo, int n, int H, int W, int sh, int sw,
                  float* dwa, float* dwg, cudaStream_t st);
int tc_conv_fwd_adhoc(int precision, const float* x, const float* w, const float* bias, float* y,
                      int B, int H, int W, int Cin, int kh, int kw, int Cout, int sh, int sw, cudaStream_t st);
int tc_conv_bwd_adhoc(int precision, const float* x, const float* w, const float* dy, float* dx, float* dw, float* dbias,
                      int B, int H, int W, int Cin, int kh, int kw, int Cout, int sh, int sw, cudaStream_t st, int w16 = 0);

void tc_profile_enable(int on);
bool tc_profile_is_on();
int tc_profile_collect(double ms[3], double flops[3], long long launches[3]);
int tc_profile_launches(double* ms, double* flops, long long* meta4, int capacity, int* n_out);
void tc_set_prep_batched(int v);
void tc_set_debug(int v);
```

Baseline: 9.492.

## Split conv gathers into boundary tap classes to skip padded-out taps

Implicit-GEMM convolutions (forward, dgrad, wgrad) now split the output rows and columns into classes whose valid-tap sets match. Each class carries only the taps that land inside the input, so zero-padded taps at image borders no longer cost MMA work. Classes are packed into the kernel parameters (up to 16 for NT, 8 for TN) with a per-tile class lookup, and wgrad uses a new 4D TMA map. It is enabled by default and adds per-tile class decode overhead, more launch parameters, and a more complex tiling that may leave partial tiles.

```diff
diff --git a/include/cgvc.h b/include/cgvc.h
--- a/include/cgvc.h
+++ b/include/cgvc.h
@@ -100,6 +100,8 @@
 int cgvc_profile_enable(int on);
 int cgvc_profile_collect(double* ms3, double* flops3, long long* launches3);
 int cgvc_profile_launches(double* ms, double* flops, long long* meta4, int capacity, int* n_out);
+#define CGVC_TAP_CLASS_INTS 68
+int cgvc_tap_classes(int dgrad, int classes, int B, int H, int W, int kh, int kw, int sh, int sw, int* out, int capacity, int* n_out);
 
 int cgvc_conv_forward(cgvc_handle h, int precision, const float* x, const float* w, const float* bias, float* y,
                       int B, int H, int W, int Cin, int kh, int kw, int Cout, int sh, int sw, void* stream);
diff --git a/voice-converter-cyclegan_b200/_native.py b/voice-converter-cyclegan_b200/_native.py
--- a/voice-converter-cyclegan_b200/_native.py
+++ b/voice-converter-cyclegan_b200/_native.py
@@ -71,6 +71,7 @@
         "cgvc_profile_enable": (ci, [ci]),
         "cgvc_profile_collect": (ci, [P(C.c_double), P(C.c_double), P(C.c_longlong)]),
         "cgvc_profile_launches": (ci, [P(C.c_double), P(C.c_double), P(C.c_longlong), ci, P(ci)]),
+        "cgvc_tap_classes": (ci, [ci] * 9 + [P(ci), ci, P(ci)]),
         "cgvc_conv_forward": (ci, [vp, ci, vp, vp, vp, vp] + [ci] * 9 + [vp]),
         "cgvc_conv_backward": (ci, [vp, ci, vp, vp, vp, vp, vp, vp] + [ci] * 9 + [vp]),
         "cgvc_in_glu_forward": (ci, [vp] * 8 + [ci] * 4 + [vp]),
diff --git a/voice-converter-cyclegan_b200/csrc/engine.cu b/voice-converter-cyclegan_b200/csrc/engine.cu
--- a/voice-converter-cyclegan_b200/csrc/engine.cu
+++ b/voice-converter-cyclegan_b200/csrc/engine.cu
@@ -1450,6 +1450,12 @@
   if (!strcmp(name, "debug_taps")) { e->debug_taps = value != 0; return 0; }
   if (!strcmp(name, "cuda_graph")) { e->use_graphs = value != 0; return 0; }
   if (!strcmp(name, "tc_debug")) { tc_set_debug(value); return 0; }
+  if (!strcmp(name, "tap_classes")) {
+    e->tcw.tap_classes = value != 0;
+    for (auto& kv : e->graphs) cudaGraphExecDestroy(kv.second.exec);
+    e->graphs.clear();
+    return 0;
+  }
   if (!strcmp(name, "post_onepass")) {
     post_set_onepass(value);
     for (auto& kv : e->graphs) cudaGraphExecDestroy(kv.second.exec);
@@ -1502,6 +1508,26 @@
   if (!ms3 || !flops3 || !launches3) return CGVC_ERR_ARG;
   return tc_profile_collect(ms3, flops3, launches3) == 0 ? 0 : CGVC_ERR_CUDA;
 }
+int cgvc_tap_classes(int dgrad, int classes, int B, int H, int W, int kh, int kw, int sh, int sw, int* out, int capacity, int* n_out) {
+  if (!out || !n_out || capacity < 0 || dgrad < 0 || dgrad > 2 || B < 1 || H < 1 || W < 1 || kh < 1 || kw < 1 || kh * kw > CGVC_MAX_TAPS || sh < 1 || sw < 1)
+    return CGVC_ERR_ARG;
+  static_assert(CGVC_TAP_CLASS_INTS == 14 + 3 * CGVC_MAX_TAPS, "record layout of include/cgvc.h");
+  std::vector<GatherGeom> gs;
+  if (dgrad == 1) gs = classes ? dgrad_classes(B, H, W, kh, kw, sh, sw) : dgrad_geoms(B, H, W, kh, kw, sh, sw);
+  else if (dgrad == 2 && classes) gs = wgrad_classes(B, H, W, kh, kw, sh, sw);
+  else gs = classes && dgrad == 0 ? fwd_classes(B, H, W, kh, kw, sh, sw) : std::vector<GatherGeom>{fwd_geom(B, H, W, kh, kw, sh, sw)};
+  *n_out = (int)gs.size();
+  for (int i = 0; i < (int)gs.size() && i < capacity; ++i) {
+    const GatherGeom& g = gs[i];
+    int* r = out + (size_t)CGVC_TAP_CLASS_INTS * i;
+    const int head[14] = {g.B, g.Hy, g.Wx, g.Hs, g.Ws, g.sy, g.sx, g.ntaps, g.Hd, g.Wd, g.dsy, g.dsx, g.doy, g.dox};
+    for (int k = 0; k < 14; ++k) r[k] = head[k];
+    for (int t = 0; t < CGVC_MAX_TAPS; ++t) {
+      r[14 + t] = g.oy[t]; r[14 + CGVC_MAX_TAPS + t] = g.ox[t]; r[14 + 2 * CGVC_MAX_TAPS + t] = g.widx[t];
+    }
+  }
+  return 0;
+}
 
 int cgvc_sample_plan(cgvc_handle e, const long long* offsets_A_dev, int n_A, const long long* offsets_B_dev, int n_B,
                      unsigned long long seed, long long epoch, int crop_frames, int* plan_dev, int* err_dev, void* stream) {
@@ -1533,7 +1559,8 @@
   DeviceGuard dguard; CK(dguard.set(e->cfg.device));
   cudaStream_t st = (cudaStream_t)stream;
   if (precision != CGVC_PREC_FP32_SIMT)
-    return tc_result(e, tc_conv_fwd_adhoc(precision, x, w, bias, y, B, H, W, Cin, kh, kw, Cout, sh, sw, st), nullptr, "conv forward");
+    return tc_result(e, tc_conv_fwd_adhoc(precision, x, w, bias, y, B, H, W, Cin, kh, kw, Cout, sh, sw, st, e->tcw.tap_classes), nullptr,
+                     "conv forward");
   GatherGeom g = fwd_geom(B, H, W, kh, kw, sh, sw);
   GemmOperands op; memset(&op, 0, sizeof op);
   op.src = x; op.s_ld = Cin; op.C = Cin; op.w = w; op.w_ts = (long long)Cin * Cout; op.w_cs = Cout; op.w_ns = 1; op.N = Cout;
@@ -1549,8 +1576,8 @@
   DeviceGuard dguard; CK(dguard.set(e->cfg.device));
   cudaStream_t st = (cudaStream_t)stream;
   if (precision != CGVC_PREC_FP32_SIMT)
-    return tc_result(e, tc_conv_bwd_adhoc(precision, x, w, dy, dx, dw, dbias, B, H, W, Cin, kh, kw, Cout, sh, sw, st, e->tcw.wgrad16 ? 1 : 0),
-                     nullptr, "conv backward");
+    return tc_result(e, tc_conv_bwd_adhoc(precision, x, w, dy, dx, dw, dbias, B, H, W, Cin, kh, kw, Cout, sh, sw, st, e->tcw.wgrad16 ? 1 : 0,
+                                          e->tcw.tap_classes), nullptr, "conv backward");
   ConvW c; c.k = 0; c.b = 0; c.kh = kh; c.kw = kw; c.cin = Cin; c.cout = Cout;
   if (dx) RET(conv_dgrad_simt(e, w, c, sh, sw, B, H, W, dy, Cout, 0, dx, 0, st));
   if (dw) {
diff --git a/voice-converter-cyclegan_b200/csrc/geom.h b/voice-converter-cyclegan_b200/csrc/geom.h
--- a/voice-converter-cyclegan_b200/csrc/geom.h
+++ b/voice-converter-cyclegan_b200/csrc/geom.h
@@ -42,3 +42,85 @@
   }
   return out;
 }
+
+#define CGVC_MAX_CLASSES 16
+
+static inline uint32_t tap_mask(const GatherGeom& g, int dim, int v) {
+  uint32_t m = 0;
+  for (int t = 0; t < g.ntaps; ++t) {
+    const int s = dim == 0 ? v * g.sy + g.oy[t] : v * g.sx + g.ox[t];
+    if (s >= 0 && s < (dim == 0 ? g.Hs : g.Ws)) m |= 1u << t;
+  }
+  return m;
+}
+
+static inline bool split_geom(const GatherGeom& g, bool split_h, bool split_w, std::vector<GatherGeom>& out) {
+  struct Run { int v0, len; uint32_t mask; };
+  std::vector<Run> rh, rw;
+  for (int dim = 0; dim < 2; ++dim) {
+    std::vector<Run>& r = dim == 0 ? rh : rw;
+    const int n = dim == 0 ? g.Hy : g.Wx;
+    const bool split = dim == 0 ? split_h : split_w;
+    for (int v = 0; v < n; ++v) {
+      const uint32_t m = split ? tap_mask(g, dim, v) : ~0u;
+      if (!r.empty() && r.back().mask == m) r.back().len++;
+      else r.push_back(Run{v, 1, m});
+    }
+  }
+  for (const Run& a : rh) for (const Run& b : rw) {
+    GatherGeom c = g;
+    c.Hy = a.len; c.Wx = b.len;
+    c.doy = g.doy + a.v0 * g.dsy; c.dox = g.dox + b.v0 * g.dsx;
+    c.ntaps = 0;
+    for (int t = 0; t < g.ntaps; ++t) {
+      if (!((a.mask & b.mask) >> t & 1u)) continue;
+      c.oy[c.ntaps] = (short)(g.oy[t] + a.v0 * g.sy); c.ox[c.ntaps] = (short)(g.ox[t] + b.v0 * g.sx); c.widx[c.ntaps] = g.widx[t];
+      c.ntaps++;
+    }
+    if (c.ntaps == 0) return false;
+    out.push_back(c);
+  }
+  return true;
+}
+
+static inline double geom_work(const std::vector<GatherGeom>& gs) {
+  double w = 0.0;
+  for (const GatherGeom& g : gs) w += (double)g.Hy * g.Wx * g.ntaps;
+  return w;
+}
+
+static inline std::vector<GatherGeom> row_classes(const std::vector<GatherGeom>& base) {
+  bool two_d = false;
+  for (const GatherGeom& g : base) two_d |= g.Hs > 1;
+  if (!two_d) return base;
+  const double full = geom_work(base);
+  auto split_all = [&](bool h, bool w, std::vector<GatherGeom>& out) {
+    out.clear();
+    for (const GatherGeom& g : base) if (!split_geom(g, h, w, out)) return false;
+    return out.size() <= CGVC_MAX_CLASSES;
+  };
+  std::vector<GatherGeom> t;
+  const bool h = split_all(true, false, t) && geom_work(t) <= 0.98 * full;
+  const bool w = split_all(false, true, t) && geom_work(t) <= 0.98 * full;
+  if (h && w && split_all(true, true, t)) return t;
+  if (h && split_all(true, false, t)) return t;
+  if (w && split_all(false, true, t)) return t;
+  return base;
+}
+
+static inline std::vector<GatherGeom> fwd_classes(int B, int H, int W, int kh, int kw, int sh, int sw) {
+  return row_classes(std::vector<GatherGeom>{fwd_geom(B, H, W, kh, kw, sh, sw)});
+}
+static inline std::vector<GatherGeom> dgrad_classes(int B, int H, int W, int kh, int kw, int sh, int sw) {
+  return row_classes(dgrad_geoms(B, H, W, kh, kw, sh, sw));
+}
+
+#define CGVC_MAX_WG_CLASSES 8
+static inline std::vector<GatherGeom> wgrad_classes(int B, int H, int W, int kh, int kw, int sh, int sw) {
+  const std::vector<GatherGeom> base{fwd_geom(B, H, W, kh, kw, sh, sw)};
+  if (base[0].Hs <= 1) return base;
+  std::vector<GatherGeom> t;
+  if (!split_geom(base[0], true, false, t) || t.size() > CGVC_MAX_WG_CLASSES || geom_work(t) > 0.98 * geom_work(base)) return base;
+  for (const GatherGeom& g : t) if (g.Hy != 1 || 64 % g.Wx != 0) return base;
+  return t;
+}
diff --git a/voice-converter-cyclegan_b200/csrc/tc_gemm.cu b/voice-converter-cyclegan_b200/csrc/tc_gemm.cu
--- a/voice-converter-cyclegan_b200/csrc/tc_gemm.cu
+++ b/voice-converter-cyclegan_b200/csrc/tc_gemm.cu
@@ -42,6 +42,17 @@
   return enc(m, dt, 3, const_cast<void*>(base), dims, strides, box, es, CU_TENSOR_MAP_INTERLEAVE_NONE,
              b0 * esize == 64 ? CU_TENSOR_MAP_SWIZZLE_64B : CU_TENSOR_MAP_SWIZZLE_128B, CU_TENSOR_MAP_L2_PROMOTION_L2_256B,
              CU_TENSOR_MAP_FLOAT_OOB_FILL_NONE) == CUDA_SUCCESS;
+}
+
+bool make_tmap4_16(CUtensorMap* m, const void* base, CUtensorMapDataType dt, uint64_t d0, uint64_t d1, uint64_t d2, uint64_t d3, uint32_t b1, uint32_t b3) {
+  EncodeTiledFn enc = get_encoder();
+  if (!enc) return false;
+  cuuint64_t dims[4] = {d0, d1, d2, d3};
+  cuuint64_t strides[3] = {d0 * 2, d0 * d1 * 2, d0 * d1 * d2 * 2};
+  cuuint32_t box[4] = {64, b1, 1, b3};
+  cuuint32_t es[4] = {1, 1, 1, 1};
+  return enc(m, dt, 4, const_cast<void*>(base), dims, strides, box, es, CU_TENSOR_MAP_INTERLEAVE_NONE,
+             CU_TENSOR_MAP_SWIZZLE_128B, CU_TENSOR_MAP_L2_PROMOTION_L2_256B, CU_TENSOR_MAP_FLOAT_OOB_FILL_NONE) == CUDA_SUCCESS;
 }
 
 __device__ __forceinline__ uint32_t smem_u32(const void* p) { return (uint32_t)__cvta_generic_to_shared(p); }
@@ -74,6 +85,10 @@
   asm volatile("cp.async.bulk.tensor.3d.shared::cluster.global.tile.mbarrier::complete_tx::bytes [%0], [%1, {%2, %3, %4}], [%5];"
                ::"r"(dst_smem), "l"(map), "r"(c0), "r"(c1), "r"(c2), "r"(smem_u32(bar)) : "memory");
 }
+__device__ __forceinline__ void tma_load4(uint32_t dst_smem, const CUtensorMap* map, int c0, int c1, int c2, int c3, uint64_t* bar) {
+  asm volatile("cp.async.bulk.tensor.4d.shared::cluster.global.tile.mbarrier::complete_tx::bytes [%0], [%1, {%2, %3, %4, %5}], [%6];"
+               ::"r"(dst_smem), "l"(map), "r"(c0), "r"(c1), "r"(c2), "r"(c3), "r"(smem_u32(bar)) : "memory");
+}
 __device__ __forceinline__ void tma_prefetch_desc(const CUtensorMap* map) {
   asm volatile("prefetch.tensormap [%0];" ::"l"(map) : "memory");
 }
@@ -119,7 +134,9 @@
 __device__ __forceinline__ uint32_t sw128(int r, int c) { return (uint32_t)((r >> 3) * 1024 + (r & 7) * 128 + ((c ^ (r & 7)) << 4)); }
 
 struct TcNTParams {
-  GatherGeom g;
+  GatherGeom g[CGVC_MAX_CLASSES];
+  int ncls;
+  int mt0[CGVC_MAX_CLASSES + 1];
   const __nv_bfloat16 *a_hi, *a_lo; int a_ld; int C;
   const __nv_bfloat16 *b_hi, *b_lo; int Nw;
   int N;
@@ -143,19 +160,26 @@
   PackGeom pk;
 };
 
+static_assert(sizeof(TcNTParams) <= 4096, "the NT kernel's parameters stay within the classic 4 KB kernel-parameter space");
+
+
 struct TcTNParams {
-  GatherGeom g;
+  GatherGeom g[CGVC_MAX_WG_CLASSES];
+  int ncls;
+  int tap0[CGVC_MAX_WG_CLASSES + 1];
+  int rows4;
   const __nv_bfloat16 *x_hi, *x_lo; int x_ld; int C;
   const __nv_bfloat16 *g_hi, *g_lo; int g_ld; int N;
   float* dw_a; float* dw_g; int n_split;
   int ksplit;
-  FastDiv div_hw, div_w;
+  FastDiv div_hw[CGVC_MAX_WG_CLASSES], div_w[CGVC_MAX_WG_CLASSES];
   CUtensorMap tm_g_hi, tm_g_lo;
   const uint8_t *x8_hi, *x8_lo;
   const uint8_t *g8_hi, *g8_lo;
   int w16;
   int fold_n;
 };
+static_assert(sizeof(TcTNParams) <= 4096, "the TN kernel's parameters stay within the classic 4 KB kernel-parameter space");
 
 __device__ __forceinline__ float* tn_dst(float* base, int slab, int C, int c, int ncols, int col, int fold_n) {
   if (fold_n) { const int t = col / fold_n; return base + ((long long)t * C + c) * fold_n + (col - t * fold_n); }
@@ -374,7 +398,7 @@
 __device__ __forceinline__ void nt_tile_epilogue(const TcNTParams& p, const long long M, const int HW, const long long m0, const int n0,
                                                  const int q, const int lane, float* stg, float** rowp, float* bc, float (*epi_xch)[32],
                                                  const float* acc, const int grp = 0, const int ngrp = 1) {
-  const GatherGeom& g = p.g;
+  const GatherGeom& g = p.g[0];
   const int barid = 1 + grp;
   const int arow = q * 32 + lane;
   const long long mq = m0 + q * 32;
@@ -692,9 +716,8 @@
 }
 
 template <int BN>
-__device__ __forceinline__ void nt_store_fragments(const TcNTParams& p, const float (&d)[BN / 2], const long long M, const int HW,
-                                                   const long long m0, const int n0, const int r, const int c) {
-  const GatherGeom& g = p.g;
+__device__ __forceinline__ void nt_store_fragments(const TcNTParams& p, const GatherGeom& g, const float (&d)[BN / 2], const long long M,
+                                                   const int HW, const long long m0, const int n0, const int r, const int c) {
   float* rowp[2];
 #pragma unroll
   for (int h = 0; h < 2; ++h) {
@@ -751,14 +774,10 @@
 
   const uint32_t smem_base = (smem_u32(smem_raw) + 1023u) & ~1023u;
   const int warp = threadIdx.x >> 5, lane = threadIdx.x & 31;
-  const GatherGeom& g = p.g;
-  const long long M = (long long)g.B * g.Hy * g.Wx;
-  const int HW = g.Hy * g.Wx;
   const int cchunks = p.C >> 6;
-  const int kb_pass = g.ntaps * cchunks;
-  const int num_kb = NPL == 3 ? 2 * kb_pass : kb_pass;
-  const int m_tiles = (int)((M + 127) / 128);
+  const int m_tiles = p.mt0[p.ncls];
   const int n_tiles = p.n_tiles;
+  auto tile_class = [&](int mt) { int c = 0; if (EPI == 0 && !PK) while (mt >= p.mt0[c + 1]) ++c; return c; };
   const int num_tiles = m_tiles * n_tiles;
 
   if (threadIdx.x == 0) {
@@ -777,7 +796,11 @@
     int stage = 0; uint32_t phase = 0;
     int it = 0;
     for (int tile = blockIdx.x; tile < num_tiles; tile += gridDim.x, ++it) {
-      const long long m0 = (long long)(tile % m_tiles) * 128;
+      const int mt = tile % m_tiles, cls = tile_class(mt);
+      const GatherGeom& g = p.g[cls];
+      const long long M = (long long)g.B * g.Hy * g.Wx;
+      const int HW = g.Hy * g.Wx;
+      const long long m0 = (long long)(mt - p.mt0[cls]) * 128;
       const int n0 = (tile / m_tiles) * BN;
       if (EPI != 0 && it > 0) mbar_wait(&acc_free_bar, (uint32_t)(it - 1) & 1u);
       int rb[8], ry[8], rx[8];
@@ -861,8 +884,14 @@
     float* acc_s = reinterpret_cast<float*>(smem_raw + (smem_base - smem_u32(smem_raw)));
     int stage = 0; uint32_t phase = 0;
     for (int tile = blockIdx.x; tile < num_tiles; tile += gridDim.x) {
-      const long long m0 = (long long)(tile % m_tiles) * 128;
+      const int mt = tile % m_tiles, cls = tile_class(mt);
+      const GatherGeom& g = p.g[cls];
+      const long long M = (long long)g.B * g.Hy * g.Wx;
+      const int HW = g.Hy * g.Wx;
+      const long long m0 = (long long)(mt - p.mt0[cls]) * 128;
       const int n0 = (tile / m_tiles) * BN;
+      const int kb_pass = g.ntaps * cchunks;
+      const int num_kb = NPL == 3 ? 2 * kb_pass : kb_pass;
       float d[BN / 2];
 #pragma unroll
       for (int i = 0; i < BN / 2; ++i) d[i] = 0.f;
@@ -879,7 +908,7 @@
       if (lane == 0) mbar_arrive(&empty_bar[prev]);
       const int r0 = wg * 64 + (tw >> 5) * 16 + ((tw & 31) >> 2), c0 = 2 * (tw & 3);
       if constexpr (EPI == 0) {
-        if (!(p.debug & 3)) nt_store_fragments<BN>(p, d, M, HW, m0, n0, r0, c0);
+        if (!(p.debug & 3)) nt_store_fragments<BN>(p, g, d, M, HW, m0, n0, r0, c0);
       } else {
         consumer_bar();
         if (!(p.debug & 2)) {
@@ -922,21 +951,23 @@
 
   const uint32_t smem_base = (smem_u32(smem_raw) + 1023u) & ~1023u;
   const int warp = threadIdx.x >> 5, lane = threadIdx.x & 31;
-  const GatherGeom& g = p.g;
-  const long long M = (long long)g.B * g.Hy * g.Wx;
-  const int HW = g.Hy * g.Wx;
   const int n_tiles = (p.g_ld + BN - 1) / BN, c_tiles = (p.x_ld + 127) / 128;
-  const int num_items = n_tiles * c_tiles * g.ntaps * p.ksplit;
+  const int npairs = p.tap0[p.ncls];
+  const int num_items = n_tiles * c_tiles * npairs * p.ksplit;
   constexpr int pass0 = (NPL == 3 && !W16) ? 0 : 1;
-  long long chunk_rows = (M + p.ksplit - 1) / p.ksplit;
-  chunk_rows = (chunk_rows + 63) / 64 * 64;
-
-  struct Item { int n0, c0, tap; long long mbeg, mend; int num_kb; };
+
+  struct Item { int n0, c0, cls, tap; long long mbeg, mend; int num_kb; };
   auto decode = [&](int item) -> Item {
     Item w;
     int n_t = item % n_tiles; int t1 = item / n_tiles;
     int c_t = t1 % c_tiles; int t2 = t1 / c_tiles;
-    w.tap = t2 % g.ntaps; int ks = t2 / g.ntaps;
+    const int pair = t2 % npairs; int ks = t2 / npairs;
+    w.cls = 0; while (pair >= p.tap0[w.cls + 1]) ++w.cls;
+    w.tap = pair - p.tap0[w.cls];
+    const GatherGeom& g = p.g[w.cls];
+    const long long M = (long long)g.B * g.Hy * g.Wx;
+    long long chunk_rows = (M + p.ksplit - 1) / p.ksplit;
+    chunk_rows = (chunk_rows + 63) / 64 * 64;
     w.n0 = n_t * BN; w.c0 = c_t * 128;
     w.mbeg = (long long)ks * chunk_rows;
     w.mend = (w.mbeg + chunk_rows < M) ? w.mbeg + chunk_rows : M;
@@ -958,20 +989,24 @@
     int stage = 0; uint32_t phase = 0;
     for (int item = blockIdx.x; item < num_items; item += gridDim.x) {
       const Item w = decode(item);
+      const GatherGeom& g = p.g[w.cls];
+      const int HW = g.Hy * g.Wx;
       for (int pass = pass0; pass < 2; ++pass)
       for (int kb = 0; kb < w.num_kb; ++kb) {
         mbar_wait(&empty_bar[stage], phase ^ 1);
         const uint32_t sA = smem_base + stage * Cfg::STAGE;
         const uint32_t sB = sA + Cfg::PLANES * Cfg::A_PLANE;
         long long xoff[4];
+        long long grow[4];
 #pragma unroll
         for (int i = 0; i < 4; ++i) {
           const long long m = w.mbeg + (long long)kb * 64 + rsub + 16 * i;
-          xoff[i] = -1;
+          xoff[i] = -1; grow[i] = m;
           if (m < w.mend) {
             const uint32_t mu = (uint32_t)m;
-            int b = (int)fdiv(mu, p.div_hw); int rem = (int)(mu - (uint32_t)b * (uint32_t)HW);
-            int y = (int)fdiv((uint32_t)rem, p.div_w); int x = rem - y * g.Wx;
+            int b = (int)fdiv(mu, p.div_hw[w.cls]); int rem = (int)(mu - (uint32_t)b * (uint32_t)HW);
+            int y = (int)fdiv((uint32_t)rem, p.div_w[w.cls]); int x = rem - y * g.Wx;
+            if (p.rows4) grow[i] = ((long long)b * g.Hd + g.doy) * g.Wd + x;
             int yy = y * g.sy + g.oy[w.tap], xx = x * g.sx + g.ox[w.tap];
             if (yy >= 0 && yy < g.Hs && xx >= 0 && xx < g.Ws)
               xoff[i] = ((long long)(b * g.Hs + yy) * g.Ws + xx) * p.x_ld + w.c0 + chunk * 8;
@@ -996,7 +1031,7 @@
               const int col = w.n0 + a * 64 + chunk * 8;
               const bool ok = m < w.mend && col < p.g_ld;
               uint2 vh = make_uint2(0u, 0u), vl = make_uint2(0u, 0u);
-              if (ok) { vh = __ldg(reinterpret_cast<const uint2*>(p.g8_hi + m * p.g_ld + col)); vl = __ldg(reinterpret_cast<const uint2*>(p.g8_lo + m * p.g_ld + col)); }
+              if (ok) { vh = __ldg(reinterpret_cast<const uint2*>(p.g8_hi + grow[i] * p.g_ld + col)); vl = __ldg(reinterpret_cast<const uint2*>(p.g8_lo + grow[i] * p.g_ld + col)); }
               st_shared16(sB + a * 8192 + so, e4m3x8_to_f16x8(vh));
               st_shared16(sB + Cfg::B_PLANE + a * 8192 + so, e4m3x8_to_f16x8(vl));
             }
@@ -1014,8 +1049,13 @@
 #pragma unroll
             for (int a = 0; a < 4; ++a) {
               if ((w.n0 + a * 64) < p.g_ld) {
-                tma_load3(sB + a * 8192, &p.tm_g_hi, w.n0 + a * 64, row0, 0, &full_bar[stage]);
-                if (NPL == 2) tma_load3(sB + Cfg::B_PLANE + a * 8192, &p.tm_g_lo, w.n0 + a * 64, row0, 0, &full_bar[stage]);
+                if (p.rows4) {
+                  tma_load4(sB + a * 8192, &p.tm_g_hi, w.n0 + a * 64, 0, g.doy, row0 / g.Wx, &full_bar[stage]);
+                  if (NPL == 2) tma_load4(sB + Cfg::B_PLANE + a * 8192, &p.tm_g_lo, w.n0 + a * 64, 0, g.doy, row0 / g.Wx, &full_bar[stage]);
+                } else {
+                  tma_load3(sB + a * 8192, &p.tm_g_hi, w.n0 + a * 64, row0, 0, &full_bar[stage]);
+                  if (NPL == 2) tma_load3(sB + Cfg::B_PLANE + a * 8192, &p.tm_g_lo, w.n0 + a * 64, row0, 0, &full_bar[stage]);
+                }
               }
             }
           }
@@ -1069,7 +1109,7 @@
 #pragma unroll
         for (int h = 0; h < 2; ++h) {
           if (c + 8 * h >= p.C) continue;
-          float* dst = tn_dst(base, g.widx[w.tap], p.C, c + 8 * h, ncols, nn, p.fold_n);
+          float* dst = tn_dst(base, p.g[w.cls].widx[w.tap], p.C, c + 8 * h, ncols, nn, p.fold_n);
           asm volatile("red.global.add.v2.f32 [%0], {%1, %2};" ::"l"(dst), "f"(d[4 * j + 2 * h]), "f"(d[4 * j + 2 * h + 1]) : "memory");
         }
       }
@@ -1266,18 +1306,30 @@
 }
 
 cudaError_t launch_nt(TcNTParams p, int precision, cudaStream_t st, int epi) {
-  const long long M = (long long)p.g.B * p.g.Hy * p.g.Wx;
+  if (p.ncls < 1 || p.ncls > CGVC_MAX_CLASSES || ((epi != 0 || p.pk.off) && p.ncls != 1)) return cudaErrorInvalidValue;
+  long long M = 0, mt = 0;
+  double flops = 0.0;
+  int K = 0;
+  p.mt0[0] = 0;
+  for (int c = 0; c < p.ncls; ++c) {
+    const GatherGeom& g = p.g[c];
+    const long long Mc = (long long)g.B * g.Hy * g.Wx;
+    if (g.ntaps == 0) return cudaErrorInvalidValue;
+    M += Mc; mt += (Mc + 127) / 128; p.mt0[c + 1] = (int)mt;
+    flops += 2.0 * (double)Mc * p.N * g.ntaps * p.C;
+    if (g.ntaps * p.C > K) K = g.ntaps * p.C;
+  }
   if (M == 0) return cudaSuccess;
   const bool x3 = precision == 1;
-  if (p.g.ntaps == 0) return cudaErrorInvalidValue;
   const int bn = tile_rows(p.N, p.Nw);
   p.n_tiles = bn == 32 ? 1 : p.Nw / bn;
-  const long long tiles = ((M + 127) / 128) * p.n_tiles;
+  const long long tiles = mt * p.n_tiles;
+  if (tiles >= (1ll << 31)) return cudaErrorInvalidValue;
   dim3 grid((unsigned)(tiles < num_sms() ? tiles : num_sms()));
   cudaError_t e;
   ++g_cgvc_launches;
   p.debug = g_tc_debug;
-  prof_begin(st, 2.0 * (double)M * p.N * p.g.ntaps * p.C, (epi == 1 || epi == 2 || epi == 5) ? 2 : 0, M, p.N, p.g.ntaps * p.C);
+  prof_begin(st, flops, (epi == 1 || epi == 2 || epi == 5) ? 2 : 0, M, p.N, K);
 #define LAUNCH_NT(BN_, NPL_, EPI_, ...)                                                                        \
   do {                                                                                                         \
     e = set_smem(tc_gg_nt_kernel<BN_, NPL_, EPI_, ##__VA_ARGS__>, NTCfg<BN_, NPL_>::SMEM);                     \
@@ -1286,7 +1338,7 @@
   } while (0)
   if (epi != 0 && bn != 256) return cudaErrorInvalidValue;
   if (p.pk.off) {
-    if (epi != 0 || p.g.B != 1 || p.g.Hy != 1) return cudaErrorInvalidValue;
+    if (epi != 0 || p.g[0].B != 1 || p.g[0].Hy != 1) return cudaErrorInvalidValue;
     const int npl = precision == 3 ? 3 : x3 ? 2 : 1;
     if (bn == 256)      { if (npl == 3) LAUNCH_NT(256, 3, 0, true); else if (npl == 2) LAUNCH_NT(256, 2, 0, true); else LAUNCH_NT(256, 1, 0, true); }
     else if (bn == 128) { if (npl == 3) LAUNCH_NT(128, 3, 0, true); else if (npl == 2) LAUNCH_NT(128, 2, 0, true); else LAUNCH_NT(128, 1, 0, true); }
@@ -1315,12 +1367,26 @@
 }
 
 cudaError_t launch_tn(TcTNParams p, int precision, cudaStream_t st) {
-  const long long M = (long long)p.g.B * p.g.Hy * p.g.Wx;
+  if (p.ncls < 1 || p.ncls > CGVC_MAX_WG_CLASSES || (p.ncls > 1 && !p.rows4)) return cudaErrorInvalidValue;
+  long long M = 0, Mmin = -1;
+  double flops = 0.0;
+  int K = 0;
+  p.tap0[0] = 0;
+  for (int c = 0; c < p.ncls; ++c) {
+    const GatherGeom& g = p.g[c];
+    const long long Mc = (long long)g.B * g.Hy * g.Wx;
+    if (g.ntaps == 0) return cudaErrorInvalidValue;
+    M += Mc; if (Mmin < 0 || Mc < Mmin) Mmin = Mc;
+    p.tap0[c + 1] = p.tap0[c] + g.ntaps;
+    flops += 2.0 * (double)Mc * p.N * g.ntaps * p.C;
+    if (g.ntaps * p.C > K) K = g.ntaps * p.C;
+    p.div_hw[c] = make_fastdiv((uint32_t)(g.Hy * g.Wx)); p.div_w[c] = make_fastdiv((uint32_t)g.Wx);
+  }
   if (M == 0) return cudaSuccess;
   if (M >= (1ll << 31)) return cudaErrorInvalidValue;
-  const int tiles = ((p.g_ld + 255) / 256) * ((p.x_ld + 127) / 128) * p.g.ntaps;
+  const int tiles = ((p.g_ld + 255) / 256) * ((p.x_ld + 127) / 128) * p.tap0[p.ncls];
   const int nsm = num_sms();
-  long long maxsplit = M / 1024; if (maxsplit < 1) maxsplit = 1; if (maxsplit > 32) maxsplit = 32;
+  long long maxsplit = Mmin / 1024; if (maxsplit < 1) maxsplit = 1; if (maxsplit > 32) maxsplit = 32;
   int ksplit = 1; double best = 0.0;
   for (int ks = 1; ks <= (int)maxsplit; ++ks) {
     long long items = (long long)tiles * ks;
@@ -1329,12 +1395,11 @@
     if (eff > best + 0.02) { best = eff; ksplit = ks; }
   }
   p.ksplit = ksplit;
-  p.div_hw = make_fastdiv((uint32_t)(p.g.Hy * p.g.Wx)); p.div_w = make_fastdiv((uint32_t)p.g.Wx);
   const long long items = (long long)tiles * ksplit;
   dim3 grid((unsigned)(items < nsm ? items : nsm));
   cudaError_t e;
   ++g_cgvc_launches;
-  prof_begin(st, 2.0 * (double)M * p.N * p.g.ntaps * p.C, 1, M, p.N, p.g.ntaps * p.C);
+  prof_begin(st, flops, 1, M, p.N, K);
 #define LAUNCH_TN(NPL_, W16_)                                                                     \
   do {                                                                                            \
     e = set_smem(tc_gg_tn_kernel<NPL_, W16_>, TNCfg<NPL_, W16_>::SMEM);                           \
@@ -1423,11 +1488,16 @@
 }
 
 int layer_fwd(const TcLayer& L, int precision, const __nv_bfloat16* xhi, const __nv_bfloat16* xlo, int n, int H, int W, int sh, int sw,
-              float* P, cudaStream_t st, const TcFuse* fuse = nullptr, bool* fused_out = nullptr, const PackGeom* pk = nullptr) {
+              float* P, cudaStream_t st, bool classes, const TcFuse* fuse = nullptr, bool* fused_out = nullptr, const PackGeom* pk = nullptr) {
   if (!layer_ok(L) || (precision == 3 && !layer_ok_q(L))) return TC_UNSUPPORTED;
   if (pk && (n != 1 || H != 1 || L.kh != 1 || fuse)) return (int)cudaErrorInvalidValue;
   TcNTParams p; memset(&p, 0, sizeof p);
-  p.g = fwd_geom(n, H, W, L.kh, L.kw, sh, sw);
+  {
+    const std::vector<GatherGeom> gs = classes ? fwd_classes(n, H, W, L.kh, L.kw, sh, sw)
+                                               : std::vector<GatherGeom>{fwd_geom(n, H, W, L.kh, L.kw, sh, sw)};
+    p.ncls = (int)gs.size();
+    for (int c = 0; c < p.ncls; ++c) p.g[c] = gs[c];
+  }
   if (pk) p.pk = *pk;
   p.a_hi = xhi; p.a_lo = xlo; p.a_ld = cin_k(L); p.C = cin_k(L);
   p.b_hi = L.wf_hi; p.b_lo = L.wf_lo; p.Nw = nt_n(L); p.N = Ntot(L);
@@ -1442,7 +1512,8 @@
   }
   int epi = 0;
   if (fuse && fuse->R > 0) {
-    const bool shape_ok = H == 1 && (fuse->R == 32 || fuse->R == 64 || fuse->R == 128) && p.g.Wx == fuse->R && nt_n(L) % 256 == 0 && Ntot(L) == nt_n(L);
+    const bool shape_ok = H == 1 && p.ncls == 1 && (fuse->R == 32 || fuse->R == 64 || fuse->R == 128) && p.g[0].Wx == fuse->R && nt_n(L) % 256 == 0 &&
+                          Ntot(L) == nt_n(L);
     if (shape_ok && L.gated && p.perm == 1) epi = 1; else if (shape_ok && L.gated && p.perm == 2) epi = 5; else if (shape_ok && !L.gated) epi = 2;
     if (epi) {
       p.R = fuse->R; p.gamma_a = fuse->gamma_a; p.beta_a = fuse->beta_a; p.gamma_g = fuse->gamma_g; p.beta_g = fuse->beta_g;
@@ -1458,19 +1529,25 @@
 }
 
 int layer_dgrad(const TcLayer& L, int precision, const __nv_bfloat16* dPhi, const __nv_bfloat16* dPlo, int n, int H, int W, int sh, int sw,
-                float* dx, int accumulate, cudaStream_t st, const TcBwdFuse* fuse = nullptr, bool* fused_out = nullptr) {
+                float* dx, int accumulate, cudaStream_t st, bool classes, const TcBwdFuse* fuse = nullptr, bool* fused_out = nullptr) {
   if (fused_out) *fused_out = false;
   if (!layer_ok(L) || (precision == 3 && (!layer_ok_q(L) || !L.wdq16))) return TC_UNSUPPORTED;
   std::vector<GatherGeom> gs = dgrad_geoms(n, H, W, L.kh, L.kw, sh, sw);
   for (const GatherGeom& g : gs) if (g.ntaps == 0) return TC_UNSUPPORTED;
+  std::vector<std::vector<GatherGeom>> launches;
+  if (classes) launches.push_back(row_classes(gs));
+  else for (const GatherGeom& g : gs) launches.push_back(std::vector<GatherGeom>{g});
   int epi = 0;
   if (fuse && fuse->R > 0 && gs.size() == 1 && H == 1 && sh == 1 && sw == 1 && (fuse->R == 32 || fuse->R == 64 || fuse->R == 128) &&
       gs[0].Wx == fuse->R && cin_n(L) % 256 == 0 && L.cin == cin_n(L) && fuse->bp && fuse->stats && fuse->dp_hi && fuse->dp_lo && fuse->gamma_a &&
       (fuse->gated ? (fuse->gamma_g && fuse->beta_a && fuse->beta_g) : (dx != nullptr)) && precision != 3)
     epi = fuse->gated ? 3 : 4;
-  for (const GatherGeom& g : gs) {
+  for (const std::vector<GatherGeom>& lg : launches) {
+    if (lg.size() > CGVC_MAX_CLASSES) return (int)cudaErrorInvalidValue;
+    const GatherGeom& g = lg[0];
     TcNTParams p; memset(&p, 0, sizeof p);
-    p.g = g;
+    p.ncls = (int)lg.size();
+    for (int c = 0; c < p.ncls; ++c) p.g[c] = lg[c];
     p.a_hi = dPhi; p.a_lo = dPlo; p.a_ld = nt_k(L); p.C = nt_k(L);
     p.b_hi = L.wd_hi; p.b_lo = L.wd_lo; p.Nw = cin_n(L); p.N = L.cin;
     p.dst = dx; p.d_ld = L.cin; p.bias = nullptr; p.accumulate = accumulate;
@@ -1495,24 +1572,36 @@
 
 int layer_wgrad(const TcLayer& L, int precision, const __nv_bfloat16* xhi, const __nv_bfloat16* xlo,
                 const __nv_bfloat16* dPhi, const __nv_bfloat16* dPlo, int n, int H, int W, int sh, int sw,
-                float* dwa, float* dwg, cudaStream_t st, int w16 = 0) {
+                float* dwa, float* dwg, cudaStream_t st, bool classes, int w16 = 0) {
   if (!layer_ok(L) || (precision == 3 && !layer_ok_q(L))) return TC_UNSUPPORTED;
   TcTNParams p; memset(&p, 0, sizeof p);
   p.w16 = (precision == 3 && w16) ? 1 : 0;
   p.fold_n = L.fold ? L.cout / L.fold : 0;
-  p.g = fwd_geom(n, H, W, L.kh, L.kw, sh, sw);
+  {
+    const std::vector<GatherGeom> gs = classes ? wgrad_classes(n, H, W, L.kh, L.kw, sh, sw)
+                                               : std::vector<GatherGeom>{fwd_geom(n, H, W, L.kh, L.kw, sh, sw)};
+    p.ncls = (int)gs.size();
+    for (int c = 0; c < p.ncls; ++c) p.g[c] = gs[c];
+    p.rows4 = p.ncls > 1;
+  }
+  const GatherGeom& g0 = p.g[0];
   p.x_hi = xhi; p.x_lo = xlo; p.x_ld = cin_k(L); p.C = L.cin;
   p.g_hi = dPhi; p.g_lo = dPlo; p.g_ld = nt_k(L); p.N = Ntot(L);
   p.dw_a = dwa; p.dw_g = dwg; p.n_split = L.cout;
-  const long long M = (long long)p.g.B * p.g.Hy * p.g.Wx;
+  const long long M = (long long)n * g0.Hd * g0.Wd;
+  auto gmap = [&](CUtensorMap* m, const void* base, CUtensorMapDataType dt, uint64_t ld) {
+    if (p.rows4) return make_tmap4_16(m, base, dt, ld, (uint64_t)g0.Wd, (uint64_t)g0.Hd, (uint64_t)n, (uint32_t)g0.Wd, (uint32_t)(64 / g0.Wd));
+    return make_tmap3_t(m, base, dt, 2, ld, (uint64_t)M, 1, 64, 64);
+  };
+  const CUtensorMapDataType BF16 = CU_TENSOR_MAP_DATA_TYPE_BFLOAT16;
   if (precision == 3) {
     const long long rows_in = (long long)n * H * W;
     p.x_ld = cin_q(L); p.g_ld = nt_q(L); p.x_lo = p.g_lo = nullptr;
     p.x8_hi = reinterpret_cast<const uint8_t*>(xlo); p.x8_lo = p.x8_hi + rows_in * p.x_ld;
     p.g8_hi = reinterpret_cast<const uint8_t*>(dPlo); p.g8_lo = p.g8_hi + M * p.g_ld;
-    if (!make_tmap3_t(&p.tm_g_hi, dPhi, CU_TENSOR_MAP_DATA_TYPE_FLOAT16, 2, (uint64_t)p.g_ld, (uint64_t)M, 1, 64, 64))
+    if (!gmap(&p.tm_g_hi, dPhi, CU_TENSOR_MAP_DATA_TYPE_FLOAT16, (uint64_t)p.g_ld))
       return (int)cudaErrorInvalidValue;
-  } else if (!make_tmap3(&p.tm_g_hi, dPhi, (uint64_t)nt_k(L), (uint64_t)M, 1, 64) || !make_tmap3(&p.tm_g_lo, dPlo, (uint64_t)nt_k(L), (uint64_t)M, 1, 64)) {
+  } else if (!gmap(&p.tm_g_hi, dPhi, BF16, (uint64_t)nt_k(L)) || !gmap(&p.tm_g_lo, dPlo, BF16, (uint64_t)nt_k(L))) {
     return (int)cudaErrorInvalidValue;
   }
   return (int)launch_tn(p, precision, st);
@@ -1672,18 +1761,18 @@
 
 int tc_conv_fwd(TcWeights& w, int slot, const __nv_bfloat16* xhi, const __nv_bfloat16* xlo, int n, int H, int W, int sh, int sw,
                 float* P, cudaStream_t st, const TcFuse* fuse, bool* fused, const PackGeom* pk) {
-  return layer_fwd(w.layers[slot], w.precision, xhi, xlo, n, H, W, sh, sw, P, st, fuse, fused, pk);
+  return layer_fwd(w.layers[slot], w.precision, xhi, xlo, n, H, W, sh, sw, P, st, w.tap_classes, fuse, fused, pk);
 }
 
 int tc_conv_dgrad(TcWeights& w, int slot, const __nv_bfloat16* dPhi, const __nv_bfloat16* dPlo, int n, int H, int W, int sh, int sw,
                   float* dx, int accumulate, cudaStream_t st, const TcBwdFuse* fuse, bool* fused) {
-  return layer_dgrad(w.layers[slot], w.precision, dPhi, dPlo, n, H, W, sh, sw, dx, accumulate, st, fuse, fused);
+  return layer_dgrad(w.layers[slot], w.precision, dPhi, dPlo, n, H, W, sh, sw, dx, accumulate, st, w.tap_classes, fuse, fused);
 }
 
 int tc_conv_wgrad(TcWeights& w, int slot, const __nv_bfloat16* xhi, const __nv_bfloat16* xlo,
                   const __nv_bfloat16* dPhi, const __nv_bfloat16* dPlo, int n, int H, int W, int sh, int sw,
                   float* dwa, float* dwg, cudaStream_t st) {
-  return layer_wgrad(w.layers[slot], w.precision, xhi, xlo, dPhi, dPlo, n, H, W, sh, sw, dwa, dwg, st, w.wgrad16 ? 1 : 0);
+  return layer_wgrad(w.layers[slot], w.precision, xhi, xlo, dPhi, dPlo, n, H, W, sh, sw, dwa, dwg, st, w.tap_classes, w.wgrad16 ? 1 : 0);
 }
 
 bool tc_profile_is_on() { return g_prof_on; }
@@ -1752,7 +1841,7 @@
 }
 
 int tc_conv_fwd_adhoc(int precision, const float* x, const float* w, const float* bias, float* y,
-                      int B, int H, int W, int Cin, int kh, int kw, int Cout, int sh, int sw, cudaStream_t st) {
+                      int B, int H, int W, int Cin, int kh, int kw, int Cout, int sh, int sw, cudaStream_t st, bool classes) {
   TcLayer L{}; L.kh = kh; L.kw = kw; L.cin = Cin; L.cout = Cout; L.gated = 0;
   if (!layer_ok(L) || (precision == 3 && !layer_ok_q(L))) return TC_UNSUPPORTED;
   Temp T;
@@ -1767,12 +1856,12 @@
   r = refresh_layer(L, w, nullptr, bias ? bias : zero, nullptr, st); if (r) return r;
   cudaError_t e = tc_split_planes(precision, x, (long long)rows, Cin, xhi, xlo, st);
   if (e != cudaSuccess) return (int)e;
-  r = layer_fwd(L, precision, xhi, xlo, B, H, W, sh, sw, y, st); if (r) return r;
+  r = layer_fwd(L, precision, xhi, xlo, B, H, W, sh, sw, y, st, classes); if (r) return r;
   return (int)cudaStreamSynchronize(st);
 }
 
 int tc_conv_bwd_adhoc(int precision, const float* x, const float* w, const float* dy, float* dx, float* dw, float* dbias,
-                      int B, int H, int W, int Cin, int kh, int kw, int Cout, int sh, int sw, cudaStream_t st, int w16) {
+                      int B, int H, int W, int Cin, int kh, int kw, int Cout, int sh, int sw, cudaStream_t st, int w16, bool classes) {
   TcLayer L{}; L.kh = kh; L.kw = kw; L.cin = Cin; L.cout = Cout; L.gated = 0;
   if (!layer_ok(L) || (precision == 3 && !layer_ok_q(L))) return TC_UNSUPPORTED;
   Temp T;
@@ -1791,9 +1880,9 @@
   if (e != cudaSuccess) return (int)e;
   e = tc_split_planes(precision, dy, (long long)orows, Cout, ghi, glo, st);
   if (e != cudaSuccess) return (int)e;
-  if (dx) { r = layer_dgrad(L, precision, ghi, glo, B, H, W, sh, sw, dx, 0, st); if (r) return r; }
+  if (dx) { r = layer_dgrad(L, precision, ghi, glo, B, H, W, sh, sw, dx, 0, st, classes); if (r) return r; }
   if (dw) {
-    r = layer_wgrad(L, precision, xhi, xlo, ghi, glo, B, H, W, sh, sw, dw, nullptr, st, w16); if (r) return r;
+    r = layer_wgrad(L, precision, xhi, xlo, ghi, glo, B, H, W, sh, sw, dw, nullptr, st, classes, w16); if (r) return r;
     if (dbias) { e = launch_colsum(dy, (long long)orows, Cout, 0, Cout, dbias, st); if (e != cudaSuccess) return (int)e; }
   }
   return (int)cudaStreamSynchronize(st);
diff --git a/voice-converter-cyclegan_b200/csrc/tc_gemm.cuh b/voice-converter-cyclegan_b200/csrc/tc_gemm.cuh
--- a/voice-converter-cyclegan_b200/csrc/tc_gemm.cuh
+++ b/voice-converter-cyclegan_b200/csrc/tc_gemm.cuh
@@ -33,6 +33,7 @@
   bool quant = false;
   bool wgrad16 = false;
   bool quant_bwd = false;
+  bool tap_classes = true;
   void* prep_jobs = nullptr;
   std::vector<int> job_first;
   std::vector<size_t> job_ka;
@@ -73,9 +74,9 @@
                   const __nv_bfloat16* dPhi, const __nv_bfloat16* dPlo, int n, int H, int W, int sh, int sw,
                   float* dwa, float* dwg, cudaStream_t st);
 int tc_conv_fwd_adhoc(int precision, const float* x, const float* w, const float* bias, float* y,
-                      int B, int H, int W, int Cin, int kh, int kw, int Cout, int sh, int sw, cudaStream_t st);
+                      int B, int H, int W, int Cin, int kh, int kw, int Cout, int sh, int sw, cudaStream_t st, bool classes);
 int tc_conv_bwd_adhoc(int precision, const float* x, const float* w, const float* dy, float* dx, float* dw, float* dbias,
-                      int B, int H, int W, int Cin, int kh, int kw, int Cout, int sh, int sw, cudaStream_t st, int w16 = 0);
+                      int B, int H, int W, int Cin, int kh, int kw, int Cout, int sh, int sw, cudaStream_t st, int w16, bool classes);
 
 void tc_profile_enable(int on);
 bool tc_profile_is_on();
```

After: 9.522, median of 6. About the same (+0.3%).
